# nipponjo/tts-arabic-pytorch

Measured on AMD Instinct MI355X. Metric: audio samples/sec (FastPitch+HiFi-GAN, synthetic 64-phoneme inputs), higher is better.
Workload: dtype f32

## Files before the change

### include/ttsamd.h

```cpp
#ifndef TTSAMD_H
#define TTSAMD_H

#include <stdint.h>

#ifdef __cplusplus
extern "C" {
#endif

#define TTSAMD_OK 0
#define TTSAMD_EINVAL (-1)
#define TTSAMD_EHIP (-2)
#define TTSAMD_ENOMEM (-3)

typedef struct ttsamd_tensor {
    const char* name;
    const float* data;
    int32_t ndim;
    int64_t shape[4];
} ttsamd_tensor;

typedef struct ttsamd_hifigan_cfg {
    int32_t num_mels;
    int32_t upsample_initial_channel;
    int32_t n_ups;
    int32_t upsample_rates[8];
    int32_t upsample_kernel_sizes[8];
    int32_t n_kernels;
    int32_t resblock_kernel_sizes[8];
    int32_t n_dilations;
    int32_t resblock_dilations[8][8];
} ttsamd_hifigan_cfg;

typedef struct ttsamd_fastpitch_cfg {
    int32_t n_mel_channels;
    int32_t n_symbols;
    int32_t padding_idx;
    int32_t d_model;
    int32_t in_fft_n_layers, in_fft_n_heads, in_fft_d_head, in_fft_kernel, in_fft_filter;
    int32_t out_fft_n_layers, out_fft_n_heads, out_fft_d_head, out_fft_kernel, out_fft_filter;
    int32_t dur_kernel, dur_filter, dur_n_layers;
    int32_t pitch_kernel, pitch_filter, pitch_n_layers, pitch_emb_kernel;
    int32_t energy_conditioning, energy_kernel, energy_filter, energy_n_layers, energy_emb_kernel;
    int32_t n_speakers;
    float speaker_emb_weight;
} ttsamd_fastpitch_cfg;

typedef struct ttsamd_tacotron2_cfg {
    int32_t n_symbol;
    int32_t num_speakers;
    int32_t speaker_embedding_dim;
    int32_t symbol_embedding_dim;
    int32_t encoder_embedding_dim;
    int32_t encoder_n_convolution;
    int32_t encoder_kernel_size;
    int32_t n_mels;
    int32_t prenet_dim;
    int32_t attention_rnn_dim;
    int32_t decoder_rnn_dim;
    int32_t attention_hidden_dim;
    int32_t attention_location_n_filter;
    int32_t attention_location_kernel_size;
    int32_t postnet_n_convolution;
    int32_t postnet_kernel_size;
    int32_t postnet_embedding_dim;
    float gate_threshold;
    int32_t decoder_early_stopping;
} ttsamd_tacotron2_cfg;

typedef struct ttsamd_tagger_cfg {
    int32_t n_vocab;
    int32_t emb_dim;
    int32_t n_lstm;
    int32_t lstm_hidden[4];
    int32_t hard_sigmoid;
    int32_t bn_after_lstm0;
    float bn_eps;
    int32_t n_dense;
    int32_t dense_dim[4];
} ttsamd_tagger_cfg;

const char* ttsamd_last_error(void);
#define TTSAMD_ABI_VERSION 7
int32_t ttsamd_version(void);
int32_t ttsamd_set_option(const char* name, const char* value);
int32_t ttsamd_get_option(const char* name, char* value, int32_t capacity);
const char* ttsamd_option_name(int32_t index);
int32_t ttsamd_options_check(void);
int32_t ttsamd_device_ok(void);


int32_t ttsamd_hifigan_create(const ttsamd_tensor* weights, int32_t n_weights,
                              const ttsamd_hifigan_cfg* cfg, void** handle);
int32_t ttsamd_hifigan_destroy(void* handle);
int64_t ttsamd_hifigan_workspace_bytes(void* handle, int32_t batch, int32_t t_max);
int32_t ttsamd_hifigan_forward(void* handle, const float* mel, const int64_t* lens,
                               int32_t batch, int32_t t_max, float* wave,
                               void* workspace, int64_t workspace_bytes, void* stream);


int32_t ttsamd_fastpitch_create(const ttsamd_tensor* weights, int32_t n_weights,
                                const ttsamd_fastpitch_cfg* cfg, void** handle);
int32_t ttsamd_fastpitch_destroy(void* handle);
int64_t ttsamd_fastpitch_encode_workspace_bytes(void* handle, int32_t batch, int32_t n_tokens);
int64_t ttsamd_fastpitch_decode_workspace_bytes(void* handle, int32_t batch, int32_t t_max);

int32_t ttsamd_fastpitch_encode(void* handle, const int64_t* ids, int32_t batch, int32_t n_tokens,
                                int32_t speaker, float pace, const float* dur_tgt,
                                const float* pitch_tgt, const float* energy_tgt,
                                float pitch_mul, float pitch_add, float max_duration,
                                float* enc_cond, float* dur_pred, float* pitch_pred,
                                float* energy_pred, int64_t* reps, int64_t* dec_lens,
                                void* workspace, int64_t workspace_bytes, void* stream);

int32_t ttsamd_length_regulate(const float* enc, const int64_t* reps, int32_t batch,
                               int32_t n_tokens, int32_t channels, int32_t t_max,
                               float* out, int32_t* idx, void* stream);

int32_t ttsamd_fastpitch_decode(void* handle, float* x, const int64_t* dec_lens, int32_t batch,
                                int32_t t_max, float* mel, void* workspace,
                                int64_t workspace_bytes, void* stream);

int32_t ttsamd_fastpitch_set_batch_mode(void* handle, int32_t mode);

int32_t ttsamd_denoiser_create(void** handle);
int32_t ttsamd_denoiser_destroy(void* handle);
int64_t ttsamd_denoiser_workspace_bytes(int32_t batch, int32_t n_max);
int32_t ttsamd_denoiser_bias_spec(void* handle, const float* audio, const int64_t* n_dev, int32_t n,
                                  float* bias_spec, void* workspace, int64_t workspace_bytes,
                                  void* stream);
int32_t ttsamd_denoise(void* handle, float* wave, int64_t wave_stride, const int64_t* nsamples,
                       int32_t batch, int32_t n_max, const float* bias_spec, float strength,
                       void* workspace, int64_t workspace_bytes, void* stream);

int32_t ttsamd_vocos_create(const ttsamd_tensor* weights, int32_t n_weights, int32_t input_channels,
                            int32_t dim, int32_t intermediate_dim, int32_t num_layers, void** handle);
int32_t ttsamd_vocos_destroy(void* handle);
int64_t ttsamd_vocos_workspace_bytes(void* handle, int32_t batch, int32_t t_max);
int32_t ttsamd_vocos_bias_vec(void* handle, float* bias_vec, void* workspace, int64_t workspace_bytes,
                              void* stream);
int32_t ttsamd_vocos_forward(void* handle, const float* mel, const int64_t* lens, int32_t batch,
                             int32_t t_max, float denoise, const float* bias_vec, float* wave,
                             void* workspace, int64_t workspace_bytes, void* stream);

int32_t ttsamd_tacotron2_create(const ttsamd_tensor* weights, int32_t n_weights,
                                const ttsamd_tacotron2_cfg* cfg, void** handle);
int32_t ttsamd_tacotron2_destroy(void* handle);
int64_t ttsamd_tacotron2_workspace_bytes(void* handle, int32_t batch, int32_t n_tokens, int32_t max_step);
int32_t ttsamd_tacotron2_infer(void* handle, const int64_t* tokens, const int64_t* lengths,
                               const int64_t* speaker_ids, int32_t batch, int32_t n_tokens, int32_t max_step,
                               int64_t dropout_seed, float* mel_post, int32_t* mel_lens, float* alignments,
                               float* mel_raw, int32_t* n_steps, void* workspace, int64_t workspace_bytes,
                               void* stream);

int32_t ttsamd_tagger_create(const ttsamd_tensor* weights, int32_t n_weights, const ttsamd_tagger_cfg* cfg,
                             void** handle);
int32_t ttsamd_tagger_destroy(void* handle);
int64_t ttsamd_tagger_workspace_bytes(void* handle, int32_t batch, int32_t n_chars);
int32_t ttsamd_tagger_forward(void* handle, const int64_t* ids, int32_t batch, int32_t n_chars, float* probs,
                              void* workspace, int64_t workspace_bytes, void* stream);


int64_t ttsamd_conv1d_packed_floats(int32_t cout, int32_t cin, int32_t k);
int32_t ttsamd_conv1d(const float* x, const float* w, const float* bias, const int64_t* lens,
                      int32_t batch, int32_t cin, int32_t cout, int32_t k, int32_t dilation,
                      int32_t lin, float in_slope, int32_t relu_out, float* y, float* packed,
                      void* stream);
int32_t ttsamd_conv1d_ex(const float* x, const float* w, const float* bias, const float* res, const int64_t* lens, int32_t batch,
                         int32_t cin, int32_t cout, int32_t k, int32_t dilation, int32_t lin, float in_slope,
                         int32_t relu_out, int32_t mode, float div, float* y, float* packed, void* stream);

int64_t ttsamd_resblock_pair_packed_floats(int32_t channels, int32_t k, int32_t variant);
int32_t ttsamd_resblock_pair(const float* x, float* y, const float* w1, const float* b1, const float* w2, const float* b2,
                             int32_t channels, int32_t k, int32_t dil, const int64_t* lens, int32_t len_mul, int32_t L,
                             int32_t batch, int32_t mode, float div, float slope, int32_t variant, float* packed, int64_t packed_floats,
                             void* stream);

int32_t ttsamd_bfo_pack(const float* x, int32_t batch, int32_t channels, int32_t len, float slope, void* out, void* stream);
int32_t ttsamd_bfo_unpack(const void* in, int32_t batch, int32_t channels, int32_t len, float slope, float* out, void* stream);
int64_t ttsamd_bfo_weight_elems(int32_t cout, int32_t cin, int32_t k, int32_t up);
int32_t ttsamd_bfo_pack_weight(const float* w, int32_t cout, int32_t cin, int32_t k, int32_t up, uint16_t* out);
int32_t ttsamd_bfo_conv1d(const void* x, const void* w_packed, const float* bias, const void* res, const void* sum_in,
                          const int64_t* lens, int32_t len_mul, int32_t batch, int32_t cin, int32_t cout, int32_t k,
                          int32_t dilation, int32_t up, int32_t len_in, int32_t mode, float div, float res_slope,
                          float out_slope, void* y, float* y_f32, const float* res_f32, void* stream);
int32_t ttsamd_bfo_resblock_pair(const void* x, const void* w1, const float* b1, const void* w2, const float* b2,
                                 const void* sum_in, const int64_t* lens, int32_t len_mul, int32_t batch, int32_t channels,
                                 int32_t k, int32_t dilation, int32_t len, int32_t mode, float div, float in_slope,
                                 float mid_slope, float out_slope, void* y, void* stream);
int32_t ttsamd_bfo_resblock_chain(const void* x, const void* const* w1, const float* const* b1, const void* const* w2,
                                  const float* const* b2, const int32_t* dilations, const void* sum_in, const int64_t* lens,
                                  int32_t len_mul, int32_t batch, int32_t channels, int32_t len, int32_t mode, float div,
                                  float in_slope, float mid_slope, float out_slope, void* y, void* stream, int32_t k);
int32_t ttsamd_bfo_conv_post(const void* x, const float* w, const float* bias, const int64_t* lens, int32_t len_mul,
                             int32_t batch, int32_t channels, int32_t len, float* wave, int64_t wave_stride, void* stream);

int32_t ttsamd_bfo3_pack(const float* x, int32_t batch, int32_t channels, int32_t len, float slope, void* out, void* stream);
int32_t ttsamd_bfo3_unpack(const void* in, int32_t batch, int32_t channels, int32_t len, float slope, float* out, void* stream);
int64_t ttsamd_bfo3_weight_elems(int32_t cout, int32_t cin, int32_t k, int32_t up);
int32_t ttsamd_bfo3_pack_weight(const float* w, int32_t cout, int32_t cin, int32_t k, int32_t up, uint16_t* out);
int32_t ttsamd_bfo3_conv1d(const void* x, const void* w_packed, const float* bias, const void* res, const void* sum_in,
                           const int64_t* lens, int32_t len_mul, int32_t batch, int32_t cin, int32_t cout, int32_t k,
                           int32_t dilation, int32_t up, int32_t len_in, int32_t mode, float div, float res_slope,
                           float out_slope, void* y, float* y_f32, const float* res_f32, void* stream);
int32_t ttsamd_bfo3_resblock_pair(const void* x, const void* w1, const float* b1, const void* w2, const float* b2,
                                  const void* sum_in, const int64_t* lens, int32_t len_mul, int32_t batch, int32_t channels,
                                  int32_t k, int32_t dilation, int32_t len, int32_t mode, float div, float in_slope,
                                  float mid_slope, float out_slope, void* y, void* stream);
int32_t ttsamd_bfo3_resblock_chain(const void* x, const void* const* w1, const float* const* b1, const void* const* w2,
                                   const float* const* b2, const int32_t* dilations, const void* sum_in, const int64_t* lens,
                                   int32_t len_mul, int32_t batch, int32_t channels, int32_t len, int32_t mode, float div,
                                   float in_slope, float mid_slope, float out_slope, void* y, void* stream);
int32_t ttsamd_bfo3_conv_post(const void* x, const float* w, const float* bias, const int64_t* lens, int32_t len_mul,
                              int32_t batch, int32_t channels, int32_t len, float* wave, int64_t wave_stride, void* stream);

int32_t ttsamd_set_precision(int32_t precision);
int32_t ttsamd_get_precision(void);

#define TTSAMD_DP_ID_BYTES 128
#define TTSAMD_DP_HIFIGAN 0
#define TTSAMD_DP_FASTPITCH 1
int32_t ttsamd_dp_unique_id(void* id128 );
int32_t ttsamd_dp_init(int32_t rank, int32_t world, const void* id128 , void** comm);
int32_t ttsamd_dp_destroy(void* comm);
int32_t ttsamd_dp_rank(void* comm);
int32_t ttsamd_dp_world(void* comm);
int32_t ttsamd_dp_broadcast(void* comm, void* buf, int64_t nbytes, int32_t root, void* stream);
int32_t ttsamd_dp_broadcast_weights(void* comm, int32_t kind, void* handle, int32_t root, void* stream);
int32_t ttsamd_dp_allgather(void* comm, const void* send, void* recv, int64_t nbytes_per_rank, void* stream);
int32_t ttsamd_dp_pack_audio(const float* wave, int64_t wave_stride, const int64_t* nsamples, int32_t batch,
                             int64_t n_max, float* packed, void* stream);
int32_t ttsamd_dp_gather_audio(void* comm, const float* packed, float* recv, const int64_t* counts,
                               const int64_t* offsets, int32_t root, void* stream);

int32_t ttsamd_profile_enable(int32_t on);
int32_t ttsamd_profile_read(double* out3);

#ifdef __cplusplus
}
#endif
#endif
```

### tts-arabic-pytorch_amd/csrc/api.hip

```cpp
#include <cerrno>
#include <cstdio>
#include <cstdlib>
#include <cstring>
#include <algorithm>
#include <atomic>
#include <mutex>
#include <string>
#include <vector>

#include "kernels.hpp"

namespace ttsamd {

static thread_local std::string g_err;

void set_error(const char* fmt, ...) {
    char buf[1024];
    va_list ap;
    va_start(ap, fmt);
    vsnprintf(buf, sizeof(buf), fmt, ap);
    va_end(ap);
    g_err = buf;
}

static int g_precision = 0;
int32_t default_precision() { return g_precision; }

struct Prof {
    std::mutex mu;
    bool on = false;
    std::vector<hipEvent_t> ev;
    size_t used = 0;
    size_t launches = 0;
    double flops_per_frame = 0.0;
} g_prof;

void prof_section_begin(hipStream_t s) {
    if (!g_prof.on) return;
    std::lock_guard<std::mutex> lk(g_prof.mu);
    if (g_prof.used + 2 > g_prof.ev.size()) {
        hipEvent_t a, b;
        if (hipEventCreate(&a) != hipSuccess || hipEventCreate(&b) != hipSuccess) return;
        g_prof.ev.push_back(a);
        g_prof.ev.push_back(b);
    }
    (void)hipEventRecord(g_prof.ev[g_prof.used], s);
}

void prof_section_end(hipStream_t s) {
    if (!g_prof.on) return;
    std::lock_guard<std::mutex> lk(g_prof.mu);
    if (g_prof.used + 2 > g_prof.ev.size()) return;
    (void)hipEventRecord(g_prof.ev[g_prof.used + 1], s);
    g_prof.used += 2;
}

void prof_add(double flops_per_frame) {
    if (!g_prof.on) return;
    std::lock_guard<std::mutex> lk(g_prof.mu);
    g_prof.launches += 1;
    g_prof.flops_per_frame += flops_per_frame;
}

void prof_begin(hipStream_t s, double flops_per_frame) {
    prof_section_begin(s);
    prof_add(flops_per_frame);
}

void prof_end(hipStream_t s) { prof_section_end(s); }

struct HifiGan;
struct FastPitch;
struct Denoiser;
struct Vocos;
int32_t vocos_create(const ttsamd_tensor*, int32_t, int32_t, int32_t, int32_t, int32_t, Vocos**);
void vocos_destroy(Vocos*);
int64_t vocos_workspace_bytes(const Vocos*, int32_t, int32_t);
int64_t vocos_bias_workspace_bytes(const Vocos*);
int32_t vocos_bias_vec(const Vocos*, float*, void*, int64_t, hipStream_t);
int32_t vocos_forward(const Vocos*, const float*, const int64_t*, int32_t, int32_t, float, const float*, float*, void*,
                      int64_t, hipStream_t);
struct Taco2;
int32_t tacotron2_create(const ttsamd_tensor*, int32_t, const ttsamd_tacotron2_cfg*, Taco2**);
void tacotron2_destroy(Taco2*);
int64_t tacotron2_workspace_bytes(const Taco2*, int32_t, int32_t, int32_t);
int32_t tacotron2_infer(const Taco2*, const int64_t*, const int64_t*, const int64_t*, int32_t, int32_t, int32_t, int64_t,
                        float*, int32_t*, float*, float*, int32_t*, void*, int64_t, hipStream_t);
struct Tagger;
int32_t tagger_create(const ttsamd_tensor*, int32_t, const ttsamd_tagger_cfg*, Tagger**);
void tagger_destroy(Tagger*);
int64_t tagger_workspace_bytes(const Tagger*, int32_t, int32_t);
int32_t tagger_forward(const Tagger*, const int64_t*, int32_t, int32_t, float*, void*, int64_t, hipStream_t);
int32_t denoiser_create(Denoiser**);
void denoiser_destroy(Denoiser*);
int64_t denoiser_workspace_bytes(int32_t, int32_t);
int32_t denoiser_bias_spec(const Denoiser*, const float*, const int64_t*, int32_t, float*, void*, int64_t, hipStream_t);
int32_t denoise(const Denoiser*, float*, int64_t, const int64_t*, int32_t, int32_t, const float*, float, void*, int64_t,
                hipStream_t);
int32_t hifigan_create(const ttsamd_tensor*, int32_t, const ttsamd_hifigan_cfg*, HifiGan**);
void hifigan_destroy(HifiGan*);
int64_t hifigan_workspace_bytes(const HifiGan*, int32_t, int32_t);
int32_t hifigan_forward(const HifiGan*, const float*, const int64_t*, int32_t, int32_t, float*, void*, int64_t,
                        hipStream_t);
int32_t fastpitch_create(const ttsamd_tensor*, int32_t, const ttsamd_fastpitch_cfg*, int32_t, FastPitch**);
void fastpitch_destroy(FastPitch*);
int64_t fastpitch_encode_workspace_bytes(const FastPitch*, int32_t, int32_t);
int64_t fastpitch_decode_workspace_bytes(const FastPitch*, int32_t, int32_t);
int32_t fastpitch_encode(const FastPitch*, const int64_t*, int32_t, int32_t, int32_t, float, const float*,
                         const float*, const float*, float, float, float, float*, float*, float*, float*, int64_t*,
                         int64_t*, void*, int64_t, hipStream_t);
void fastpitch_set_batch_mode(const FastPitch*, int);
int32_t fastpitch_decode(const FastPitch*, float*, const int64_t*, int32_t, int32_t, float*, void*, int64_t,
                         hipStream_t);

__global__ void pack_conv_weight_kernel(const float* __restrict__ w, int cout, int cin, int k, int cp,
                                        float* __restrict__ out) {
    const int64_t i = (int64_t)blockIdx.x * 256 + threadIdx.x;
    const int64_t n = (int64_t)cin * k * cp;
    if (i >= n) return;
    const int pq = (int)(i % 4);
    const int co = (int)((i / 4) % cp);
    const int kk = (int)((i / (4 * (int64_t)cp)) % 2);
    const int t = (int)((i / (8 * (int64_t)cp)) % k);
    const int o = (int)(i / (8 * (int64_t)cp * k));
    out[i] = co < cout ? w[((int64_t)co * cin + (8 * o + 2 * pq + kk)) * k + t] : 0.f;
}

__global__ void split_bf16_kernel(const float* __restrict__ packed, int64_t n, unsigned short* __restrict__ out) {
    const int64_t i = (int64_t)blockIdx.x * 256 + threadIdx.x;
    if (i >= n) return;
    const float f = packed[i];
    unsigned u = __float_as_uint(f);
    u += 0x7fffu + ((u >> 16) & 1u);
    const unsigned h = u >> 16;
    const float r = f - __uint_as_float(h << 16);
    unsigned v = __float_as_uint(r);
    v += 0x7fffu + ((v >> 16) & 1u);
    out[i] = (unsigned short)h;
    out[n + i] = (unsigned short)(v >> 16);
}

namespace {
struct OptDesc { const char* name; int kind; long long lo, hi; };
const OptDesc kOpts[OPT_COUNT] = {
#define TTS_OPT_DESC(name, kind, lo, hi) {"TTSAMD_" #name, kind, lo, hi},
    TTS_OPTIONS(TTS_OPT_DESC)
#undef TTS_OPT_DESC
};
std::atomic<const char*> g_opt[OPT_COUNT];
std::once_flag g_opt_once;
std::string g_opt_env_error;

bool opt_valid(const OptDesc& d, const char* v) {
    if (!v || !*v) return false;
    char* end = nullptr;
    errno = 0;
    const long long x = std::strtoll(v, &end, d.kind == 1 ? 16 : 10);
    return errno == 0 && end != v && *end == '\0' && x >= d.lo && x <= d.hi;
}
void opt_init() {
    std::call_once(g_opt_once, [] {
        for (int i = 0; i < OPT_COUNT; ++i) {
            const char* e = std::getenv(kOpts[i].name);
            if (!e || !*e) continue;
            if (!opt_valid(kOpts[i], e)) {
                if (g_opt_env_error.empty()) {
                    char buf[256];
                    std::snprintf(buf, sizeof buf, "%s='%s' in the environment is not a valid value (%s in [%llx, %llx])", kOpts[i].name, e,
                                  kOpts[i].kind == 1 ? "hex mask" : "integer", kOpts[i].lo, kOpts[i].hi);
                    g_opt_env_error = buf;
                }
                continue;
            }
            g_opt[i].store(strdup(e), std::memory_order_release);
        }
    });
}
int opt_find(const char* name) {
    if (!name) return -1;
    for (int i = 0; i < OPT_COUNT; ++i)
        if (std::strcmp(name, kOpts[i].name) == 0 || std::strcmp(name, kOpts[i].name + 7) == 0) return i;
    return -1;
}
}

int64_t opt_int(Opt o, int64_t unset) {
    opt_init();
    const char* v = g_opt[o].load(std::memory_order_acquire);
    return v ? (int64_t)std::strtoll(v, nullptr, kOpts[o].kind == 1 ? 16 : 10) : unset;
}

}

using namespace ttsamd;

extern "C" {

const char* ttsamd_last_error(void) { return g_err.c_str(); }
int32_t ttsamd_version(void) { return TTSAMD_ABI_VERSION; }

int32_t ttsamd_set_option(const char* name, const char* value) {
    opt_init();
    const int i = opt_find(name);
    TTS_REQUIRE(i >= 0, "set_option: unknown option '%s' (ttsamd_option_name lists them)", name ? name : "(null)");
    if (!value || !*value) {
        g_opt[i].store(nullptr, std::memory_order_release);
        return 0;
    }
    TTS_REQUIRE(opt_valid(kOpts[i], value), "set_option: %s='%s' is not a valid value (%s in [%llx, %llx])", kOpts[i].name, value,
                kOpts[i].kind == 1 ? "hex mask" : "integer", kOpts[i].lo, kOpts[i].hi);
    g_opt[i].store(strdup(value), std::memory_order_release);
    return 0;
}
int32_t ttsamd_get_option(const char* name, char* value, int32_t capacity) {
    opt_init();
    const int i = opt_find(name);
    TTS_REQUIRE(i >= 0 && value && capacity > 0, "get_option: unknown option '%s' or no buffer", name ? name : "(null)");
    const char* v = g_opt[i].load(std::memory_order_acquire);
    std::snprintf(value, (size_t)capacity, "%s", v ? v : "");
    return 0;
}
const char* ttsamd_option_name(int32_t index) { return (index >= 0 && index < OPT_COUNT) ? kOpts[index].name : nullptr; }
int32_t ttsamd_options_check(void) {
    opt_init();
    TTS_REQUIRE(g_opt_env_error.empty(), "%s", g_opt_env_error.c_str());
    return 0;
}

int32_t ttsamd_device_ok(void) {
    int n = 0;
    if (hipGetDeviceCount(&n) != hipSuccess || n <= 0) return 0;
    hipDeviceProp_t prop;
    if (hipGetDeviceProperties(&prop, 0) != hipSuccess) return 0;
    return std::string(prop.gcnArchName).rfind("gfx950", 0) == 0 ? 1 : 0;
}

int32_t ttsamd_hifigan_create(const ttsamd_tensor* weights, int32_t n, const ttsamd_hifigan_cfg* cfg, void** handle) {
    HifiGan* h = nullptr;
    const int32_t rc = hifigan_create(weights, n, cfg, &h);
    if (rc == 0) *handle = h;
    return rc;
}
int32_t ttsamd_hifigan_destroy(void* handle) {
    hifigan_destroy((HifiGan*)handle);
    return 0;
}
int64_t ttsamd_hifigan_workspace_bytes(void* handle, int32_t batch, int32_t t_max) {
    if (!handle || batch < 1 || t_max < 1) return 0;
    return hifigan_workspace_bytes((HifiGan*)handle, batch, t_max);
}
int32_t ttsamd_hifigan_forward(void* handle, const float* mel, const int64_t* lens, int32_t batch, int32_t t_max,
                               float* wave, void* workspace, int64_t workspace_bytes, void* stream) {
    return hifigan_forward((HifiGan*)handle, mel, lens, batch, t_max, wave, workspace, workspace_bytes,
                           (hipStream_t)stream);
}

int32_t ttsamd_fastpitch_create(const ttsamd_tensor* weights, int32_t n, const ttsamd_fastpitch_cfg* cfg,
                                void** handle) {
    FastPitch* h = nullptr;
    const int32_t rc = fastpitch_create(weights, n, cfg, 16384, &h);
    if (rc == 0) *handle = h;
    return rc;
}
int32_t ttsamd_fastpitch_destroy(void* handle) {
    fastpitch_destroy((FastPitch*)handle);
    return 0;
}
int64_t ttsamd_fastpitch_encode_workspace_bytes(void* handle, int32_t batch, int32_t n_tokens) {
    if (!handle || batch < 1 || n_tokens < 1) return 0;
    return fastpitch_encode_workspace_bytes((FastPitch*)handle, batch, n_tokens);
}
int64_t ttsamd_fastpitch_decode_workspace_bytes(void* handle, int32_t batch, int32_t t_max) {
    if (!handle || batch < 1 || t_max < 1) return 0;
    return fastpitch_decode_workspace_bytes((FastPitch*)handle, batch, t_max);
}
int32_t ttsamd_fastpitch_encode(void* handle, const int64_t* ids, int32_t batch, int32_t n_tokens, int32_t speaker,
                                float pace, const float* dur_tgt, const float* pitch_tgt, const float* energy_tgt,
                                float pitch_mul, float pitch_add, float max_duration, float* enc_cond,
                                float* dur_pred, float* pitch_pred, float* energy_pred, int64_t* reps,
                                int64_t* dec_lens, void* workspace, int64_t workspace_bytes, void* stream) {
    return fastpitch_encode((FastPitch*)handle, ids, batch, n_tokens, speaker, pace, dur_tgt, pitch_tgt, energy_tgt,
                            pitch_mul, pitch_add, max_duration, enc_cond, dur_pred, pitch_pred, energy_pred, reps,
                            dec_lens, workspace, workspace_bytes, (hipStream_t)stream);
}
int32_t ttsamd_length_regulate(const float* enc, const int64_t* reps, int32_t batch, int32_t n_tokens,
                               int32_t channels, int32_t t_max, float* out, int32_t* idx, void* stream) {
    TTS_REQUIRE(enc && reps && out && batch >= 1 && n_tokens >= 1 && channels >= 1 && t_max >= 0,
                "length_regulate: bad argument");
    return launch_regulate_gather(enc, reps, nullptr, 0, batch, n_tokens, channels, t_max, out, idx,
                                  (hipStream_t)stream);
}
int32_t ttsamd_fastpitch_set_batch_mode(void* handle, int32_t mode) {
    TTS_REQUIRE(handle != nullptr, "fastpitch_set_batch_mode: null handle");
    TTS_REQUIRE(mode == 0 || mode == 1, "fastpitch_set_batch_mode: mode %d (0 = padded-batch arithmetic, 1 = every utterance alone)", mode);
    fastpitch_set_batch_mode((const FastPitch*)handle, mode);
    return 0;
}
int32_t ttsamd_fastpitch_decode(void* handle, float* x, const int64_t* dec_lens, int32_t batch, int32_t t_max,
                                float* mel, void* workspace, int64_t workspace_bytes, void* stream) {
    return fastpitch_decode((FastPitch*)handle, x, dec_lens, batch, t_max, mel, workspace, workspace_bytes,
                            (hipStream_t)stream);
}

int32_t ttsamd_denoiser_create(void** handle) {
    Denoiser* h = nullptr;
    const int32_t rc = denoiser_create(&h);
    if (rc == 0) *handle = h;
    return rc;
}
int32_t ttsamd_denoiser_destroy(void* handle) {
    denoiser_destroy((Denoiser*)handle);
    return 0;
}
int64_t ttsamd_denoiser_workspace_bytes(int32_t batch, int32_t n_max) {
    if (batch < 1 || n_max < 1) return 0;
    return denoiser_workspace_bytes(batch, n_max);
}
int32_t ttsamd_denoiser_bias_spec(void* handle, const float* audio, const int64_t* n_dev, int32_t n,
                                  float* bias_spec, void* workspace, int64_t workspace_bytes, void* stream) {
    return denoiser_bias_spec((Denoiser*)handle, audio, n_dev, n, bias_spec, workspace, workspace_bytes,
                              (hipStream_t)stream);
}
int32_t ttsamd_denoise(void* handle, float* wave, int64_t wave_stride, const int64_t* nsamples, int32_t batch,
                       int32_t n_max, const float* bias_spec, float strength, void* workspace,
                       int64_t workspace_bytes, void* stream) {
    return denoise((Denoiser*)handle, wave, wave_stride, nsamples, batch, n_max, bias_spec, strength, workspace,
                   workspace_bytes, (hipStream_t)stream);
}

int32_t ttsamd_vocos_create(const ttsamd_tensor* weights, int32_t n, int32_t input_channels, int32_t dim,
                            int32_t intermediate_dim, int32_t num_layers, void** handle) {
    Vocos* h = nullptr;
    const int32_t rc = vocos_create(weights, n, input_channels, dim, intermediate_dim, num_layers, &h);
    if (rc == 0) *handle = h;
    return rc;
}
int32_t ttsamd_vocos_destroy(void* handle) {
    vocos_destroy((Vocos*)handle);
    return 0;
}
int64_t ttsamd_vocos_workspace_bytes(void* handle, int32_t batch, int32_t t_max) {
    if (!handle || batch < 1 || t_max < 1) return 0;
    const int64_t a = vocos_workspace_bytes((Vocos*)handle, batch, t_max), b = vocos_bias_workspace_bytes((Vocos*)handle);
    return a > b ? a : b;
}
int32_t ttsamd_vocos_bias_vec(void* handle, float* bias_vec, void* workspace, int64_t workspace_bytes, void* stream) {
    return vocos_bias_vec((Vocos*)handle, bias_vec, workspace, workspace_bytes, (hipStream_t)stream);
}
int32_t ttsamd_vocos_forward(void* handle, const float* mel, const int64_t* lens, int32_t batch, int32_t t_max,
                             float denoise, const float* bias_vec, float* wave, void* workspace,
                             int64_t workspace_bytes, void* stream) {
    return vocos_forward((Vocos*)handle, mel, lens, batch, t_max, denoise, bias_vec, wave, workspace, workspace_bytes,
                         (hipStream_t)stream);
}

int32_t ttsamd_tacotron2_create(const ttsamd_tensor* weights, int32_t n, const ttsamd_tacotron2_cfg* cfg, void** handle) {
    TTS_REQUIRE(handle, "tacotron2_create: null handle");
    Taco2* h = nullptr;
    const int32_t rc = tacotron2_create(weights, n, cfg, &h);
    if (rc == 0) *handle = h;
    return rc;
}
int32_t ttsamd_tacotron2_destroy(void* handle) {
    tacotron2_destroy((Taco2*)handle);
    return 0;
}
int64_t ttsamd_tacotron2_workspace_bytes(void* handle, int32_t batch, int32_t n_tokens, int32_t max_step) {
    if (!handle || batch < 1 || n_tokens < 1 || max_step < 1) return 0;
    return tacotron2_workspace_bytes((Taco2*)handle, batch, n_tokens, max_step);
}
int32_t ttsamd_tacotron2_infer(void* handle, const int64_t* tokens, const int64_t* lengths, const int64_t* speaker_ids,
                               int32_t batch, int32_t n_tokens, int32_t max_step, int64_t dropout_seed, float* mel_post,
                               int32_t* mel_lens, float* alignments, float* mel_raw, int32_t* n_steps, void* workspace,
                               int64_t workspace_bytes, void* stream) {
    return tacotron2_infer((Taco2*)handle, tokens, lengths, speaker_ids, batch, n_tokens, max_step, dropout_seed, mel_post,
                           mel_lens, alignments, mel_raw, n_steps, workspace, workspace_bytes, (hipStream_t)stream);
}

int32_t ttsamd_tagger_create(const ttsamd_tensor* weights, int32_t n, const ttsamd_tagger_cfg* cfg, void** handle) {
    TTS_REQUIRE(handle, "tagger_create: null handle");
    Tagger* h = nullptr;
    const int32_t rc = tagger_create(weights, n, cfg, &h);
    if (rc == 0) *handle = h;
    return rc;
}
int32_t ttsamd_tagger_destroy(void* handle) {
    tagger_destroy((Tagger*)handle);
    return 0;
}
int64_t ttsamd_tagger_workspace_bytes(void* handle, int32_t batch, int32_t n_chars) {
    if (!handle || batch < 1 || n_chars < 1) return 0;
    return tagger_workspace_bytes((Tagger*)handle, batch, n_chars);
}
int32_t ttsamd_tagger_forward(void* handle, const int64_t* ids, int32_t batch, int32_t n_chars, float* probs,
                              void* workspace, int64_t workspace_bytes, void* stream) {
    return tagger_forward((Tagger*)handle, ids, batch, n_chars, probs, workspace, workspace_bytes, (hipStream_t)stream);
}

int64_t ttsamd_conv1d_packed_floats(int32_t cout, int32_t cin, int32_t k) {
    return 2 * (int64_t)cin * k * cout_padded(cout) +
           ((k == 3 || k == 7 || k == 11) ? (int64_t)cin * (wino2_groups(k) + wino4_groups(k)) * cout_padded(cout) : 0);
}

__global__ void pack_wino4_weight_kernel(const float* __restrict__ w, int cout, int cin, int k, int cp, float* __restrict__ out) {
    const int ng = k == 3 ? 6 : (k == 7 ? 16 : 24), nsf = k == 3 ? 1 : (k == 7 ? 2 : 4);
    const int64_t i = (int64_t)blockIdx.x * 256 + threadIdx.x;
    const int64_t n = (int64_t)cin * ng * cp;
    if (i >= n) return;
    const int pq = (int)(i & 3);
    const int64_t r = i >> 2;
    const int co = (int)(r % cp);
    const int64_t r2 = r / cp;
    const int kk = (int)(r2 & 1);
    const int64_t r3 = r2 >> 1;
    const int t = (int)(r3 % ng), o = (int)(r3 / ng);
    float v = 0.f;
    if (co < cout) {
        const float* g = w + ((int64_t)co * cin + (8 * o + 2 * pq + kk)) * k;
        if (t < 6 * nsf) {
            const int s = t / 6, j = t % 6;
            const double g0 = g[3 * s], g1 = 3 * s + 1 < k ? g[3 * s + 1] : 0.0, g2 = 3 * s + 2 < k ? g[3 * s + 2] : 0.0;
            v = j == 0 ? (float)(g0 / 4) : (j == 1 ? (float)(-(g0 + g1 + g2) / 6) : (j == 2 ? (float)(-(g0 - g1 + g2) / 6) :
                (j == 3 ? (float)(g0 / 24 + g1 / 12 + g2 / 6) : (j == 4 ? (float)(g0 / 24 - g1 / 12 + g2 / 6) : (float)g2))));
        } else {
            v = g[6];
        }
    }
    out[i] = v;
}

__global__ void pack_wino2_weight_kernel(const float* __restrict__ w, int cout, int cin, int k, int cp, float* __restrict__ out) {
    const int ns = k / 3, ng = 4 * ns + 2 * (k - 3 * ns);
    const int64_t i = (int64_t)blockIdx.x * 256 + threadIdx.x;
    const int64_t n = (int64_t)cin * ng * cp;
    if (i >= n) return;
    const int pq = (int)(i & 3);
    const int64_t r = i >> 2;
    const int co = (int)(r % cp);
    const int64_t r2 = r / cp;
    const int kk = (int)(r2 & 1);
    const int64_t r3 = r2 >> 1;
    const int t = (int)(r3 % ng), o = (int)(r3 / ng);
    float v = 0.f;
    if (co < cout) {
        const float* g = w + ((int64_t)co * cin + (8 * o + 2 * pq + kk)) * k;
        if (t < 4 * ns) {
            const int s = t >> 2, j = t & 3;
            const double g0 = g[3 * s], g1 = g[3 * s + 1], g2 = g[3 * s + 2];
            v = j == 0 ? (float)g0 : (j == 1 ? (float)((g0 + g1 + g2) * 0.5) : (j == 2 ? (float)((g0 - g1 + g2) * 0.5) : (float)g2));
        } else {
            const int l = (t - 4 * ns) >> 1;
            v = ((t - 4 * ns) & 1) ? -g[3 * ns + l] : g[3 * ns + l];
        }
    }
    out[i] = v;
}

int32_t ttsamd_conv1d_ex(const float* x, const float* w, const float* bias, const float* res, const int64_t* lens, int32_t batch,
                         int32_t cin, int32_t cout, int32_t k, int32_t dilation, int32_t lin, float in_slope,
                         int32_t relu_out, int32_t mode, float div, float* y, float* packed, void* stream) {
    TTS_REQUIRE(x && w && y && packed, "conv1d: null argument");
    TTS_REQUIRE(mode >= 0 && mode <= 2 && (mode != 2 || div != 0.f), "conv1d: bad mode / div");
    TTS_REQUIRE(relu_out == 0 || mode == 0, "conv1d: relu_out with an accumulate mode (mode %d) is not defined", mode);
    hipStream_t s = (hipStream_t)stream;
    const int cp = cout_padded(cout);
    const int64_t n = (int64_t)cin * k * cp;
    hipLaunchKernelGGL(pack_conv_weight_kernel, dim3((unsigned)((n + 255) / 256)), dim3(256), 0, s, w, cout, cin, k,
                       cp, packed);
    TTS_CHECK_HIP(hipGetLastError());
    ConvParams p;
    std::memset(&p, 0, sizeof(p));
    p.x = x; p.x_bs = (int64_t)cin * lin; p.x_cs = lin;
    p.w = packed; p.bias = bias;
    p.precision = default_precision();
    if (p.precision != 0) {
        unsigned short* planes = reinterpret_cast<unsigned short*>(packed + n);
        hipLaunchKernelGGL(split_bf16_kernel, dim3((unsigned)((n + 255) / 256)), dim3(256), 0, s, packed, n, planes);
        TTS_CHECK_HIP(hipGetLastError());
        p.w_bf16 = planes;
    }
    if ((k == 3 || k == 7 || k == 11) && p.precision == 0 && cin % 8 == 0) {
        float* wino = packed + 2 * n;
        const int64_t nw = (int64_t)cin * wino2_groups(k) * cp;
        hipLaunchKernelGGL(pack_wino2_weight_kernel, dim3((unsigned)((nw + 255) / 256)), dim3(256), 0, s, w, cout, cin, k, cp, wino);
        TTS_CHECK_HIP(hipGetLastError());
        p.w_wino = wino;
        float* wino4 = wino + nw;
        const int64_t nw4 = (int64_t)cin * wino4_groups(k) * cp;
        hipLaunchKernelGGL(pack_wino4_weight_kernel, dim3((unsigned)((nw4 + 255) / 256)), dim3(256), 0, s, w, cout, cin, k, cp, wino4);
        TTS_CHECK_HIP(hipGetLastError());
        p.w_wino4 = wino4;
    }
    p.y = y; p.y_bs = (int64_t)cout * lin; p.y_cs = lin; p.y_ts = 1;
    p.lens_in = lens; p.lens_out = lens; p.len_in_mul = 1; p.len_out_mul = 1;
    p.Lin = lin; p.Nout = lin; p.Cin = cin; p.Cout = cout; p.CoutP = cp; p.K = k;
    p.dil = dilation; p.pad = (k * dilation - dilation) / 2;
    p.res = res; p.r_bs = (int64_t)cout * lin; p.r_cs = lin;
    p.n_phase = 1; p.in_slope = in_slope; p.relu_out = relu_out; p.mode = mode; p.div = div; p.batch = batch;
    prof_begin(s, 2.0 * cout * cin * k);
    const int32_t rc = launch_conv(p, s);
    prof_end(s);
    return rc;
}

int32_t ttsamd_conv1d(const float* x, const float* w, const float* bias, const int64_t* lens, int32_t batch,
                      int32_t cin, int32_t cout, int32_t k, int32_t dilation, int32_t lin, float in_slope,
                      int32_t relu_out, float* y, float* packed, void* stream) {
    return ttsamd_conv1d_ex(x, w, bias, nullptr, lens, batch, cin, cout, k, dilation, lin, in_slope, relu_out, 0, 1.f, y, packed, stream);
}

int64_t ttsamd_resblock_pair_packed_floats(int32_t channels, int32_t k, int32_t variant) {
    if (channels < 1 || k < 1) return 0;
    const int64_t n = 2 * (int64_t)channels * k * channels;
    const int nwino = (variant == 4 ? 1 : (variant == 5 ? 2 : 0));
    if (variant == 6) return n + ((k == 3 || k == 7 || k == 11) ? 2 * (int64_t)channels * wino4_groups(k) * channels : 0);
    return n + ((k == 3 || k == 7 || k == 11) ? nwino * (int64_t)channels * wino2_groups(k) * channels : 0);
}

int32_t ttsamd_resblock_pair(const float* x, float* y, const float* w1, const float* b1, const float* w2, const float* b2,
                             int32_t channels, int32_t k, int32_t dil, const int64_t* lens, int32_t len_mul, int32_t L,
                             int32_t batch, int32_t mode, float div, float slope, int32_t variant, float* packed, int64_t packed_floats,
                             void* stream) {
    TTS_REQUIRE(x && y && w1 && b1 && w2 && b2 && packed && channels % 32 == 0 && k >= 1 && batch >= 1 && L >= 1 && len_mul >= 1 &&
                mode >= 0 && mode <= 2, "resblock_pair: bad argument");
    TTS_REQUIRE(packed_floats >= ttsamd_resblock_pair_packed_floats(channels, k, variant),
                "resblock_pair: `packed` holds %lld floats, variant %d at C = %d, k = %d needs %lld (ttsamd_resblock_pair_packed_floats)",
                (long long)packed_floats, variant, channels, k, (long long)ttsamd_resblock_pair_packed_floats(channels, k, variant));
    hipStream_t s = (hipStream_t)stream;
    const int64_t n = (int64_t)channels * k * channels;
    for (int i = 0; i < 2; ++i) {
        hipLaunchKernelGGL(pack_conv_weight_kernel, dim3((unsigned)((n + 255) / 256)), dim3(256), 0, s, i == 0 ? w1 : w2, channels,
                           channels, k, channels, packed + i * n);
        TTS_CHECK_HIP(hipGetLastError());
    }
    const double fl = 2.0 * (2.0 * channels * channels * k);
    int32_t rc;
    prof_begin(s, fl);
    if (variant == 1) {
        rc = launch_fused_pair(channels, x, y, packed, b1, packed + n, b2, k, dil, lens, len_mul, L, batch, mode, div, slope, s);
    } else if (variant >= 2 && variant <= 5) {
        const float *w2w = nullptr, *w1w = nullptr;
        if (variant >= 4) {
            TTS_REQUIRE((k == 3 || k == 7 || k == 11) && (channels <= 64 || (variant == 5 && channels == 128)),
                        "resblock_pair: variants 4 / 5 are built for C = 32 / 64 (5: and 128), k = 3 / 7 / 11");
            const int64_t nw = (int64_t)channels * wino2_groups(k) * channels;
            for (int i = 0; i < (variant == 5 ? 2 : 1); ++i) {
                float* wino = packed + 2 * n + i * nw;
                hipLaunchKernelGGL(pack_wino2_weight_kernel, dim3((unsigned)((nw + 255) / 256)), dim3(256), 0, s, i == 0 ? w2 : w1, channels,
                                   channels, k, channels, wino);
                TTS_CHECK_HIP(hipGetLastError());
                (i == 0 ? w2w : w1w) = wino;
            }
        }
        rc = launch_fused_pair2(channels, x, y, packed, b1, packed + n, b2, k, dil, lens, len_mul, L, batch, mode, div, slope,
                                variant == 3 ? 1 : 2, s, w2w, w1w);
    } else if (variant == 6) {
        TTS_REQUIRE(channels == 32 && (k == 3 || k == 7 || k == 11), "resblock_pair: variant 6 is built for C = 32, k = 3 / 7 / 11");
        const int64_t nw4 = (int64_t)channels * wino4_groups(k) * channels;
        for (int i = 0; i < 2; ++i) {
            hipLaunchKernelGGL(pack_wino4_weight_kernel, dim3((unsigned)((nw4 + 255) / 256)), dim3(256), 0, s, i == 0 ? w1 : w2, channels,
                               channels, k, channels, packed + 2 * n + i * nw4);
            TTS_CHECK_HIP(hipGetLastError());
        }
        rc = launch_fused_pair4(channels, x, y, packed + 2 * n, b1, packed + 2 * n + nw4, b2, k, dil, lens, len_mul, L, batch, mode, div,
                                slope, s);
    } else if (variant == -1) {
        rc = 0;
    } else {
        set_error("resblock_pair: variant %d (1: first generation, 2 / 3: second generation with 256- / 128-column blocks, 4 / 5: 256 columns + Winograd phase B / both phases, 6: C = 32 with both phases on Winograd F(4,3))", variant);
        rc = TTSAMD_EINVAL;
    }
    prof_end(s);
    return rc;
}

int32_t ttsamd_set_precision(int32_t precision) {
    TTS_REQUIRE(precision >= 0 && precision <= 2, "set_precision: 0 = fp32 MFMA, 1 = bf16 MFMA, 2 = split-bf16 MFMA");
    g_precision = precision;
    return 0;
}
int32_t ttsamd_get_precision(void) { return g_precision; }

int32_t ttsamd_profile_enable(int32_t on) {
    std::lock_guard<std::mutex> lk(g_prof.mu);
    g_prof.on = on != 0;
    g_prof.used = 0;
    g_prof.launches = 0;
    g_prof.flops_per_frame = 0.0;
    return 0;
}

int32_t ttsamd_profile_read(double* out3) {
    TTS_REQUIRE(out3, "profile_read: null argument");
    std::lock_guard<std::mutex> lk(g_prof.mu);
    std::vector<std::pair<float, float>> iv;
    for (size_t i = 0; i + 1 < g_prof.used; i += 2) {
        TTS_CHECK_HIP(hipEventSynchronize(g_prof.ev[i + 1]));
        float t0 = 0.f, t1 = 0.f;
        if (i > 0) TTS_CHECK_HIP(hipEventElapsedTime(&t0, g_prof.ev[0], g_prof.ev[i]));
        TTS_CHECK_HIP(hipEventElapsedTime(&t1, g_prof.ev[0], g_prof.ev[i + 1]));
        iv.emplace_back(t0, std::max(t0, t1));
    }
    std::sort(iv.begin(), iv.end());
    double ms = 0.0;
    float lo = 0.f, hi = -1.f;
    for (const auto& v : iv) {
        if (hi < lo || v.first > hi) {
            if (hi >= lo) ms += hi - lo;
            lo = v.first;
            hi = v.second;
        } else {
            hi = std::max(hi, v.second);
        }
    }
    if (hi >= lo) ms += hi - lo;
    out3[0] = ms;
    out3[1] = (double)g_prof.launches;
    out3[2] = (double)(g_prof.used / 2);
    return 0;
}

}
```

### tts-arabic-pytorch_amd/csrc/common.hpp

```cpp
#pragma once
#include <hip/hip_runtime.h>
#include <stdint.h>
#include <atomic>
#include <cstdarg>
#include <cstdio>
#include <cstdlib>
#include <string>

#include "../../include/ttsamd.h"

namespace ttsamd {

void set_error(const char* fmt, ...);

#define TTS_CHECK_HIP(expr)                                                         \
    do {                                                                            \
        hipError_t e_ = (expr);                                                     \
        if (e_ != hipSuccess) {                                                     \
            ttsamd::set_error("%s failed: %s (%s:%d)", #expr, hipGetErrorString(e_), \
                              __FILE__, __LINE__);                                  \
            return TTSAMD_EHIP;                                                     \
        }                                                                           \
    } while (0)

#define TTS_REQUIRE(cond, ...)              \
    do {                                    \
        if (!(cond)) {                      \
            ttsamd::set_error(__VA_ARGS__); \
            return TTSAMD_EINVAL;           \
        }                                   \
    } while (0)

#define TTS_TRY(expr)               \
    do {                            \
        int32_t rc_ = (expr);       \
        if (rc_ != 0) return rc_;   \
    } while (0)

inline int64_t align_up(int64_t x, int64_t a) { return (x + a - 1) / a * a; }

inline hipError_t lds_opt_in(const void* fn, int bytes, std::atomic<uint64_t>& done) {
    int dev = 0;
    hipError_t e = hipGetDevice(&dev);
    if (e != hipSuccess) return e;
    if (dev >= 0 && dev < 64 && ((done.load(std::memory_order_acquire) >> dev) & 1)) return hipSuccess;
    e = hipFuncSetAttribute(fn, hipFuncAttributeMaxDynamicSharedMemorySize, bytes);
    if (e == hipSuccess && dev >= 0 && dev < 64) done.fetch_or(1ull << dev, std::memory_order_release);
    return e;
}

#define TTS_OPTIONS(X)                                                                                     \
    X(HIFIGAN_STREAMS, 0, 0, 1)    \
    X(WINO, 0, 0, 1)                                              \
    X(WINO2, 0, 0, 31)             \
    X(WINO4, 0, 0, 31)             \
    X(FUSED_PAIR, 0, 0, 1)                   \
    X(FUSED2, 0, 0, 1)                                           \
    X(FUSED2_MASK, 1, 0, 0x1ff)               \
    X(FUSED2_MASK_N1, 1, 0, 0x1ff)          \
    X(FUSED2_WB, 0, 0, 2)                     \
    X(PAIR4, 0, 0, 1)              \
    X(CONVT, 0, 0, 1)                              \
    X(BFO, 0, 0, 1)                \
    X(BFO_CHAIN, 0, 0, 1)                           \
    X(BFO_CHAIN7, 0, 0, 1)                                 \
    X(BFO_FF, 0, 0, 1)                              \
    X(BFO_SPLITK, 0, 0, 1)                                              \
    X(BFO_SMALL_TILES, 0, 0, 1)            \
    X(BF16_ATTN, 0, 0, 1)                                         \
    X(BF16_PACKED_T, 0, 0, 1)                   \
    X(ATT_RA, 0, 1, 4)                             \
    X(ATT_SPLIT, 0, 0, 1)                      \
    X(XCD_W, 0, 0, 1)                            \
    X(XCD_WMAX_KB, 0, 0, 1 << 20)     \
    X(DEEP_SPLITK, 0, 0, 1)        \
    X(TACO_PERSISTENT, 0, 0, 2)    \
    X(TACO_SEG, 0, 8, 1 << 20)
enum Opt : int {
#define TTS_OPT_ENUM(name, kind, lo, hi) OPT_##name,
    TTS_OPTIONS(TTS_OPT_ENUM)
#undef TTS_OPT_ENUM
    OPT_COUNT
};
int64_t opt_int(Opt o, int64_t unset);

struct Arena {
    char* base;
    int64_t size;
    int64_t off = 0;
    bool ok = true;
    Arena(void* p, int64_t n) : base((char*)p), size(n) {}
    template <typename T>
    T* take(int64_t count) {
        int64_t bytes = align_up(count * (int64_t)sizeof(T), 256);
        if (base != nullptr && off + bytes > size) ok = false;
        T* r = base ? (T*)(base + off) : nullptr;
        off += bytes;
        return r;
    }
};

struct ConvParams {
    const float* x;
    int64_t x_bs;
    int32_t x_cs;
    const float* w;
    const void* w_bf16;
    const float* w_wino;
    const float* w_wino4;
    int32_t precision;
    const float* bias;
    float* y;
    int64_t y_bs;
    int32_t y_cs, y_ts;
    const float* res;
    int64_t r_bs;
    int32_t r_cs;
    const int64_t* lens_in;
    const int64_t* lens_out;
    int32_t len_in_mul, len_out_mul;
    int32_t Lin, Nout;
    int32_t Cin, Cout, CoutP, K;
    int32_t dil, pad;
    int32_t n_phase;
    int32_t phase_p;
    float in_slope;
    const float* scale;
    int32_t relu_out;
    int32_t mode;
    float div;
    int32_t batch;
    float* splitk_ws;
    int64_t splitk_floats;
    int32_t ksplit;
    int32_t y_packed;
    float pack_slope;
    int32_t x_packed;
    int32_t xcd_w;
    int32_t tile_major;
    int32_t compact;
    unsigned long long* timing;
};
constexpr int64_t kSplitKFloats = 4 << 20;
constexpr int64_t kSplitKFloatsFp = 8 << 20;

void conv_log(const char* kind, int K, int cin, int cout, int nout, int batch, int has_res, int mode, int len_mul, int ragged,
              int n_phase);
bool compact_order(const void* lens, int batch);
int32_t launch_conv(const ConvParams& p, hipStream_t stream);
bool convt_supported(const ConvParams& p);
int32_t launch_convt(const ConvParams& p, hipStream_t stream);
bool fused_pair_supported(int32_t channels, int32_t k, int32_t dil, int32_t L, const float* x, const float* y);
int32_t launch_fused_pair(int32_t channels, const float* x, float* y, const float* w1, const float* b1, const float* w2,
                          const float* b2, int32_t k, int32_t dil, const int64_t* lens, int32_t len_mul, int32_t L, int32_t batch,
                          int32_t mode, float div, float slope, hipStream_t stream);
bool fused_pair2_supported(int32_t channels, int32_t k, int32_t dil, int32_t L, const float* x, const float* y, int32_t ntw);
int32_t launch_fused_pair2(int32_t channels, const float* x, float* y, const float* w1, const float* b1, const float* w2,
                           const float* b2, int32_t k, int32_t dil, const int64_t* lens, int32_t len_mul, int32_t L, int32_t batch,
                           int32_t mode, float div, float slope, int32_t ntw, hipStream_t stream, const float* w2_wino = nullptr,
                           const float* w1_wino = nullptr);
bool fused_pair4_supported(int32_t channels, int32_t k, int32_t dil, int32_t L, const float* x, const float* y);
int32_t launch_fused_pair4(int32_t channels, const float* x, float* y, const float* w1_wino4, const float* b1, const float* w2_wino4,
                           const float* b2, int32_t k, int32_t dil, const int64_t* lens, int32_t len_mul, int32_t L, int32_t batch,
                           int32_t mode, float div, float slope, hipStream_t stream);
int wino_route(const ConvParams& p);
int32_t launch_wino(const ConvParams& p, hipStream_t stream);
void pack_wino_weight(const float* w, int cout, int cin, float* out);
int wino2_groups(int k);
int wino2_block_outputs(int coutp, int dil);
int32_t launch_wino2(const ConvParams& p, hipStream_t stream);
void pack_wino2_weight(const float* w, int cout, int cin, int k, float* out);
int wino4_groups(int k);
int wino4_block_outputs(int dil);
int wino4_ksplit(const ConvParams& p);
int32_t launch_splitk_reduce(const ConvParams& q, hipStream_t stream);
int32_t launch_wino4(const ConvParams& p, hipStream_t stream);
void wino4_filter_groups(const float* g, int k, float* o);
void pack_wino4_weight(const float* w, int cout, int cin, int k, float* out);
void pack_conv_weight(const float* w, int cout, int cin, int k, float* out);
void pack_convt_weight(const float* w, int cin, int cout, int kt, int u, int p, float* out);
inline int cout_padded(int cout) { return (int)align_up(cout, 32); }
void split_packed_bf16(const float* packed, int64_t n, uint16_t* out);
int32_t default_precision();

#ifdef __HIPCC__
__device__ __forceinline__ bool live_tile(const int64_t* __restrict__ lens, const int mul, const int n_max, const int tile_w,
                                          const int batch, const unsigned lin, int& b, int& tile) {
    const int lane = threadIdx.x & 63;
    unsigned base = 0;
    for (int u0 = 0; u0 < batch; u0 += 64) {
        int n = 0;
        if (u0 + lane < batch) n = (max(min(n_max, (int)lens[u0 + lane] * mul), 0) + tile_w - 1) / tile_w;
        int incl = n;
#pragma unroll
        for (int d = 1; d < 64; d <<= 1) {
            const int t = __shfl_up(incl, d, 64);
            if (lane >= d) incl += t;
        }
        const unsigned total = (unsigned)__shfl(incl, 63, 64);
        if (lin < base + total) {
            const unsigned long long m = __ballot(base + (unsigned)incl > lin);
            const int l = __ffsll((long long)m) - 1;
            b = u0 + l;
            tile = (int)(lin - base) - (__shfl(incl, l, 64) - __shfl(n, l, 64));
            return true;
        }
        base += total;
    }
    return false;
}
#endif

}
```

### tts-arabic-pytorch_amd/csrc/hifigan.hip

```cpp
#include <cmath>
#include <cstring>
#include <cstdlib>
#include <map>
#include <mutex>
#include <string>
#include <vector>

#include "kernels.hpp"
#include "bfo3.hpp"

namespace ttsamd {

constexpr unsigned kFused2Mask = 0x00F;
constexpr int kPair4MinK = 7;
constexpr unsigned kFused2MaskN1 = 0x000;
constexpr int64_t kFused2SmallColumns = 2 * 256 * 252;

struct ConvW {
    int64_t w_off = 0, b_off = 0;
    int64_t w16_off = 0, w_n = 0;
    int64_t wo_off = -1;
    int64_t wo3_off = -1;
    int64_t ww4_off = -1;
    int64_t ww_off = -1;
    int cin = 0, cout = 0, k = 0;
};

struct HifiGan {
    ttsamd_hifigan_cfg cfg;
    float* dev = nullptr;
    uint16_t* dev16 = nullptr;
    int64_t dev_n = 0, dev16_n = 0;
    ConvW conv_pre, conv_post;
    std::vector<ConvW> ups;
    std::vector<ConvW> c1, c2;
    int hop = 1;
    int64_t max_cl = 0;
    bool bfo_ok = false;
    mutable std::mutex mu;
    mutable hipStream_t side[2] = {nullptr, nullptr};
    mutable hipEvent_t ev_fork = nullptr, ev_done[3] = {nullptr, nullptr, nullptr};
};

static bool use_branch_streams(const HifiGan* h, int32_t B, int32_t T) {
    if (h->cfg.n_kernels != 3) return false;
    const int64_t streams = opt_int(OPT_HIFIGAN_STREAMS, -1);
    if (streams >= 0) return streams == 1;
    if (default_precision() == 1 && h->bfo_ok) {
        if (opt_int(OPT_BFO, 1) != 0) return (int64_t)B * T >= 8192;
    }
    return true;
}

struct Fused2Switches {
    bool on = true, mask_forced = false;
    bool wino_b = true, wino_a = true;
    bool pair4 = true;
    unsigned mask = kFused2Mask, mask_n1 = kFused2MaskN1;
};
static Fused2Switches read_fused2_switches() {
    Fused2Switches sw;
    sw.on = opt_int(OPT_FUSED2, 1) != 0;
    const int64_t m = opt_int(OPT_FUSED2_MASK, -1);
    sw.mask_forced = m >= 0;
    if (sw.mask_forced) sw.mask = (unsigned)m;
    sw.mask_n1 = (unsigned)opt_int(OPT_FUSED2_MASK_N1, kFused2MaskN1);
    const int64_t wb = opt_int(OPT_FUSED2_WB, 2);
    sw.wino_b = wb != 0;
    sw.wino_a = wb == 2;
    sw.pair4 = opt_int(OPT_PAIR4, 1) != 0;
    return sw;
}

static int fused2_choice(const Fused2Switches& sw, int32_t channels, int32_t k, int32_t dil, int32_t L, const float* x, const float* y,
                         int64_t columns) {
    if (!sw.on) return 0;
    const int ci = channels == 32 ? 0 : (channels == 64 ? 1 : (channels == 128 ? 2 : -1));
    const int ki = k == 3 ? 0 : (k == 7 ? 1 : (k == 11 ? 2 : -1));
    if (ci < 0 || ki < 0) return 0;
    const unsigned bit = 1u << (3 * ci + ki);
    const bool small = columns < (int64_t)kFused2SmallColumns && !sw.mask_forced;
    if (small) return 0;
    if (!(sw.mask & bit)) return 0;
    int ntw = (sw.mask_n1 & bit) ? 1 : 2;
    if (!fused_pair2_supported(channels, k, dil, L, x, y, ntw)) {
        ntw = 3 - ntw;
        if (!fused_pair2_supported(channels, k, dil, L, x, y, ntw)) return 0;
    }
    return ntw;
}

using TensorMap = std::map<std::string, const ttsamd_tensor*>;

static int64_t numel(const ttsamd_tensor* t) {
    int64_t n = 1;
    for (int i = 0; i < t->ndim; ++i) n *= t->shape[i];
    return n;
}

static int32_t folded_weight(const TensorMap& tm, const std::string& base, int ndim_expected,
                             std::vector<float>& out, int64_t shape[3]) {
    const ttsamd_tensor *w = nullptr, *g = nullptr, *v = nullptr;
    auto it = tm.find(base + ".weight");
    if (it != tm.end()) w = it->second;
    if (!w) {
        auto ig = tm.find(base + ".parametrizations.weight.original0");
        auto iv = tm.find(base + ".parametrizations.weight.original1");
        if (ig == tm.end() || iv == tm.end()) {
            ig = tm.find(base + ".weight_g");
            iv = tm.find(base + ".weight_v");
        }
        TTS_REQUIRE(ig != tm.end() && iv != tm.end(), "hifigan: no weight for layer '%s'", base.c_str());
        g = ig->second;
        v = iv->second;
    }
    const ttsamd_tensor* src = w ? w : v;
    TTS_REQUIRE(src->ndim == ndim_expected, "hifigan: '%s' has ndim %d, expected %d", base.c_str(), src->ndim,
                ndim_expected);
    for (int i = 0; i < 3; ++i) shape[i] = src->shape[i];
    const int64_t n = numel(src);
    out.resize(n);
    if (w) {
        std::memcpy(out.data(), w->data, n * sizeof(float));
        return 0;
    }
    const int64_t d0 = v->shape[0], inner = n / d0;
    TTS_REQUIRE(numel(g) == d0, "hifigan: '%s' weight_g has %lld elements, expected %lld", base.c_str(),
                (long long)numel(g), (long long)d0);
    for (int64_t i = 0; i < d0; ++i) {
        double ss = 0.0;
        const float* vr = v->data + i * inner;
        for (int64_t j = 0; j < inner; ++j) ss += (double)vr[j] * vr[j];
        const float scale = g->data[i] / (float)std::sqrt(ss);
        for (int64_t j = 0; j < inner; ++j) out[i * inner + j] = vr[j] * scale;
    }
    return 0;
}

static int32_t get_bias(const TensorMap& tm, const std::string& base, int n, std::vector<float>& blob,
                        int64_t& off) {
    auto it = tm.find(base + ".bias");
    TTS_REQUIRE(it != tm.end() && numel(it->second) == n, "hifigan: missing/mis-sized '%s.bias'", base.c_str());
    off = (int64_t)blob.size();
    blob.insert(blob.end(), it->second->data, it->second->data + n);
    blob.resize(align_up((int64_t)blob.size(), 64));
    return 0;
}

static void add_bf16(std::vector<float>& blob, std::vector<uint16_t>& blob16, ConvW& cw, int64_t n) {
    cw.w_n = n;
    cw.w16_off = (int64_t)blob16.size();
    blob16.resize(blob16.size() + 2 * n);
    split_packed_bf16(blob.data() + cw.w_off, n, blob16.data() + cw.w16_off);
}

static int32_t add_conv(const TensorMap& tm, const std::string& base, int cin, int cout, int k,
                        std::vector<float>& blob, std::vector<uint16_t>& blob16, ConvW& cw) {
    std::vector<float> w;
    int64_t shp[3];
    TTS_TRY(folded_weight(tm, base, 3, w, shp));
    TTS_REQUIRE(shp[0] == cout && shp[1] == cin && shp[2] == k, "hifigan: '%s' has shape [%lld,%lld,%lld], expected [%d,%d,%d]",
                base.c_str(), (long long)shp[0], (long long)shp[1], (long long)shp[2], cout, cin, k);
    cw.cin = cin; cw.cout = cout; cw.k = k;
    cw.w_off = (int64_t)blob.size();
    blob.resize(blob.size() + (size_t)cin * k * cout_padded(cout));
    pack_conv_weight(w.data(), cout, cin, k, blob.data() + cw.w_off);
    add_bf16(blob, blob16, cw, (int64_t)cin * k * cout_padded(cout));
    if ((k == 3 || k == 7 || k == 11) && cin % 8 == 0 && cout % 32 == 0) {
        blob.resize(align_up((int64_t)blob.size(), 64));
        cw.ww_off = (int64_t)blob.size();
        blob.resize(blob.size() + (size_t)cin * wino2_groups(k) * cout_padded(cout));
        pack_wino2_weight(w.data(), cout, cin, k, blob.data() + cw.ww_off);
        if (cout >= 64 || (cout == 32 && cin == 32 && k >= kPair4MinK)) {
            blob.resize(align_up((int64_t)blob.size(), 64));
            cw.ww4_off = (int64_t)blob.size();
            blob.resize(blob.size() + (size_t)cin * wino4_groups(k) * cout_padded(cout));
            pack_wino4_weight(w.data(), cout, cin, k, blob.data() + cw.ww4_off);
        }
    }
    if (cin % 8 == 0 && cout % 32 == 0) {
        blob16.resize(align_up((int64_t)blob16.size(), 64));
        cw.wo_off = (int64_t)blob16.size();
        blob16.resize(blob16.size() + (size_t)bfo_packed_conv_elems(cout, cin, k));
        bfo_pack_conv_weight(w.data(), cout, cin, k, blob16.data() + cw.wo_off);
        blob16.resize(align_up((int64_t)blob16.size(), 64));
        cw.wo3_off = (int64_t)blob16.size();
        blob16.resize(blob16.size() + (size_t)bfo3_packed_conv_elems(cout, cin, k));
        bfo3_pack_conv_weight(w.data(), cout, cin, k, blob16.data() + cw.wo3_off);
    }
    blob.resize(align_up((int64_t)blob.size(), 64));
    return get_bias(tm, base, cout, blob, cw.b_off);
}

void hifigan_destroy(HifiGan* h);

__global__ void hifigan_touch_kernel() {}

int32_t hifigan_create(const ttsamd_tensor* weights, int32_t n, const ttsamd_hifigan_cfg* cfg, HifiGan** out) {
    TTS_REQUIRE(weights && cfg && out, "hifigan_create: null argument");
    TTS_REQUIRE(cfg->n_ups >= 1 && cfg->n_ups <= 8 && cfg->n_kernels >= 1 && cfg->n_kernels <= 8 &&
                cfg->n_dilations >= 1 && cfg->n_dilations <= 8, "hifigan_create: bad config counts");
    TensorMap tm;
    for (int i = 0; i < n; ++i) tm[weights[i].name] = &weights[i];
    auto* h = new HifiGan();
    h->cfg = *cfg;
    std::vector<float> blob;
    std::vector<uint16_t> blob16;
    const int c0 = cfg->upsample_initial_channel;
    int32_t rc = add_conv(tm, "conv_pre", cfg->num_mels, c0, 7, blob, blob16, h->conv_pre);
    int ch = c0, mul = 1;
    h->max_cl = c0;
    for (int i = 0; rc == 0 && i < cfg->n_ups; ++i) {
        const int u = cfg->upsample_rates[i], kt = cfg->upsample_kernel_sizes[i];
        const int cin = ch, cout = ch / 2;
        if (kt != 2 * u || (kt - u) % 2 != 0) {
            set_error("hifigan: upsample kernel %d / rate %d: only kernel = 2*rate is built", kt, u);
            rc = TTSAMD_EINVAL;
            break;
        }
        std::vector<float> w;
        int64_t shp[3];
        rc = folded_weight(tm, "ups." + std::to_string(i), 3, w, shp);
        if (rc) break;
        if (shp[0] != cin || shp[1] != cout || shp[2] != kt) {
            set_error("hifigan: ups.%d has shape [%lld,%lld,%lld], expected [%d,%d,%d]", i, (long long)shp[0],
                      (long long)shp[1], (long long)shp[2], cin, cout, kt);
            rc = TTSAMD_EINVAL;
            break;
        }
        ConvW cw;
        cw.cin = cin; cw.cout = cout; cw.k = kt;
        cw.w_off = (int64_t)blob.size();
        blob.resize(blob.size() + (size_t)u * cin * 2 * cout_padded(cout));
        pack_convt_weight(w.data(), cin, cout, kt, u, (kt - u) / 2, blob.data() + cw.w_off);
        add_bf16(blob, blob16, cw, (int64_t)u * cin * 2 * cout_padded(cout));
        if (cin % 16 == 0 && cout % 32 == 0 && (u == 8 || u == 2)) {
            blob16.resize(align_up((int64_t)blob16.size(), 64));
            cw.wo_off = (int64_t)blob16.size();
            blob16.resize(blob16.size() + (size_t)bfo_packed_convt_elems(cin, cout, u));
            bfo_pack_convt_weight(w.data(), cin, cout, u, blob16.data() + cw.wo_off);
            blob16.resize(align_up((int64_t)blob16.size(), 64));
            cw.wo3_off = (int64_t)blob16.size();
            blob16.resize(blob16.size() + (size_t)bfo3_packed_convt_elems(cin, cout, u));
            bfo3_pack_convt_weight(w.data(), cin, cout, u, blob16.data() + cw.wo3_off);
        }
        blob.resize(align_up((int64_t)blob.size(), 64));
        rc = get_bias(tm, "ups." + std::to_string(i), cout, blob, cw.b_off);
        if (rc) break;
        h->ups.push_back(cw);
        ch = cout;
        mul *= u;
        h->max_cl = std::max<int64_t>(h->max_cl, (int64_t)ch * mul);
        for (int j = 0; rc == 0 && j < cfg->n_kernels; ++j) {
            const int r = i * cfg->n_kernels + j, kk = cfg->resblock_kernel_sizes[j];
            for (int m = 0; rc == 0 && m < cfg->n_dilations; ++m) {
                ConvW a, b;
                rc = add_conv(tm, "resblocks." + std::to_string(r) + ".convs1." + std::to_string(m), ch, ch, kk, blob, blob16, a);
                if (rc) break;
                rc = add_conv(tm, "resblocks." + std::to_string(r) + ".convs2." + std::to_string(m), ch, ch, kk, blob, blob16, b);
                h->c1.push_back(a);
                h->c2.push_back(b);
            }
        }
    }
    h->hop = mul;
    if (rc == 0) {
        bool ok = h->conv_pre.wo_off >= 0 && ch == 32 && cfg->num_mels % 8 == 0;
        for (const ConvW& cw : h->ups) ok = ok && cw.wo_off >= 0;
        for (size_t i = 0; i < h->c1.size(); ++i) ok = ok && h->c1[i].wo_off >= 0 && h->c2[i].wo_off >= 0;
        for (int j = 0; j < cfg->n_kernels; ++j) {
            const int kk = cfg->resblock_kernel_sizes[j];
            ok = ok && (kk == 3 || kk == 7 || kk == 11);
            for (int m = 0; m < cfg->n_dilations; ++m) ok = ok && cfg->resblock_dilations[j][m] >= 1 && cfg->resblock_dilations[j][m] <= BFO_DMAX;
        }
        h->bfo_ok = ok;
    }
    if (rc == 0) {
        std::vector<float> w;
        int64_t shp[3];
        rc = folded_weight(tm, "conv_post", 3, w, shp);
        if (rc == 0 && (shp[0] != 1 || shp[1] != ch || shp[2] != 7)) {
            set_error("hifigan: conv_post has shape [%lld,%lld,%lld], expected [1,%d,7]", (long long)shp[0],
                      (long long)shp[1], (long long)shp[2], ch);
            rc = TTSAMD_EINVAL;
        }
        if (rc == 0) {
            h->conv_post.cin = ch; h->conv_post.cout = 1; h->conv_post.k = 7;
            h->conv_post.w_off = (int64_t)blob.size();
            blob.insert(blob.end(), w.begin(), w.end());
            blob.resize(align_up((int64_t)blob.size(), 64));
            rc = get_bias(tm, "conv_post", 1, blob, h->conv_post.b_off);
        }
    }
    if (rc == 0) {
        h->dev_n = (int64_t)blob.size();
        h->dev16_n = (int64_t)blob16.size();
        hipError_t e = hipMalloc((void**)&h->dev, blob.size() * sizeof(float));
        if (e == hipSuccess) e = hipMemcpy(h->dev, blob.data(), blob.size() * sizeof(float), hipMemcpyHostToDevice);
        if (e == hipSuccess) e = hipMalloc((void**)&h->dev16, blob16.size() * sizeof(uint16_t));
        if (e == hipSuccess) e = hipMemcpy(h->dev16, blob16.data(), blob16.size() * sizeof(uint16_t), hipMemcpyHostToDevice);
        if (e != hipSuccess) {
            set_error("hifigan_create: weight upload failed: %s", hipGetErrorString(e));
            rc = TTSAMD_EHIP;
        }
        if (e == hipSuccess && cfg->n_kernels == 3) {
            for (auto& st : h->side)
                if (e == hipSuccess) {
                    int lo = 0, hi = 0;
                    (void)hipDeviceGetStreamPriorityRange(&lo, &hi);
                    e = hipStreamCreateWithPriority(&st, hipStreamNonBlocking, hi);
                }
            if (e == hipSuccess) e = hipEventCreateWithFlags(&h->ev_fork, hipEventDisableTiming);
            for (auto& ev : h->ev_done)
                if (e == hipSuccess) e = hipEventCreateWithFlags(&ev, hipEventDisableTiming);
            for (auto& st : h->side)
                if (e == hipSuccess) {
                    hipLaunchKernelGGL(hifigan_touch_kernel, dim3(1), dim3(64), 0, st);
                    e = hipGetLastError();
                }
            for (auto& st : h->side)
                if (e == hipSuccess && st) e = hipStreamSynchronize(st);
            if (e != hipSuccess) {
                set_error("hifigan_create: branch streams: %s", hipGetErrorString(e));
                rc = TTSAMD_EHIP;
            }
        }
    }
    if (rc != 0) {
        hifigan_destroy(h);
        return rc;
    }
    *out = h;
    return 0;
}

void hifigan_destroy(HifiGan* h) {
    if (!h) return;
    if (h->dev) (void)hipFree(h->dev);
    if (h->dev16) (void)hipFree(h->dev16);
    for (hipStream_t st : h->side) if (st) (void)hipStreamDestroy(st);
    if (h->ev_fork) (void)hipEventDestroy(h->ev_fork);
    for (hipEvent_t e : h->ev_done) if (e) (void)hipEventDestroy(e);
    delete h;
}

int64_t hifigan_workspace_bytes(const HifiGan* h, int32_t B, int32_t T) {
    Arena a(nullptr, 0);
    const int nb = use_branch_streams(h, B, T) ? 3 : 1;
    for (int i = 0; i < 2 + 2 * nb; ++i) a.take<float>((int64_t)B * h->max_cl * T);
    for (int i = 0; i < nb; ++i) a.take<float>(kSplitKFloats);
    a.take<uint16_t>((int64_t)B * align_up(h->cfg.num_mels, 8) * T * 2);
    return a.off;
}

int32_t hifigan_forward(const HifiGan* h, const float* mel, const int64_t* lens, int32_t B, int32_t T, float* wave,
                        void* ws, int64_t ws_bytes, hipStream_t s) {
    TTS_REQUIRE(h && mel && wave && B >= 1 && T >= 1, "hifigan_forward: bad argument");
    Arena a(ws, ws_bytes);
    const bool multi = use_branch_streams(h, B, T);
    const int nb = multi ? 3 : 1;
    float* cur = a.take<float>((int64_t)B * h->max_cl * T);
    float* ups_out = a.take<float>((int64_t)B * h->max_cl * T);
    float *Tbs[3], *Rs[3], *splitks[3];
    for (int i = 0; i < nb; ++i) {
        Tbs[i] = a.take<float>((int64_t)B * h->max_cl * T);
        Rs[i] = a.take<float>((int64_t)B * h->max_cl * T);
    }
    for (int i = 0; i < nb; ++i) splitks[i] = a.take<float>(kSplitKFloats);
    for (int i = nb; i < 3; ++i) { Tbs[i] = Tbs[0]; Rs[i] = Rs[0]; splitks[i] = splitks[0]; }
    uint16_t* mel_o = a.take<uint16_t>((int64_t)B * align_up(h->cfg.num_mels, 8) * T * 2);
    if (!ws || !a.ok) {
        set_error("hifigan_forward: workspace of %lld bytes needed, %lld given", (long long)a.off, (long long)ws_bytes);
        return TTSAMD_ENOMEM;
    }
    const ttsamd_hifigan_cfg& cfg = h->cfg;
    std::unique_lock<std::mutex> lk(h->mu, std::defer_lock);
    hipStream_t bs[3] = {s, s, s};
    if (multi) {
        lk.lock();
        TTS_REQUIRE(h->ev_fork && h->side[0] && h->side[1], "hifigan_forward: the branch streams were not created (hifigan_create)");
        bs[1] = h->side[0];
        bs[2] = h->side[1];
    }

    struct Join {
        bool on; hipStream_t a, b;
        ~Join() { if (on) { (void)hipStreamSynchronize(a); (void)hipStreamSynchronize(b); } }
    } join{false, bs[1], bs[2]};
    const auto fail = [&](int32_t rc) { join.on = multi && rc != 0; return rc; };

    ConvParams p;
    std::memset(&p, 0, sizeof(p));
    p.batch = B;
    p.lens_in = lens; p.lens_out = lens;
    p.n_phase = 1; p.div = 1.f;
    p.splitk_ws = splitks[0]; p.splitk_floats = kSplitKFloats;
    const bool pack_t = default_precision() == 1 && opt_int(OPT_BF16_PACKED_T, 1) != 0;
    const Fused2Switches f2sw = read_fused2_switches();
    const bool fused_ok = default_precision() == 0 && opt_int(OPT_FUSED_PAIR, 1) != 0;
    const bool convt_ok = opt_int(OPT_CONVT, 1) != 0;
    bool in_section = false;
    int pack_io = 0;
    auto conv = [&](const ConvW& cw, const float* x, hipStream_t st, float* y, const float* res, int L, int mul,
                    int dil, float slope, int mode, float div) -> int32_t {
        p.x = x; p.x_bs = (int64_t)cw.cin * L; p.x_cs = L;
        p.w = h->dev + cw.w_off; p.bias = h->dev + cw.b_off;
        p.w_bf16 = h->dev16 + cw.w16_off; p.precision = default_precision();
        p.w_wino = cw.ww_off >= 0 ? h->dev + cw.ww_off : nullptr;
        p.w_wino4 = (cw.ww4_off >= 0 && cw.cout >= 64) ? h->dev + cw.ww4_off : nullptr;
        p.y = y; p.y_bs = (int64_t)cw.cout * L; p.y_cs = L; p.y_ts = 1;
        p.res = res; p.r_bs = (int64_t)cw.cout * L; p.r_cs = L;
        p.len_in_mul = mul; p.len_out_mul = mul; p.Lin = L; p.Nout = L;
        p.Cin = cw.cin; p.Cout = cw.cout; p.CoutP = cout_padded(cw.cout); p.K = cw.k;
        p.dil = dil; p.pad = (cw.k * dil - dil) / 2;
        p.n_phase = 1; p.phase_p = 0;
        p.in_slope = slope; p.relu_out = 0; p.mode = mode; p.div = div;
        p.x_packed = (pack_io & 1) ? 1 : 0; p.y_packed = (pack_io & 2) ? 1 : 0; p.pack_slope = 0.1f;
        if (in_section) prof_add(2.0 * cw.cout * cw.cin * cw.k * mul);
        else prof_begin(st, 2.0 * cw.cout * cw.cin * cw.k * mul);
        const int32_t rc = launch_conv(p, st);
        if (!in_section) prof_end(st);
        return rc;
    };

#define HG_TRY(expr) do { int32_t rc_ = (expr); if (rc_ != 0) return fail(rc_); } while (0)
#define HG_CHECK_HIP(expr) do { hipError_t e_ = (expr); if (e_ != hipSuccess) { set_error("%s failed: %s (%s:%d)", #expr, hipGetErrorString(e_), __FILE__, __LINE__); return fail(TTSAMD_EHIP); } } while (0)
    const int prec = default_precision();
    if ((prec == 1 || prec == 2) && h->bfo_ok && opt_int(OPT_BFO, 1) != 0) {
        const bool x3 = prec == 2;
        const uint16_t* W16 = h->dev16;
        const auto woff = [x3](const ConvW& cw) { return x3 ? cw.wo3_off : cw.wo_off; };
        const auto l_conv = x3 ? bfo3_launch_conv : bfo_launch_conv;
        const auto l_convt = x3 ? bfo3_launch_convt : bfo_launch_convt;
        const auto l_pair = x3 ? bfo3_launch_pair : bfo_launch_pair;
        const auto pair_ok = x3 ? bfo3_pair_supported : bfo_pair_supported;
        const bool chain3_on = opt_int(OPT_BFO_CHAIN, 1) != 0;
        void *curo = cur, *upso = ups_out;
        HG_TRY((x3 ? bfo3_launch_pack : bfo_launch_pack)(mel, B, cfg.num_mels, T, 1.f, mel_o, s));
        BfoConvParams cp;
        std::memset(&cp, 0, sizeof(cp));
        cp.batch = B; cp.lens = lens; cp.div = 1.f; cp.res_slope = 1.f;
        cp.x = mel_o; cp.y = curo; cp.w = W16 + woff(h->conv_pre); cp.bias = h->dev + h->conv_pre.b_off;
        cp.len_mul = 1; cp.Lin = T; cp.Cin = h->conv_pre.cin; cp.Cout = h->conv_pre.cout; cp.K = 7; cp.dil = 1; cp.up = 1;
        cp.mode = 0; cp.out_slope = 0.1f;
        prof_begin(s, 2.0 * cp.Cout * cp.Cin * 7);
        int32_t rc = l_conv(cp, s);
        prof_end(s);
        HG_TRY(rc);
        int L = T, mul = 1;
        for (int i = 0; i < cfg.n_ups; ++i) {
            const int u = cfg.upsample_rates[i];
            const ConvW& uw = h->ups[i];
            cp.x = curo; cp.y = upso; cp.w = W16 + woff(uw); cp.bias = h->dev + uw.b_off; cp.res = nullptr; cp.sum_in = nullptr;
            cp.len_mul = mul; cp.Lin = L; cp.Cin = uw.cin; cp.Cout = uw.cout; cp.K = 2; cp.dil = 1; cp.up = u;
            cp.mode = 0; cp.out_slope = 0.1f;
            prof_begin(s, 2.0 * uw.cout * uw.cin * 2 * u * mul);
            rc = l_convt(cp, s);
            prof_end(s);
            HG_TRY(rc);
            L *= u; mul *= u;
            const float next_slope = i + 1 < cfg.n_ups ? 0.1f : 0.01f;
            if (multi) {
                prof_section_begin(s);
                in_section = true;
                HG_CHECK_HIP(hipEventRecord(h->ev_fork, s));
            }
            for (int j = 0; j < cfg.n_kernels; ++j) {
                hipStream_t st = bs[j % 3];
                void *Tb = Tbs[j % 3], *R = Rs[j % 3];
                if (multi && j > 0) HG_CHECK_HIP(hipStreamWaitEvent(st, h->ev_fork, 0));
                const void* src = upso;
                {
                    const int li0 = (i * cfg.n_kernels + j) * cfg.n_dilations;
                    int32_t dl[3] = {0, 0, 0};
                    for (int m = 0; m < cfg.n_dilations && m < 3; ++m) dl[m] = cfg.resblock_dilations[j][m];
                    const bool chain3 = x3 && chain3_on && bfo3_chain_supported(h->c1[li0].cin, h->c1[li0].k, dl, cfg.n_dilations, L);
                    if (chain3 || (!x3 && bfo_chain_wanted(h->c1[li0].cin, h->c1[li0].k, dl, cfg.n_dilations, L, B))) {
                        BfoChainParams cc;
                        std::memset(&cc, 0, sizeof(cc));
                        cc.x = src; cc.y = curo; cc.sum_in = curo;
                        for (int m = 0; m < 3; ++m) {
                            const ConvW &w1 = h->c1[li0 + m], &w2 = h->c2[li0 + m];
                            cc.w1[m] = W16 + woff(w1); cc.w2[m] = W16 + woff(w2); cc.b1[m] = h->dev + w1.b_off; cc.b2[m] = h->dev + w2.b_off;
                            cc.dil[m] = dl[m];
                        }
                        cc.lens = lens; cc.len_mul = mul; cc.L = L; cc.batch = B; cc.k = h->c1[li0].k;
                        cc.mode = cfg.n_kernels == 1 ? 0 : (j == 0 ? 0 : (j + 1 < cfg.n_kernels ? 1 : 2));
                        cc.div = (float)cfg.n_kernels; cc.in_slope = 0.1f; cc.mid_slope = 0.1f;
                        cc.out_slope = j + 1 == cfg.n_kernels ? next_slope : 1.f;
                        if (multi && j > 0) HG_CHECK_HIP(hipStreamWaitEvent(st, h->ev_done[j - 1], 0));
                        const double fl = 3 * 2.0 * (2.0 * h->c1[li0].cin * h->c1[li0].cin * h->c1[li0].k) * mul;
                        if (in_section) prof_add(fl); else prof_begin(st, fl);
                        rc = x3 ? bfo3_launch_chain(h->c1[li0].cin, cc, st) : bfo_launch_chain(h->c1[li0].cin, cc, st);
                        if (!in_section) prof_end(st);
                        HG_TRY(rc);
                        if (multi) HG_CHECK_HIP(hipEventRecord(h->ev_done[j], st));
                        continue;
                    }
                }
                for (int m = 0; m < cfg.n_dilations; ++m) {
                    const int li = (i * cfg.n_kernels + j) * cfg.n_dilations + m;
                    const int d = cfg.resblock_dilations[j][m];
                    const bool last = m + 1 == cfg.n_dilations;
                    const ConvW &w1 = h->c1[li], &w2 = h->c2[li];
                    void* dst = last ? curo : (src == R ? Tb : R);
                    const int mode = !last || cfg.n_kernels == 1 ? 0 : (j == 0 ? 0 : (j + 1 < cfg.n_kernels ? 1 : 2));
                    const float out_slope = !last ? 0.1f : (j + 1 == cfg.n_kernels ? next_slope : 1.f);
                    if (multi && last && j > 0) HG_CHECK_HIP(hipStreamWaitEvent(st, h->ev_done[j - 1], 0));
                    const double fl = 2.0 * (2.0 * w1.cin * w1.cin * w1.k) * mul;
                    if (pair_ok(w1.cin, w1.k, d, L)) {
                        BfoPairParams pp;
                        std::memset(&pp, 0, sizeof(pp));
                        pp.x = src; pp.y = dst; pp.sum_in = curo;
                        pp.w1 = W16 + woff(w1); pp.w2 = W16 + woff(w2); pp.b1 = h->dev + w1.b_off; pp.b2 = h->dev + w2.b_off;
                        pp.lens = lens; pp.len_mul = mul; pp.L = L; pp.dil = d; pp.batch = B;
                        pp.mode = mode; pp.div = (float)cfg.n_kernels; pp.in_slope = 0.1f; pp.mid_slope = 0.1f; pp.out_slope = out_slope;
                        if (in_section) prof_add(fl); else prof_begin(st, fl);
                        rc = l_pair(w1.cin, w1.k, pp, st);
                        if (!in_section) prof_end(st);
                        HG_TRY(rc);
                    } else {
                        void* t1 = Tb;
                        if (!last) dst = R;
                        cp.x = src; cp.y = t1; cp.w = W16 + woff(w1); cp.bias = h->dev + w1.b_off; cp.res = nullptr; cp.sum_in = nullptr;
                        cp.len_mul = mul; cp.Lin = L; cp.Cin = w1.cin; cp.Cout = w1.cout; cp.K = w1.k; cp.dil = d; cp.up = 1;
                        cp.mode = 0; cp.out_slope = 0.1f; cp.res_slope = 1.f;
                        cp.splitk_ws = splitks[j % 3]; cp.splitk_floats = kSplitKFloats;
                        if (in_section) prof_add(fl); else prof_begin(st, fl);
                        rc = l_conv(cp, st);
                        if (rc == 0) {
                            cp.x = t1; cp.y = dst; cp.w = W16 + woff(w2); cp.bias = h->dev + w2.b_off; cp.res = src; cp.sum_in = curo;
                            cp.dil = 1; cp.mode = mode; cp.div = (float)cfg.n_kernels; cp.out_slope = out_slope; cp.res_slope = 0.1f;
                            rc = l_conv(cp, st);
                        }
                        if (!in_section) prof_end(st);
                        HG_TRY(rc);
                    }
                    if (multi && last) HG_CHECK_HIP(hipEventRecord(h->ev_done[j], st));
                    src = dst;
                }
            }
            if (multi) {
                HG_CHECK_HIP(hipStreamWaitEvent(s, h->ev_done[cfg.n_kernels - 1], 0));
                in_section = false;
                prof_section_end(s);
            }
        }
        HG_TRY((x3 ? bfo3_launch_conv_post : bfo_launch_conv_post)(curo, h->dev + h->conv_post.w_off, h->dev + h->conv_post.b_off, lens, mul, B, h->conv_post.cin,
                                    L, wave, (int64_t)L, s));
        return 0;
    }

    HG_TRY(conv(h->conv_pre, mel, s, cur, nullptr, T, 1, 1, 1.0f, 0, 1.f));
    int L = T, mul = 1;
    for (int i = 0; i < cfg.n_ups; ++i) {
        const int u = cfg.upsample_rates[i], kt = cfg.upsample_kernel_sizes[i];
        const ConvW& uw = h->ups[i];
        p.x = cur; p.x_bs = (int64_t)uw.cin * L; p.x_cs = L;
        p.w = h->dev + uw.w_off; p.bias = h->dev + uw.b_off;
        p.w_bf16 = h->dev16 + uw.w16_off; p.precision = default_precision(); p.w_wino = nullptr; p.w_wino4 = nullptr;
        p.y = ups_out; p.y_bs = (int64_t)uw.cout * L * u; p.y_cs = L * u; p.y_ts = u;
        p.res = nullptr;
        p.len_in_mul = mul; p.len_out_mul = mul; p.Lin = L; p.Nout = L;
        p.Cin = uw.cin; p.Cout = uw.cout; p.CoutP = cout_padded(uw.cout); p.K = 2;
        p.dil = -1; p.pad = 0; p.n_phase = u; p.phase_p = (kt - u) / 2;
        p.in_slope = 0.1f; p.relu_out = 0; p.mode = 0; p.div = 1.f;
        p.x_packed = 0; p.y_packed = 0;
        prof_begin(s, 2.0 * uw.cout * uw.cin * 2 * u * mul);
        int32_t rc = (convt_ok && convt_supported(p)) ? launch_convt(p, s) : launch_conv(p, s);
        prof_end(s);
        HG_TRY(rc);
        L *= u; mul *= u;
        if (multi) {
            prof_section_begin(s);
            in_section = true;
            HG_CHECK_HIP(hipEventRecord(h->ev_fork, s));
        }
        for (int j = 0; j < cfg.n_kernels; ++j) {
            hipStream_t st = bs[j % 3];
            float *Tb = Tbs[j % 3], *R = Rs[j % 3];
            p.splitk_ws = splitks[j % 3];
            if (multi && j > 0) HG_CHECK_HIP(hipStreamWaitEvent(st, h->ev_fork, 0));
            const float* src = ups_out;
            for (int m = 0; m < cfg.n_dilations; ++m) {
                const int li = (i * cfg.n_kernels + j) * cfg.n_dilations + m;
                const int d = cfg.resblock_dilations[j][m];
                {
                    const bool last = m + 1 == cfg.n_dilations;
                    float* dst = last ? cur : (src == R ? Tb : R);
                    const ConvW &w1 = h->c1[li], &w2 = h->c2[li];
                    const bool square = w1.cin == w1.cout && w2.cin == w1.cin && w2.cout == w1.cin && w1.k == w2.k;
                    const int ntw2 = (fused_ok && square) ? fused2_choice(f2sw, w1.cin, w1.k, d, L, src, dst, (int64_t)B * L) : 0;
                    const bool f43 = ntw2 == 2 && f2sw.pair4 && f2sw.wino_a && w1.k >= kPair4MinK && w1.ww4_off >= 0 && w2.ww4_off >= 0 &&
                                     fused_pair4_supported(w1.cin, w1.k, d, L, src, dst);
                    if (ntw2 != 0 || (fused_ok && square && fused_pair_supported(w1.cin, w1.k, d, L, src, dst))) {
                        const int mode = !last ? 0 : (cfg.n_kernels == 1 ? 0 : (j == 0 ? 0 : (j + 1 < cfg.n_kernels ? 1 : 2)));
                        if (multi && last && j > 0) HG_CHECK_HIP(hipStreamWaitEvent(st, h->ev_done[j - 1], 0));
                        const double fl = 2.0 * (2.0 * w1.cin * w1.cin * w1.k) * mul;
                        if (in_section) prof_add(fl); else prof_begin(st, fl);
                        const int32_t frc = f43
                            ? launch_fused_pair4(w1.cin, src, dst, h->dev + w1.ww4_off, h->dev + w1.b_off, h->dev + w2.ww4_off,
                                                 h->dev + w2.b_off, w1.k, d, lens, mul, L, B, mode, (float)cfg.n_kernels, 0.1f, st)
                            : ntw2 != 0
                            ? launch_fused_pair2(w1.cin, src, dst, h->dev + w1.w_off, h->dev + w1.b_off, h->dev + w2.w_off,
                                                 h->dev + w2.b_off, w1.k, d, lens, mul, L, B, mode, (float)cfg.n_kernels, 0.1f, ntw2, st,
                                                 (f2sw.wino_b && w2.ww_off >= 0) ? h->dev + w2.ww_off : nullptr,
                                                 (f2sw.wino_a && w1.ww_off >= 0) ? h->dev + w1.ww_off : nullptr)
                            : launch_fused_pair(w1.cin, src, dst, h->dev + w1.w_off, h->dev + w1.b_off, h->dev + w2.w_off,
                                                h->dev + w2.b_off, w1.k, d, lens, mul, L, B, mode, (float)cfg.n_kernels, 0.1f, st);
                        if (!in_section) prof_end(st);
                        HG_TRY(frc);
                        if (multi && last) HG_CHECK_HIP(hipEventRecord(h->ev_done[j], st));
                        src = dst;
                        continue;
                    }
                }
                pack_io = pack_t ? 2 : 0;
                HG_TRY(conv(h->c1[li], src, st, Tb, nullptr, L, mul, d, 0.1f, 0, 1.f));
                pack_io = pack_t ? 1 : 0;
                if (m + 1 < cfg.n_dilations) {
                    HG_TRY(conv(h->c2[li], Tb, st, R, src, L, mul, 1, 0.1f, 0, 1.f));
                    pack_io = 0;
                    src = R;
                } else {
                    const int mode = (j == 0) ? 0 : (j + 1 < cfg.n_kernels ? 1 : 2);
                    const int md = cfg.n_kernels == 1 ? 0 : mode;
                    if (multi && j > 0) HG_CHECK_HIP(hipStreamWaitEvent(st, h->ev_done[j - 1], 0));
                    HG_TRY(conv(h->c2[li], Tb, st, cur, src, L, mul, 1, 0.1f, md, (float)cfg.n_kernels));
                    pack_io = 0;
                    if (multi) HG_CHECK_HIP(hipEventRecord(h->ev_done[j], st));
                }
            }
        }
        p.splitk_ws = splitks[0];
        if (multi) {
            HG_CHECK_HIP(hipStreamWaitEvent(s, h->ev_done[cfg.n_kernels - 1], 0));
            in_section = false;
            prof_section_end(s);
        }
    }
    HG_TRY(launch_conv_post(cur, (int64_t)h->conv_post.cin * L, L, h->dev + h->conv_post.w_off,
                             h->dev + h->conv_post.b_off, lens, mul, B, h->conv_post.cin, L, 0.01f, wave,
                             (int64_t)L, s));
#undef HG_TRY
#undef HG_CHECK_HIP
    return 0;
}

void hifigan_blobs(const void* hv, void** f32, int64_t* n_f32, void** b16, int64_t* n_b16) {
    const HifiGan* h = (const HifiGan*)hv;
    *f32 = h->dev; *n_f32 = h->dev_n; *b16 = h->dev16; *n_b16 = h->dev16_n;
}

}
```

### tts-arabic-pytorch_amd/csrc/resblock_fused2.hip

```cpp
#include <algorithm>
#include <cstdlib>
#include <cstring>

#include "conv_mfma_common.hpp"

namespace ttsamd {

struct FusedPair2Params {
    const float* x;
    float* y;
    const float4* w1;
    const float4* w2;
    const float4* w1w;
    const float4* w2w;
    const float* b1;
    const float* b2;
    const int64_t* lens;
    int32_t len_mul, L, dil, batch;
    int32_t mode;
    float div, slope;
    int32_t compact;
};

template <int K, int C, int NTW>
struct Fused2Geo {
    static constexpr int NOCT = C / 8, MT = C / 32;
    static constexpr int H = (K - 1) / 2;
    static constexpr int NB = 128 * NTW;
    static constexpr int TS = (NB - 2 * H) & ~3;
    static constexpr int TSTR = NB + K - 1;
    static constexpr int NG = NOCT * K;
    static constexpr int NS = K / 3, NL = K - 3 * NS, NGW = 4 * NS + 2 * NL;
    static constexpr int TSH = TSTR / 2;
    static constexpr int PF = 2;
    static constexpr int MPO = 4 * MT * NTW * K;
    static constexpr int UO = NOCT * MPO <= 640 ? NOCT : (4 * MPO <= 640 ? 4 : 2);
    static_assert(NOCT % UO == 0 && (UO * K) % PF == 0, "unrolled body of the group loop");
    static constexpr int WAVES = (C == 128 && NTW == 2) ? 1 : (C == 32 ? 4 : 2);
    __host__ __device__ static constexpr int npa(int d) { return d * (128 / d); }
    __host__ __device__ static constexpr int ts_wa(int d) { return (2 * npa(d) - 2 * H) & ~3; }
    static size_t lds_bytes(int dil) { return (size_t)2 * NOCT * (NB + (K - 1) * dil) * sizeof(float4); }
};

__device__ __forceinline__ float lrelu_max(const float v, const float slope) {
    return __builtin_amdgcn_fmed3f(v, v * slope, __builtin_inff());
}

template <int K, int C, int NTW, bool ACT>
__device__ __forceinline__ void conv_phase2(f32x16 (&acc)[C / 32][NTW], float4 (&aq)[2][C / 32], const float4* sb, const int bstr,
                                            const int bdil, const float4* __restrict__ wl, const float4* __restrict__ wnext,
                                            const float slope) {
    using G = Fused2Geo<K, C, NTW>;
    constexpr int NOCT = G::NOCT, MT = G::MT, NG = G::NG, PF = G::PF, UO = G::UO, GB = UO * K;
    float4 bq[NTW];
#pragma unroll
    for (int j = 0; j < NTW; ++j) bq[j] = sb[32 * j];
#pragma unroll 1
    for (int ob = 0; ob < NOCT; ob += UO) {
        const float4* sbo = sb + ob * 2 * bstr;
        const int g0 = ob * K;
#pragma unroll
        for (int gl = 0; gl < GB; ++gl) {
            float4 a4[MT], b4[NTW];
#pragma unroll
            for (int mt = 0; mt < MT; ++mt) a4[mt] = aq[gl % PF][mt];
#pragma unroll
            for (int j = 0; j < NTW; ++j) b4[j] = bq[j];
            {
                const int gn = g0 + gl + PF;
                const float4* __restrict__ src = gn < NG ? wl + (int64_t)gn * 2 * C : wnext + (int64_t)(gn - NG) * 2 * C;
#pragma unroll
                for (int mt = 0; mt < MT; ++mt) aq[gl % PF][mt] = src[32 * mt];
            }
            {
                const int o1 = (gl + 1) / K, t1 = (gl + 1) % K;
                const float4* nb = (gl + 1 < GB) ? sbo + o1 * 2 * bstr + t1 * bdil
                                                 : sb + min(ob + UO, NOCT - 1) * 2 * bstr;
#pragma unroll
                for (int j = 0; j < NTW; ++j) bq[j] = nb[32 * j];
            }
            __builtin_amdgcn_sched_barrier(0);
            float bv[NTW][4];
#pragma unroll
            for (int j = 0; j < NTW; ++j) {
                bv[j][0] = b4[j].x; bv[j][1] = b4[j].y; bv[j][2] = b4[j].z; bv[j][3] = b4[j].w;
                if (ACT) {
#pragma unroll
                    for (int pq = 0; pq < 4; ++pq) bv[j][pq] = lrelu_max(bv[j][pq], slope);
                }
            }
#pragma unroll
            for (int pq = 0; pq < 4; ++pq)
#pragma unroll
                for (int mt = 0; mt < MT; ++mt) {
                    const float av = pq == 0 ? a4[mt].x : (pq == 1 ? a4[mt].y : (pq == 2 ? a4[mt].z : a4[mt].w));
#pragma unroll
                    for (int j = 0; j < NTW; ++j)
                        acc[mt][j] = __builtin_amdgcn_mfma_f32_32x32x2f32(av, bv[j][pq], acc[mt][j], 0, 0, 0);
                }
        }
    }
}

template <int K, int C, bool EO, int MTW>
__device__ __forceinline__ void conv_phase2_wino(f32x16 (&acc)[4][MTW], float4 (&aq)[2][MTW], const float4* sb,
                                                 const float4* __restrict__ wl, const int rstride, const int cstep,
                                                 const float4* __restrict__ wnext) {
    using G = Fused2Geo<K, C, 2>;
    constexpr int NOCT = G::NOCT, MT = MTW, PF = G::PF, NS = G::NS, NL = G::NL, NGW = G::NGW, TSH = G::TSH;
    constexpr int NBU = NS + NL;
    constexpr int NGT = NOCT * NGW;
    typedef float f32x4v __attribute__((ext_vector_type(4)));
#define TTS_ENT(SBO, CC) (SBO)[EO ? ((CC) & 1) * TSH + ((CC) >> 1) : (CC) * cstep]
    float4 bq[2][4];
#pragma unroll
    for (int m = 0; m < 4; ++m) bq[0][m] = TTS_ENT(sb, m);
#pragma unroll 1
    for (int o = 0; o < NOCT; ++o) {
        const float4* sbo = sb + o * 2 * rstride;
        const float4* sbn = sb + min(o + 1, NOCT - 1) * 2 * rstride;
#pragma unroll
        for (int u = 0; u < NBU; ++u) {
            const int cur = u & 1, nxt = cur ^ 1;
            {
                const int un = u + 1;
                if (un < NS) {
#pragma unroll
                    for (int m = 0; m < 4; ++m) bq[nxt][m] = TTS_ENT(sbo, 3 * un + m);
                } else if (un < NBU) {
                    bq[nxt][0] = TTS_ENT(sbo, 3 * NS + (un - NS));
                    bq[nxt][1] = TTS_ENT(sbo, 3 * NS + (un - NS) + 1);
                } else {
#pragma unroll
                    for (int m = 0; m < 4; ++m) bq[nxt][m] = TTS_ENT(sbn, m);
                }
            }
            f32x4v x[4], v[4];
#pragma unroll
            for (int m = 0; m < 4; ++m) x[m] = f32x4v{bq[cur][m].x, bq[cur][m].y, bq[cur][m].z, bq[cur][m].w};
            const bool sub = u < NS;
            if (sub) { v[0] = x[0] - x[2]; v[1] = x[1] + x[2]; v[2] = x[2] - x[1]; v[3] = x[1] - x[3]; }
            else { v[0] = x[0]; v[1] = x[1]; }
            const int ng = sub ? 4 : 2;
            const int g0 = sub ? 4 * u : 4 * NS + 2 * (u - NS);
#pragma unroll
            for (int i = 0; i < ng; ++i) {
                const int g = g0 + i;
                const int plane = sub ? i : (i ? 3 : 0);
                const int slot = g % PF;
                float4 a4[MT];
#pragma unroll
                for (int mt = 0; mt < MT; ++mt) a4[mt] = aq[slot][mt];
                {
                    const int gn = o * NGW + g + PF;
                    const float4* __restrict__ src = gn < NGT ? wl + (int64_t)gn * 2 * C
                                                              : (wnext ? wnext + (int64_t)(gn - NGT) * 2 * C : wl + (int64_t)(NGT - 1) * 2 * C);
#pragma unroll
                    for (int mt = 0; mt < MT; ++mt) aq[slot][mt] = src[32 * mt];
                }
                __builtin_amdgcn_sched_barrier(0);
#pragma unroll
                for (int pq = 0; pq < 4; ++pq)
#pragma unroll
                    for (int mt = 0; mt < MT; ++mt) {
                        const float av = pq == 0 ? a4[mt].x : (pq == 1 ? a4[mt].y : (pq == 2 ? a4[mt].z : a4[mt].w));
                        acc[plane][mt] = __builtin_amdgcn_mfma_f32_32x32x2f32(av, v[i][pq], acc[plane][mt], 0, 0, 0);
                    }
            }
        }
        if (NBU & 1) {
#pragma unroll
            for (int m = 0; m < 4; ++m) bq[0][m] = bq[1][m];
        }
    }
#undef TTS_ENT
}

constexpr int kF2Wa32Waves = 3;
template <int C, int WM>
constexpr int f2_row_halves() { return (WM == 2 && C == 128) ? 2 : 1; }

template <int K, int C, int NTW, int WM>
__global__ __launch_bounds__((256 * f2_row_halves<C, WM>()), ((WM == 2 && C == 32) ? kF2Wa32Waves : Fused2Geo<K, C, NTW>::WAVES))
void resblock_pair2(const FusedPair2Params p) {
    using G = Fused2Geo<K, C, NTW>;
    constexpr int NOCT = G::NOCT, MT = G::MT, H = G::H, NB = G::NB, TSTR = G::TSTR, PF = G::PF, TSH = G::TSH;
    constexpr bool WB = WM >= 1, WA = WM == 2;
    constexpr int RH = f2_row_halves<C, WM>(), MTW = MT / RH, NTH = 256 * RH;
    static_assert(!WB || NTW == 2, "Winograd phase B: a wave's 64 columns are its 32 output pairs");
    const int TS = WA ? G::ts_wa(p.dil) : G::TS;
    extern __shared__ __attribute__((aligned(16))) float4 smem4[];
    const int tid = threadIdx.x, lane = tid & 63, wid = tid >> 6;
    const int kk = lane >> 5, l31 = lane & 31;
    const int cg = wid & 3, mt0 = RH == 2 ? MTW * (wid >> 2) : 0;
    int b = blockIdx.z;
    int q0 = blockIdx.x * TS;
    if (p.compact) {
        int tile = 0;
        if (!live_tile(p.lens, p.len_mul, p.L, TS, p.batch, blockIdx.z * gridDim.x + blockIdx.x, b, tile)) return;
        b = __builtin_amdgcn_readfirstlane(b);
        q0 = __builtin_amdgcn_readfirstlane(tile) * TS;
    }
    int len = p.L;
    if (p.lens) len = min(len, (int)p.lens[b] * p.len_mul);
    if (q0 >= len) return;
    const int dil = p.dil, L = p.L;
    const int pad1 = H * dil;
    const int W1 = NB + (K - 1) * dil;
    const int x0 = q0 - H - pad1;
    const float slope = p.slope;
    const float* __restrict__ xb = p.x + (int64_t)b * C * L;
    float4* Xs = smem4;

    const float4* __restrict__ wl1 = (WA ? p.w1w : p.w1) + kk * C + l31 + 32 * mt0;
    const float4* __restrict__ wl2 = (WB ? p.w2w : p.w2) + kk * C + l31 + 32 * mt0;
    float4 aq[PF][MTW];
#pragma unroll
    for (int g = 0; g < PF; ++g)
#pragma unroll
        for (int mt = 0; mt < MTW; ++mt) aq[g][mt] = wl1[g * 2 * C + 32 * mt];

    {
        constexpr int NE = (2 * NOCT * (NB + (K - 1) * DMAX) + NTH - 1) / NTH;
        const int n_ent = 2 * NOCT * W1;
        float v[NE][4];
        int eo[NE];
        bool ok[NE];
        int okk = 0, col = tid;
        while (col >= W1) { col -= W1; ++okk; }
#pragma unroll
        for (int u = 0; u < NE; ++u) {
            const int pos = x0 + col;
            const int okc = min(okk, 2 * NOCT - 1);
            ok[u] = pos >= 0 && pos < len;
            eo[u] = tid + NTH * u < n_ent ? okc * W1 + col : -1;
            const float* src = xb + (int64_t)((okc >> 1) * 8 + (okc & 1)) * L + min(max(pos, 0), max(len - 1, 0));
#pragma unroll
            for (int pc = 0; pc < 4; ++pc) v[u][pc] = src[(int64_t)2 * pc * L];
            col += NTH;
            while (col >= W1) { col -= W1; ++okk; }
        }
#pragma unroll
        for (int u = 0; u < NE; ++u)
            if (eo[u] >= 0) {
                if (WA) {
#pragma unroll
                    for (int pc = 0; pc < 4; ++pc) v[u][pc] = lrelu_max(v[u][pc], slope);
                }
                Xs[eo[u]] = ok[u] ? make_float4(v[u][0], v[u][1], v[u][2], v[u][3]) : make_float4(0.f, 0.f, 0.f, 0.f);
            }
    }
    __syncthreads();

    float* ep = reinterpret_cast<float*>(smem4);
    if constexpr (WA) {
        const int jw = cg * 32 + l31;
        const int npa = G::npa(dil);
        const int pa = min(jw, npa - 1);
        const int na = dil == 1 ? 2 * pa : (pa / dil) * 2 * dil + pa % dil;
        {
            f32x16 accA[4][MTW];
#pragma unroll
            for (int mt = 0; mt < MTW; ++mt)
#pragma unroll
                for (int r = 0; r < 16; ++r) {
                    const float bv = p.b1[32 * (mt0 + mt) + (r & 3) + 8 * (r >> 2) + 4 * kk];
                    accA[0][mt][r] = bv; accA[1][mt][r] = 0.f; accA[2][mt][r] = 0.f; accA[3][mt][r] = -bv;
                }
            conv_phase2_wino<K, C, false, MTW>(accA, aq, Xs + kk * W1 + na, wl1, W1, dil, wl2);
            __syncthreads();
            if (jw < npa) {
#pragma unroll
                for (int hh = 0; hh < 2; ++hh) {
                    const int col = na + hh * dil;
                    const int pos = q0 - H + col;
                    const bool live = pos >= 0 && pos < len;
                    const int ent = (col & 1) * TSH + (col >> 1);
#pragma unroll
                    for (int mt = 0; mt < MTW; ++mt)
#pragma unroll
                        for (int oc = 0; oc < 4; ++oc)
#pragma unroll
                            for (int k2 = 0; k2 < 2; ++k2) {
                                const int r = 4 * oc + k2;
                                float v0 = hh ? accA[1][mt][r] - accA[2][mt][r] - accA[3][mt][r] : accA[0][mt][r] + accA[1][mt][r] + accA[2][mt][r];
                                float v1 = hh ? accA[1][mt][r + 2] - accA[2][mt][r + 2] - accA[3][mt][r + 2]
                                              : accA[0][mt][r + 2] + accA[1][mt][r + 2] + accA[2][mt][r + 2];
                                v0 = lrelu_max(v0, slope);
                                v1 = lrelu_max(v1, slope);
                                const float2 w2v = live ? make_float2(v0, v1) : make_float2(0.f, 0.f);
                                *reinterpret_cast<float2*>(reinterpret_cast<float*>(Xs + ((4 * (mt0 + mt) + oc) * 2 + k2) * 2 * TSH + ent) + 2 * kk) = w2v;
                            }
                }
            }
            __syncthreads();
        }
        f32x16 accw[4][MTW];
#pragma unroll
        for (int g = 0; g < 4; ++g)
#pragma unroll
            for (int mt = 0; mt < MTW; ++mt)
#pragma unroll
                for (int r = 0; r < 16; ++r) accw[g][mt][r] = 0.f;
        if (p.mode != 0) {
            const int n = 2 * jw, q = q0 + n;
            const int voff = ((n < TS && q < len) ? q : 0) * 4 + 4 * kk * L * 4;
            const auto ys = __builtin_amdgcn_make_buffer_rsrc(p.y + (int64_t)b * C * L, 0, C * L * 4, 0x00020000);
#pragma unroll
            for (int mt = 0; mt < MTW; ++mt)
#pragma unroll
                for (int r = 0; r < 16; ++r) {
                    const int so = (32 * (mt0 + mt) + (r & 3) + 8 * (r >> 2)) * L * 4;
                    accw[0][mt][r] = __builtin_bit_cast(float, __builtin_amdgcn_raw_buffer_load_b32(ys, voff, so, 0));
                    accw[3][mt][r] = -__builtin_bit_cast(float, __builtin_amdgcn_raw_buffer_load_b32(ys, voff + 4, so, 0));
                }
        }
        conv_phase2_wino<K, C, true, MTW>(accw, aq, Xs + kk * 2 * TSH + jw, wl2, 2 * TSH, 0, nullptr);
        __syncthreads();
#pragma unroll
        for (int mt = 0; mt < MTW; ++mt)
#pragma unroll
            for (int r = 0; r < 16; ++r) {
                float2 y2;
                y2.x = accw[0][mt][r] + accw[1][mt][r] + accw[2][mt][r];
                y2.y = accw[1][mt][r] - accw[2][mt][r] - accw[3][mt][r];
                *reinterpret_cast<float2*>(ep + (32 * (mt0 + mt) + (r & 3) + 8 * (r >> 2) + 4 * kk) * NB + 2 * jw) = y2;
            }
    } else {
    const int colw = wid * 32 * NTW + l31;
    f32x16 acc[MT][NTW];
#pragma unroll
    for (int mt = 0; mt < MT; ++mt)
#pragma unroll
        for (int r = 0; r < 16; ++r) {
            const float bv = p.b1[32 * mt + (r & 3) + 8 * (r >> 2) + 4 * kk];
#pragma unroll
            for (int j = 0; j < NTW; ++j) acc[mt][j][r] = bv;
        }

    conv_phase2<K, C, NTW, true>(acc, aq, Xs + kk * W1 + colw, W1, dil, wl1, wl2, slope);

    if constexpr (WB) {
        const int jw = wid * 32 + l31;
        f32x16 accw[4][MT];
#pragma unroll
        for (int mt = 0; mt < MT; ++mt) {
            const int colx = 2 * jw + H + pad1;
#pragma unroll
            for (int r = 0; r < 16; ++r) { accw[1][mt][r] = 0.f; accw[2][mt][r] = 0.f; }
#pragma unroll
            for (int oc = 0; oc < 4; ++oc)
#pragma unroll
                for (int k2 = 0; k2 < 2; ++k2) {
                    const float* src = reinterpret_cast<const float*>(Xs + ((4 * mt + oc) * 2 + k2) * W1 + colx) + 2 * kk;
                    const float2 r0 = *reinterpret_cast<const float2*>(src);
                    const float2 r1 = *reinterpret_cast<const float2*>(src + 4);
                    accw[0][mt][4 * oc + k2] = r0.x;
                    accw[0][mt][4 * oc + k2 + 2] = r0.y;
                    accw[3][mt][4 * oc + k2] = -r1.x;
                    accw[3][mt][4 * oc + k2 + 2] = -r1.y;
                }
        }
        if (p.mode != 0) {
            const int n = 2 * jw, q = q0 + n;
            const int voff = ((n < TS && q < len) ? q : 0) * 4 + 4 * kk * L * 4;
            const auto ys = __builtin_amdgcn_make_buffer_rsrc(p.y + (int64_t)b * C * L, 0, C * L * 4, 0x00020000);
#pragma unroll
            for (int mt = 0; mt < MT; ++mt) {
                f32x16 t0, t1;
#pragma unroll
                for (int r = 0; r < 16; ++r) {
                    const int so = (32 * mt + (r & 3) + 8 * (r >> 2)) * L * 4;
                    t0[r] = __builtin_bit_cast(float, __builtin_amdgcn_raw_buffer_load_b32(ys, voff, so, 0));
                    t1[r] = __builtin_bit_cast(float, __builtin_amdgcn_raw_buffer_load_b32(ys, voff + 4, so, 0));
                }
#pragma unroll
                for (int r = 0; r < 16; ++r) {
                    accw[0][mt][r] = t0[r] + accw[0][mt][r];
                    accw[3][mt][r] = accw[3][mt][r] - t1[r];
                }
            }
        }
        __syncthreads();

#pragma unroll
        for (int j = 0; j < NTW; ++j) {
            const int col = wid * 32 * NTW + l31 + 32 * j;
            const int pos = q0 - H + col;
            const bool live = pos >= 0 && pos < len;
            const int ent = (col & 1) * TSH + (col >> 1);
#pragma unroll
            for (int mt = 0; mt < MT; ++mt)
#pragma unroll
                for (int oc = 0; oc < 4; ++oc)
#pragma unroll
                    for (int k2 = 0; k2 < 2; ++k2) {
                        const int r = 4 * oc + k2;
                        float v0 = acc[mt][j][r], v1 = acc[mt][j][r + 2];
                        v0 = lrelu_max(v0, slope);
                        v1 = lrelu_max(v1, slope);
                        const float2 w2v = live ? make_float2(v0, v1) : make_float2(0.f, 0.f);
                        *reinterpret_cast<float2*>(reinterpret_cast<float*>(Xs + ((4 * mt + oc) * 2 + k2) * 2 * TSH + ent) + 2 * kk) = w2v;
                    }
        }
        __syncthreads();

        conv_phase2_wino<K, C, true, MT>(accw, aq, Xs + kk * 2 * TSH + jw, wl2, 2 * TSH, 0, nullptr);

        __syncthreads();
#pragma unroll
        for (int mt = 0; mt < MT; ++mt)
#pragma unroll
            for (int r = 0; r < 16; ++r) {
                float2 y2;
                y2.x = accw[0][mt][r] + accw[1][mt][r] + accw[2][mt][r];
                y2.y = accw[1][mt][r] - accw[2][mt][r] - accw[3][mt][r];
                *reinterpret_cast<float2*>(ep + (32 * mt + (r & 3) + 8 * (r >> 2) + 4 * kk) * NB + 2 * jw) = y2;
            }
    } else {
    f32x16 acc2[MT][NTW];
#pragma unroll
    for (int mt = 0; mt < MT; ++mt)
#pragma unroll
        for (int j = 0; j < NTW; ++j) {
            const int colx = colw + 32 * j + H + pad1;
#pragma unroll
            for (int oc = 0; oc < 4; ++oc)
#pragma unroll
                for (int k2 = 0; k2 < 2; ++k2) {
                    const float2 rv = *reinterpret_cast<const float2*>(
                        reinterpret_cast<const float*>(Xs + ((4 * mt + oc) * 2 + k2) * W1 + colx) + 2 * kk);
                    acc2[mt][j][4 * oc + k2] = rv.x;
                    acc2[mt][j][4 * oc + k2 + 2] = rv.y;
                }
        }
    if (p.mode != 0) {
        int voff[NTW];
#pragma unroll
        for (int j = 0; j < NTW; ++j) {
            const int n = colw + 32 * j;
            const int q = q0 + n;
            voff[j] = ((n < TS && q < len) ? q : 0) * 4 + 4 * kk * L * 4;
        }
        const auto ys = __builtin_amdgcn_make_buffer_rsrc(p.y + (int64_t)b * C * L, 0, C * L * 4, 0x00020000);
#pragma unroll
        for (int mt = 0; mt < MT; ++mt)
#pragma unroll
            for (int j = 0; j < NTW; ++j) {
                f32x16 t;
#pragma unroll
                for (int r = 0; r < 16; ++r)
                    t[r] = __builtin_bit_cast(float, __builtin_amdgcn_raw_buffer_load_b32(
                        ys, voff[j], (32 * mt + (r & 3) + 8 * (r >> 2)) * L * 4, 0));
#pragma unroll
                for (int r = 0; r < 16; ++r) acc2[mt][j][r] = t[r] + acc2[mt][j][r];
            }
    }
    __syncthreads();

#pragma unroll
    for (int j = 0; j < NTW; ++j) {
        const int col = colw + 32 * j;
        const int pos = q0 - H + col;
        const bool live = pos >= 0 && pos < len;
#pragma unroll
        for (int mt = 0; mt < MT; ++mt)
#pragma unroll
            for (int oc = 0; oc < 4; ++oc)
#pragma unroll
                for (int k2 = 0; k2 < 2; ++k2) {
                    const int r = 4 * oc + k2;
                    float v0 = acc[mt][j][r], v1 = acc[mt][j][r + 2];
                    v0 = lrelu_max(v0, slope);
                    v1 = lrelu_max(v1, slope);
                    const float2 w2v = live ? make_float2(v0, v1) : make_float2(0.f, 0.f);
                    *reinterpret_cast<float2*>(reinterpret_cast<float*>(Xs + ((4 * mt + oc) * 2 + k2) * TSTR + col) + 2 * kk) = w2v;
                }
    }
    __syncthreads();

    conv_phase2<K, C, NTW, false>(acc2, aq, Xs + kk * TSTR + colw, TSTR, 1, wl2, wl2, slope);

    __syncthreads();
#pragma unroll
    for (int mt = 0; mt < MT; ++mt)
#pragma unroll
        for (int j = 0; j < NTW; ++j)
#pragma unroll
            for (int r = 0; r < 16; ++r) ep[(32 * mt + (r & 3) + 8 * (r >> 2) + 4 * kk) * NB + colw + 32 * j] = acc2[mt][j][r];
    }
    }
    __syncthreads();
    const bool do_div = p.mode == 2;
    const float div = p.div;
    float* __restrict__ yb = p.y + (int64_t)b * C * L;
    constexpr int LPR = NB / 4;
    constexpr int RPW = 64 / LPR;
    const int n = (lane % LPR) * 4;
    const int rsub = lane / LPR;
    const int wid_u = __builtin_amdgcn_readfirstlane(wid);
#pragma unroll 4
    for (int it = 0; it < C / (4 * RH * RPW); ++it) {
        const int ch = (wid_u + 4 * RH * it) * RPW + rsub;
        const float bs = p.b2[ch];
        const int q = q0 + n;
        if (n >= TS || q >= len) continue;
        const float4 v4 = *reinterpret_cast<const float4*>(ep + ch * NB + n);
        float vv[4] = {v4.x + bs, v4.y + bs, v4.z + bs, v4.w + bs};
        if (WA) {
            const float* xp = xb + (int64_t)ch * L + q;
            if (q + 3 < len) {
                const float4 x4 = *reinterpret_cast<const float4*>(xp);
                vv[0] += x4.x; vv[1] += x4.y; vv[2] += x4.z; vv[3] += x4.w;
            } else {
#pragma unroll
                for (int e = 0; e < 4; ++e)
                    if (q + e < len) vv[e] += xp[e];
            }
        }
        if (do_div) {
#pragma unroll
            for (int e = 0; e < 4; ++e) vv[e] = vv[e] / div;
        }
        float* yp = yb + (int64_t)ch * L + q;
        if (q + 3 < len) {
            *reinterpret_cast<float4*>(yp) = make_float4(vv[0], vv[1], vv[2], vv[3]);
        } else {
#pragma unroll
            for (int e = 0; e < 4; ++e)
                if (q + e < len) yp[e] = vv[e];
        }
    }
}


template <int K, int C, int NTW, int WM>
static int32_t launch_fused2_k(const FusedPair2Params& p, hipStream_t stream) {
    using G = Fused2Geo<K, C, NTW>;
    static std::atomic<uint64_t> lds_done{0};
    TTS_CHECK_HIP(lds_opt_in((const void*)resblock_pair2<K, C, NTW, WM>, (int)G::lds_bytes(DMAX), lds_done));
    const int ts = WM == 2 ? G::ts_wa(p.dil) : G::TS;
    dim3 grid((p.L + ts - 1) / ts, 1, p.batch);
    hipLaunchKernelGGL((resblock_pair2<K, C, NTW, WM>), grid, dim3(256 * f2_row_halves<C, WM>()), G::lds_bytes(p.dil), stream, p);
    TTS_CHECK_HIP(hipGetLastError());
    return 0;
}

bool fused_pair2_supported(int32_t channels, int32_t k, int32_t dil, int32_t L, const float* x, const float* y, int32_t ntw) {
    if (!(channels == 32 || channels == 64 || channels == 128) || !(k == 3 || k == 7 || k == 11) || !(ntw == 1 || ntw == 2)) return false;
    if (dil < 1 || dil > DMAX || (L & 3) != 0 || ((((uintptr_t)x) | ((uintptr_t)y)) & 15) != 0 || x == y) return false;
    if ((int64_t)channels * L * 4 >= ((int64_t)1 << 31)) return false;
    const size_t lds = (size_t)2 * (channels / 8) * (128 * ntw + (k - 1) * dil) * 16;
    return lds <= 160 * 1024;
}

int32_t launch_fused_pair2(int32_t channels, const float* x, float* y, const float* w1, const float* b1, const float* w2,
                           const float* b2, int32_t k, int32_t dil, const int64_t* lens, int32_t len_mul, int32_t L, int32_t batch,
                           int32_t mode, float div, float slope, int32_t ntw, hipStream_t stream, const float* w2_wino,
                           const float* w1_wino) {
    TTS_REQUIRE(fused_pair2_supported(channels, k, dil, L, x, y, ntw),
                "fused ResBlock pair (direct weights): unsupported geometry (C=%d, k=%d, dil=%d, L=%d, ntw=%d)", channels, k, dil, L, ntw);
    TTS_REQUIRE(slope > 0.f && slope <= 1.f, "fused ResBlock pair: leaky-relu slope %g outside (0, 1]", (double)slope);
    const bool wa = w2_wino != nullptr && w1_wino != nullptr && ntw == 2 && (dil == 1 || dil == 3 || dil == 5);
    const bool wb = w2_wino != nullptr && ntw == 2 && (channels <= 64 || wa);
    conv_log(wa ? "fused_pair2ww" : wb ? "fused_pair2w" : (ntw == 2 ? "fused_pair2" : "fused_pair2n"), k, channels, channels, L, batch, 1, mode, len_mul, lens != nullptr, 1);
    FusedPair2Params p;
    std::memset(&p, 0, sizeof(p));
    p.x = x; p.y = y;
    p.w1 = reinterpret_cast<const float4*>(w1); p.w2 = reinterpret_cast<const float4*>(w2);
    p.w2w = reinterpret_cast<const float4*>(w2_wino);
    p.w1w = reinterpret_cast<const float4*>(w1_wino);
    p.b1 = b1; p.b2 = b2; p.lens = lens; p.len_mul = len_mul; p.L = L; p.dil = dil; p.batch = batch;
    p.mode = mode; p.div = div; p.slope = slope;
    p.compact = compact_order(lens, batch) ? 1 : 0;
#define TTS_F2W(KK, CC) if (wa && k == KK && channels == CC) return launch_fused2_k<KK, CC, 2, 2>(p, stream); \
                        if (wb && k == KK && channels == CC) return launch_fused2_k<KK, CC, 2, 1>(p, stream);
    TTS_F2W(3, 32) TTS_F2W(7, 32) TTS_F2W(11, 32) TTS_F2W(3, 64) TTS_F2W(7, 64) TTS_F2W(11, 64)
#undef TTS_F2W
    if (wa && channels == 128) {
        if (k == 3) return launch_fused2_k<3, 128, 2, 2>(p, stream);
        if (k == 7) return launch_fused2_k<7, 128, 2, 2>(p, stream);
        if (k == 11) return launch_fused2_k<11, 128, 2, 2>(p, stream);
    }
#define TTS_F2(KK, CC, NN) if (k == KK && channels == CC && ntw == NN) return launch_fused2_k<KK, CC, NN, 0>(p, stream);
    TTS_F2(3, 32, 2) TTS_F2(7, 32, 2) TTS_F2(11, 32, 2)
    TTS_F2(3, 64, 2) TTS_F2(7, 64, 2) TTS_F2(11, 64, 2)
    TTS_F2(3, 128, 2) TTS_F2(7, 128, 2) TTS_F2(11, 128, 2)
    TTS_F2(3, 32, 1) TTS_F2(7, 32, 1) TTS_F2(11, 32, 1)
    TTS_F2(3, 64, 1) TTS_F2(7, 64, 1) TTS_F2(11, 64, 1)
    TTS_F2(3, 128, 1) TTS_F2(7, 128, 1) TTS_F2(11, 128, 1)
#undef TTS_F2
    set_error("fused ResBlock pair (direct weights): no instantiation for C=%d, k=%d, ntw=%d", channels, k, ntw);
    return TTSAMD_EINVAL;
}

}
```

### tts-arabic-pytorch_amd/ttsamd/engine.py

```python
import ctypes as C

import numpy as np
import torch

from . import lib as L
from .config import NET_CONFIG, HIFIGAN_CONFIG, VOCOS_22K_CONFIG, TACOTRON2_CONFIG


def _require_gpu():
    if not torch.cuda.is_available():
        raise L.TtsAmdError('no ROCm device visible: the ttsamd engines run only on an MI355X (gfx950); '
                            'there is no CPU fallback')
    lib = L.load()
    if not lib.ttsamd_device_ok():
        raise L.TtsAmdError('device 0 is not gfx950')
    return lib


PRECISIONS = {'f32': 0, 'bf16': 1, 'bf16x3': 2}


def set_precision(name):
    lib = L.load()
    L.check(lib.ttsamd_set_precision(PRECISIONS[name]), 'set_precision')


def get_precision():
    code = L.load().ttsamd_get_precision()
    return {v: k for k, v in PRECISIONS.items()}[code]


def _ptr(t):
    return C.c_void_p(t.data_ptr()) if t is not None else C.c_void_p(0)


def _stream():
    return C.c_void_p(torch.cuda.current_stream().cuda_stream)


def _f32(t, device):
    if t is None:
        return None
    if not isinstance(t, torch.Tensor):
        t = torch.as_tensor(np.asarray(t))
    return t.to(device=device, dtype=torch.float32).contiguous()


def _check_ids(t, n, what):
    if isinstance(t, torch.Tensor) and t.device.type == 'cpu' and t.numel():
        lo, hi = int(t.min()), int(t.max())
        if lo < 0 or hi >= n:
            raise IndexError(f'{what}: index out of range [0, {n}) (got min {lo}, max {hi})')


class _Workspace:
    def __init__(self):
        self.buf = None

    def get(self, nbytes, device):
        if self.buf is None or self.buf.numel() < nbytes or self.buf.device != device:
            self.buf = torch.empty(int(nbytes), dtype=torch.uint8, device=device)
        return self.buf


class HifiGanEngine:

    def __init__(self, state_dict, config=None, device='cuda'):
        self.lib = _require_gpu()
        self.device = torch.device(device if device != 'cuda' else 'cuda:0')
        h = dict(HIFIGAN_CONFIG if config is None else config)
        if str(h.get('resblock', '1')) != '1':
            raise L.TtsAmdError('only ResBlock1 generators are built (config.json:2)')
        cfg = L.HifiGanCfg()
        cfg.num_mels = h.get('num_mels', 80)
        cfg.upsample_initial_channel = h['upsample_initial_channel']
        cfg.n_ups = len(h['upsample_rates'])
        for i, (u, k) in enumerate(zip(h['upsample_rates'], h['upsample_kernel_sizes'])):
            cfg.upsample_rates[i], cfg.upsample_kernel_sizes[i] = u, k
        cfg.n_kernels = len(h['resblock_kernel_sizes'])
        cfg.n_dilations = len(h['resblock_dilation_sizes'][0])
        for j, (k, ds) in enumerate(zip(h['resblock_kernel_sizes'], h['resblock_dilation_sizes'])):
            cfg.resblock_kernel_sizes[j] = k
            for m, d in enumerate(ds):
                cfg.resblock_dilations[j][m] = d
        self.hop = int(np.prod(h['upsample_rates']))
        self.num_mels = cfg.num_mels
        arr, keep = L.make_tensors(state_dict)
        handle = C.c_void_p()
        with torch.cuda.device(self.device):
            L.check(self.lib.ttsamd_hifigan_create(arr, len(arr), C.byref(cfg), C.byref(handle)), 'hifigan_create')
        self.handle = handle
        self.ws = _Workspace()

    def __del__(self):
        if getattr(self, 'handle', None):
            self.lib.ttsamd_hifigan_destroy(self.handle)
            self.handle = None

    def forward(self, mel, lens=None):
        mel = _f32(mel, self.device)
        B, M, T = mel.shape
        assert M == self.num_mels
        if lens is not None:
            lens = lens.to(device=self.device, dtype=torch.int64).contiguous()
        wave = torch.zeros(B, self.hop * T, dtype=torch.float32, device=self.device)
        if T == 0:
            return wave
        with torch.cuda.device(self.device):
            nbytes = self.lib.ttsamd_hifigan_workspace_bytes(self.handle, B, T)
            ws = self.ws.get(nbytes, self.device)
            L.check(self.lib.ttsamd_hifigan_forward(self.handle, _ptr(mel), _ptr(lens), B, T, _ptr(wave), _ptr(ws),
                                                    nbytes, _stream()), 'hifigan_forward')
        return wave


class FastPitchEngine:

    def __init__(self, state_dict, config=None, device='cuda'):
        self.lib = _require_gpu()
        self.device = torch.device(device if device != 'cuda' else 'cuda:0')
        c = dict(NET_CONFIG if config is None else config)
        self.config = c
        cfg = L.FastPitchCfg()
        cfg.n_mel_channels, cfg.n_symbols, cfg.padding_idx = c['n_mel_channels'], c['n_symbols'], c['padding_idx']
        cfg.d_model = c['symbols_embedding_dim']
        cfg.in_fft_n_layers, cfg.in_fft_n_heads, cfg.in_fft_d_head = c['in_fft_n_layers'], c['in_fft_n_heads'], c['in_fft_d_head']
        cfg.in_fft_kernel, cfg.in_fft_filter = c['in_fft_conv1d_kernel_size'], c['in_fft_conv1d_filter_size']
        cfg.out_fft_n_layers, cfg.out_fft_n_heads, cfg.out_fft_d_head = c['out_fft_n_layers'], c['out_fft_n_heads'], c['out_fft_d_head']
        cfg.out_fft_kernel, cfg.out_fft_filter = c['out_fft_conv1d_kernel_size'], c['out_fft_conv1d_filter_size']
        cfg.dur_kernel, cfg.dur_filter, cfg.dur_n_layers = c['dur_predictor_kernel_size'], c['dur_predictor_filter_size'], c['dur_predictor_n_layers']
        cfg.pitch_kernel, cfg.pitch_filter, cfg.pitch_n_layers = c['pitch_predictor_kernel_size'], c['pitch_predictor_filter_size'], c['pitch_predictor_n_layers']
        cfg.pitch_emb_kernel = c['pitch_embedding_kernel_size']
        cfg.energy_conditioning = int(bool(c['energy_conditioning']))
        cfg.energy_kernel, cfg.energy_filter, cfg.energy_n_layers = c['energy_predictor_kernel_size'], c['energy_predictor_filter_size'], c['energy_predictor_n_layers']
        cfg.energy_emb_kernel = c['energy_embedding_kernel_size']
        cfg.n_speakers, cfg.speaker_emb_weight = c['n_speakers'], float(c['speaker_emb_weight'])
        assert c.get('pitch_conditioning_formants', 1) == 1
        self.d_model, self.n_mel = cfg.d_model, cfg.n_mel_channels
        arr, keep = L.make_tensors(state_dict)
        handle = C.c_void_p()
        with torch.cuda.device(self.device):
            L.check(self.lib.ttsamd_fastpitch_create(arr, len(arr), C.byref(cfg), C.byref(handle)), 'fastpitch_create')
        self.handle = handle
        self.ws = _Workspace()
        self._alone = False
        self._pad_ok = all(int(c[k]) == 3 for k in ('in_fft_conv1d_kernel_size', 'out_fft_conv1d_kernel_size', 'dur_predictor_kernel_size',
                                                    'pitch_predictor_kernel_size')) and \
            (not c['energy_conditioning'] or int(c['energy_predictor_kernel_size']) == 3)

    def __del__(self):
        if getattr(self, 'handle', None):
            self.lib.ttsamd_fastpitch_destroy(self.handle)
            self.handle = None

    def infer(self, ids, pace=1.0, dur_tgt=None, pitch_tgt=None, energy_tgt=None, pitch_mul=1.0, pitch_add=0.0,
              max_duration=75, speaker=0, return_idx=False, lens_hook=None, alone=False):
        if bool(alone) != self._alone:
            L.check(self.lib.ttsamd_fastpitch_set_batch_mode(self.handle, int(bool(alone))), 'fastpitch_set_batch_mode')
            self._alone = bool(alone)
        dev = self.device
        ids = torch.as_tensor(ids).to(device=dev, dtype=torch.int64).contiguous()
        B, Lt0 = ids.shape
        d = self.d_model
        dur_tgt, pitch_tgt, energy_tgt = _f32(dur_tgt, dev), _f32(pitch_tgt, dev), _f32(energy_tgt, dev)
        pad = B >= 2 and self._pad_ok and get_precision() != 'bf16'
        Lt = Lt0
        enc = torch.empty(B, d, Lt, dtype=torch.float32, device=dev)
        dur_pred = torch.empty(B, Lt, dtype=torch.float32, device=dev)
        pitch_pred = torch.empty(B, 1, Lt, dtype=torch.float32, device=dev)
        energy_pred = torch.empty(B, Lt, dtype=torch.float32, device=dev) if self.config['energy_conditioning'] else None
        reps = torch.empty(B, Lt, dtype=torch.int64, device=dev)
        dec_lens = torch.empty(B, dtype=torch.int64, device=dev)
        lib = self.lib
        with torch.cuda.device(dev):
            nb = lib.ttsamd_fastpitch_encode_workspace_bytes(self.handle, B, Lt)
            ws = self.ws.get(nb, dev)
            L.check(lib.ttsamd_fastpitch_encode(self.handle, _ptr(ids), B, Lt, int(speaker), float(pace), _ptr(dur_tgt),
                                                _ptr(pitch_tgt), _ptr(energy_tgt), float(pitch_mul), float(pitch_add),
                                                float(max_duration), _ptr(enc), _ptr(dur_pred), _ptr(pitch_pred),
                                                _ptr(energy_pred), _ptr(reps), _ptr(dec_lens), _ptr(ws), nb, _stream()),
                    'fastpitch_encode')
            if lens_hook is None:
                t_max0 = int(dec_lens.max().item())
            else:
                t_max0 = int(max(lens_hook(dec_lens), default=0))
            t_max = (t_max0 + 3) & ~3 if pad else t_max0
            x = torch.empty(B, d, t_max, dtype=torch.float32, device=dev)
            idx = torch.empty(B, t_max, dtype=torch.int32, device=dev) if return_idx else None
            mel = torch.empty(B, self.n_mel, t_max, dtype=torch.float32, device=dev)
            if t_max > 0:
                L.check(lib.ttsamd_length_regulate(_ptr(enc), _ptr(reps), B, Lt, d, t_max, _ptr(x), _ptr(idx), _stream()),
                        'length_regulate')
                nb = lib.ttsamd_fastpitch_decode_workspace_bytes(self.handle, B, t_max)
                ws = self.ws.get(nb, dev)
                L.check(lib.ttsamd_fastpitch_decode(self.handle, _ptr(x), _ptr(dec_lens), B, t_max, _ptr(mel), _ptr(ws), nb,
                                                    _stream()), 'fastpitch_decode')
        if t_max != t_max0:
            mel = mel[:, :, :t_max0]
            idx = None if idx is None else idx[:, :t_max0]
        out = (mel, dec_lens, dur_pred, pitch_pred, energy_pred)
        return out + (idx,) if return_idx else out


class DenoiserEngine:

    def __init__(self, device='cuda'):
        self.lib = _require_gpu()
        self.device = torch.device(device if device != 'cuda' else 'cuda:0')
        handle = C.c_void_p()
        with torch.cuda.device(self.device):
            L.check(self.lib.ttsamd_denoiser_create(C.byref(handle)), 'denoiser_create')
        self.handle = handle
        self.ws = _Workspace()

    def __del__(self):
        if getattr(self, 'handle', None):
            self.lib.ttsamd_denoiser_destroy(self.handle)
            self.handle = None

    def bias_spec(self, audio):
        audio = _f32(audio, self.device).reshape(-1)
        n = audio.numel()
        out = torch.empty(513, dtype=torch.float32, device=self.device)
        n_dev = torch.tensor([n], dtype=torch.int64, device=self.device)
        with torch.cuda.device(self.device):
            nb = self.lib.ttsamd_denoiser_workspace_bytes(1, n)
            ws = self.ws.get(nb, self.device)
            L.check(self.lib.ttsamd_denoiser_bias_spec(self.handle, _ptr(audio), _ptr(n_dev), n, _ptr(out), _ptr(ws), nb,
                                                       _stream()), 'denoiser_bias_spec')
        return out.reshape(1, 513, 1)

    def denoise(self, wave, nsamples, bias_spec, strength):
        assert wave.is_contiguous() and wave.dtype == torch.float32
        B, n_max = wave.shape
        nsamples = nsamples.to(device=self.device, dtype=torch.int64).contiguous()
        bias = _f32(bias_spec, self.device).reshape(-1)
        with torch.cuda.device(self.device):
            nb = self.lib.ttsamd_denoiser_workspace_bytes(B, n_max)
            ws = self.ws.get(nb, self.device)
            L.check(self.lib.ttsamd_denoise(self.handle, _ptr(wave), n_max, _ptr(nsamples), B, n_max, _ptr(bias),
                                            float(strength), _ptr(ws), nb, _stream()), 'denoise')
        return wave


class VocosEngine:

    def __init__(self, state_dict, config=None, device='cuda'):
        self.lib = _require_gpu()
        self.device = torch.device(device if device != 'cuda' else 'cuda:0')
        c = dict(VOCOS_22K_CONFIG if config is None else config)
        assert c['n_fft'] == 1024 and c['hop_length'] == 256 and c['padding'] == 'same'
        self.hop, self.n_mels = c['hop_length'], c['input_channels']
        arr, keep = L.make_tensors(state_dict)
        handle = C.c_void_p()
        with torch.cuda.device(self.device):
            L.check(self.lib.ttsamd_vocos_create(arr, len(arr), c['input_channels'], c['dim'], c['intermediate_dim'],
                                                 c['num_layers'], C.byref(handle)), 'vocos_create')
        self.handle = handle
        self.ws = _Workspace()
        self._bias = None

    def __del__(self):
        if getattr(self, 'handle', None):
            self.lib.ttsamd_vocos_destroy(self.handle)
            self.handle = None

    def bias_vec(self):
        if self._bias is None:
            out = torch.empty(513, dtype=torch.float32, device=self.device)
            with torch.cuda.device(self.device):
                nb = self.lib.ttsamd_vocos_workspace_bytes(self.handle, 1, 88)
                ws = self.ws.get(nb, self.device)
                L.check(self.lib.ttsamd_vocos_bias_vec(self.handle, _ptr(out), _ptr(ws), nb, _stream()), 'vocos_bias_vec')
            self._bias = out.reshape(1, 513, 1)
        return self._bias

    def forward(self, mel, lens=None, denoise=0.0):
        mel = _f32(mel, self.device)
        B, M, T0 = mel.shape
        assert M == self.n_mels
        if lens is None:
            lens = torch.full((B,), T0, dtype=torch.int64, device=self.device)
        lens = lens.to(device=self.device, dtype=torch.int64).contiguous()
        if T0 == 0:
            return torch.zeros(B, 0, dtype=torch.float32, device=self.device)
        T = (T0 + 3) & ~3
        if T != T0:
            mel = torch.nn.functional.pad(mel, (0, T - T0))
        wave = torch.zeros(B, self.hop * T, dtype=torch.float32, device=self.device)
        bias = self.bias_vec().reshape(-1) if denoise != 0 else None
        with torch.cuda.device(self.device):
            nb = self.lib.ttsamd_vocos_workspace_bytes(self.handle, B, T)
            ws = self.ws.get(nb, self.device)
            L.check(self.lib.ttsamd_vocos_forward(self.handle, _ptr(mel), _ptr(lens), B, T, float(denoise), _ptr(bias),
                                                  _ptr(wave), _ptr(ws), nb, _stream()), 'vocos_forward')
        return wave if T == T0 else wave[:, :self.hop * T0]


class Tacotron2Engine:

    def __init__(self, state_dict, config=None, device='cuda'):
        self.lib = _require_gpu()
        self.device = torch.device(device if device != 'cuda' else 'cuda:0')
        c = dict(TACOTRON2_CONFIG if config is None else config)
        self.config = c
        cfg = L.Tacotron2Cfg()
        for name, _ in L.Tacotron2Cfg._fields_:
            setattr(cfg, name, int(bool(c.get(name, True))) if name == 'decoder_early_stopping' else c[name])
        arr, keep = L.make_tensors(state_dict)
        handle = C.c_void_p()
        with torch.cuda.device(self.device):
            L.check(self.lib.ttsamd_tacotron2_create(arr, len(arr), C.byref(cfg), C.byref(handle)), 'tacotron2_create')
        self.handle = handle
        self.ws = _Workspace()
        self.n_mels = c['n_mels']
        self.max_decoder_steps = c.get('decoder_max_step', 2000)

    def __del__(self):
        if getattr(self, 'handle', None):
            self.lib.ttsamd_tacotron2_destroy(self.handle)
            self.handle = None

    def infer(self, tokens, speaker_ids=None, lengths=None, max_step=None, dropout_seed=-1):
        _check_ids(tokens, self.config['n_symbol'], 'Tacotron2 tokens')
        if speaker_ids is not None and self.config['num_speakers'] > 1:
            _check_ids(speaker_ids, self.config['num_speakers'], 'Tacotron2 speaker_ids')
        tokens = tokens.to(device=self.device, dtype=torch.int64).contiguous()
        B, Ltok = tokens.shape
        if lengths is None:
            lengths = torch.full((B,), Ltok, dtype=torch.int64)
        lengths = lengths.to(device=self.device, dtype=torch.int64).contiguous()
        if self.config['num_speakers'] > 1:
            if speaker_ids is None:
                speaker_ids = torch.zeros(B, dtype=torch.int64)
            speaker_ids = speaker_ids.to(device=self.device, dtype=torch.int64).contiguous()
        else:
            speaker_ids = None
        max_step = int(self.max_decoder_steps if max_step is None else max_step)
        if dropout_seed is None:
            dropout_seed = int(torch.randint(0, 2 ** 31 - 1, (1,)).item())
        mel_post = torch.zeros(B, self.n_mels, max_step, dtype=torch.float32, device=self.device)
        mel_raw = torch.zeros(B, self.n_mels, max_step, dtype=torch.float32, device=self.device)
        mel_lens = torch.zeros(B, dtype=torch.int32, device=self.device)
        align = torch.zeros(B, max_step, Ltok, dtype=torch.float32, device=self.device)
        n_steps = C.c_int32(0)
        with torch.cuda.device(self.device):
            nb = self.lib.ttsamd_tacotron2_workspace_bytes(self.handle, B, Ltok, max_step)
            ws = self.ws.get(nb, self.device)
            L.check(self.lib.ttsamd_tacotron2_infer(self.handle, _ptr(tokens), _ptr(lengths), _ptr(speaker_ids), B, Ltok,
                                                    max_step, int(dropout_seed), _ptr(mel_post), _ptr(mel_lens),
                                                    _ptr(align), _ptr(mel_raw), C.byref(n_steps), _ptr(ws), nb,
                                                    _stream()), 'tacotron2_infer')
        T = n_steps.value
        return mel_post[:, :, :T], mel_lens, align[:, :T]


class TaggerEngine:

    RENAME = {'emb0.weight': 'emb.weight', 'emb_input.weight': 'emb.weight'}

    def __init__(self, state_dict, config, device='cuda'):
        self.lib = _require_gpu()
        self.device = torch.device(device if device != 'cuda' else 'cuda:0')
        c = dict(config)
        cfg = L.TaggerCfg()
        cfg.n_vocab, cfg.emb_dim = c['n_vocab'], c['emb_dim']
        cfg.n_lstm, cfg.n_dense = len(c['lstm_hidden']), len(c['dense_dim'])
        for i, v in enumerate(c['lstm_hidden']):
            cfg.lstm_hidden[i] = v
        for i, v in enumerate(c['dense_dim']):
            cfg.dense_dim[i] = v
        cfg.hard_sigmoid, cfg.bn_after_lstm0, cfg.bn_eps = c['hard_sigmoid'], c['bn_after_lstm0'], c['bn_eps']
        self.n_classes = c['dense_dim'][-1]
        self.n_vocab = c['n_vocab']
        arr, keep = L.make_tensors({self.RENAME.get(k, k): v for k, v in state_dict.items()})
        handle = C.c_void_p()
        with torch.cuda.device(self.device):
            L.check(self.lib.ttsamd_tagger_create(arr, len(arr), C.byref(cfg), C.byref(handle)), 'tagger_create')
        self.handle = handle
        self.ws = _Workspace()

    def __del__(self):
        if getattr(self, 'handle', None):
            self.lib.ttsamd_tagger_destroy(self.handle)
            self.handle = None

    def forward(self, ids):
        ids = torch.as_tensor(ids)
        _check_ids(ids, self.n_vocab, 'tagger ids')
        ids = ids.to(device=self.device, dtype=torch.int64).contiguous()
        B, T = ids.shape
        probs = torch.empty(B, T, self.n_classes, dtype=torch.float32, device=self.device)
        if T == 0:
            return probs
        with torch.cuda.device(self.device):
            nb = self.lib.ttsamd_tagger_workspace_bytes(self.handle, B, T)
            ws = self.ws.get(nb, self.device)
            L.check(self.lib.ttsamd_tagger_forward(self.handle, _ptr(ids), B, T, _ptr(probs), _ptr(ws), nb, _stream()),
                    'tagger_forward')
        return probs


def conv1d(x, w, bias=None, lens=None, dilation=1, in_slope=1.0, relu_out=False, res=None, mode=0, div=1.0, y=None):
    lib = _require_gpu()
    x = x.contiguous().float()
    w = w.contiguous().float()
    B, cin, lin = x.shape
    cout, cin2, k = w.shape
    assert cin == cin2
    if y is None:
        y = torch.zeros(B, cout, lin, dtype=torch.float32, device=x.device)
    packed = torch.empty(lib.ttsamd_conv1d_packed_floats(cout, cin, k), dtype=torch.float32, device=x.device)
    with torch.cuda.device(x.device):
        L.check(lib.ttsamd_conv1d_ex(_ptr(x), _ptr(w), _ptr(bias), _ptr(res), _ptr(lens), B, cin, cout, k, dilation, lin,
                                     float(in_slope), int(relu_out), int(mode), float(div), _ptr(y), _ptr(packed), _stream()), 'conv1d')
    return y


def resblock_pair(x, w1, b1, w2, b2, dil, lens=None, len_mul=1, y=None, mode=0, div=1.0, slope=0.1, variant=2):
    lib = _require_gpu()
    x = x.contiguous().float()
    w1, w2, b1, b2 = (t.contiguous().float() for t in (w1, w2, b1, b2))
    B, Cc, Lx = x.shape
    k = w1.shape[2]
    assert tuple(w1.shape) == tuple(w2.shape) == (Cc, Cc, k)
    if y is None:
        assert mode == 0
        y = torch.zeros_like(x)
    if lens is not None:
        lens = lens.to(device=x.device, dtype=torch.int64).contiguous()
    n_packed = int(lib.ttsamd_resblock_pair_packed_floats(Cc, k, int(variant)))
    packed = torch.empty(max(n_packed, 1), dtype=torch.float32, device=x.device)
    with torch.cuda.device(x.device):
        L.check(lib.ttsamd_resblock_pair(_ptr(x), _ptr(y), _ptr(w1), _ptr(b1), _ptr(w2), _ptr(b2), Cc, k, int(dil), _ptr(lens),
                                         int(len_mul), Lx, B, int(mode), float(div), float(slope), int(variant), _ptr(packed),
                                         n_packed, _stream()), 'resblock_pair')
    return y


def length_regulate(enc, reps, t_max):
    lib = _require_gpu()
    enc = enc.contiguous().float()
    reps = reps.contiguous().to(torch.int64)
    B, Cc, Lt = enc.shape
    out = torch.empty(B, Cc, t_max, dtype=torch.float32, device=enc.device)
    idx = torch.empty(B, t_max, dtype=torch.int32, device=enc.device)
    with torch.cuda.device(enc.device):
        L.check(lib.ttsamd_length_regulate(_ptr(enc), _ptr(reps), B, Lt, Cc, t_max, _ptr(out), _ptr(idx), _stream()),
                'length_regulate')
    return out, idx
```

### tts-arabic-pytorch_amd/ttsamd/lib.py

```python
import ctypes as C
import os

_HERE = os.path.dirname(os.path.abspath(__file__))
LIB_PATH = os.environ.get('TTSAMD_LIB') or os.path.join(_HERE, 'lib', 'libttsamd.so')


class TtsAmdError(RuntimeError):
    pass


class Tensor(C.Structure):
    _fields_ = [('name', C.c_char_p), ('data', C.POINTER(C.c_float)), ('ndim', C.c_int32),
                ('shape', C.c_int64 * 4)]


class HifiGanCfg(C.Structure):
    _fields_ = [('num_mels', C.c_int32), ('upsample_initial_channel', C.c_int32), ('n_ups', C.c_int32),
                ('upsample_rates', C.c_int32 * 8), ('upsample_kernel_sizes', C.c_int32 * 8),
                ('n_kernels', C.c_int32), ('resblock_kernel_sizes', C.c_int32 * 8),
                ('n_dilations', C.c_int32), ('resblock_dilations', (C.c_int32 * 8) * 8)]


class FastPitchCfg(C.Structure):
    _fields_ = [(n, C.c_int32) for n in (
        'n_mel_channels', 'n_symbols', 'padding_idx', 'd_model',
        'in_fft_n_layers', 'in_fft_n_heads', 'in_fft_d_head', 'in_fft_kernel', 'in_fft_filter',
        'out_fft_n_layers', 'out_fft_n_heads', 'out_fft_d_head', 'out_fft_kernel', 'out_fft_filter',
        'dur_kernel', 'dur_filter', 'dur_n_layers',
        'pitch_kernel', 'pitch_filter', 'pitch_n_layers', 'pitch_emb_kernel',
        'energy_conditioning', 'energy_kernel', 'energy_filter', 'energy_n_layers', 'energy_emb_kernel',
        'n_speakers')] + [('speaker_emb_weight', C.c_float)]


class Tacotron2Cfg(C.Structure):
    _fields_ = [(n, C.c_int32) for n in (
        'n_symbol', 'num_speakers', 'speaker_embedding_dim', 'symbol_embedding_dim', 'encoder_embedding_dim',
        'encoder_n_convolution', 'encoder_kernel_size', 'n_mels', 'prenet_dim', 'attention_rnn_dim',
        'decoder_rnn_dim', 'attention_hidden_dim', 'attention_location_n_filter',
        'attention_location_kernel_size', 'postnet_n_convolution', 'postnet_kernel_size',
        'postnet_embedding_dim')] + [('gate_threshold', C.c_float), ('decoder_early_stopping', C.c_int32)]


class TaggerCfg(C.Structure):
    _fields_ = [('n_vocab', C.c_int32), ('emb_dim', C.c_int32), ('n_lstm', C.c_int32), ('lstm_hidden', C.c_int32 * 4),
                ('hard_sigmoid', C.c_int32), ('bn_after_lstm0', C.c_int32), ('bn_eps', C.c_float),
                ('n_dense', C.c_int32), ('dense_dim', C.c_int32 * 4)]


_P, _I32, _I64, _F = C.c_void_p, C.c_int32, C.c_int64, C.c_float
SYMBOLS = {
    'ttsamd_last_error': (C.c_char_p, []),
    'ttsamd_version': (_I32, []),
    'ttsamd_set_option': (_I32, [C.c_char_p, C.c_char_p]),
    'ttsamd_get_option': (_I32, [C.c_char_p, C.c_char_p, _I32]),
    'ttsamd_option_name': (C.c_char_p, [_I32]),
    'ttsamd_options_check': (_I32, []),
    'ttsamd_device_ok': (_I32, []),
    'ttsamd_hifigan_create': (_I32, [C.POINTER(Tensor), _I32, C.POINTER(HifiGanCfg), C.POINTER(_P)]),
    'ttsamd_hifigan_destroy': (_I32, [_P]),
    'ttsamd_hifigan_workspace_bytes': (_I64, [_P, _I32, _I32]),
    'ttsamd_hifigan_forward': (_I32, [_P, _P, _P, _I32, _I32, _P, _P, _I64, _P]),
    'ttsamd_fastpitch_create': (_I32, [C.POINTER(Tensor), _I32, C.POINTER(FastPitchCfg), C.POINTER(_P)]),
    'ttsamd_fastpitch_destroy': (_I32, [_P]),
    'ttsamd_fastpitch_encode_workspace_bytes': (_I64, [_P, _I32, _I32]),
    'ttsamd_fastpitch_decode_workspace_bytes': (_I64, [_P, _I32, _I32]),
    'ttsamd_fastpitch_encode': (_I32, [_P, _P, _I32, _I32, _I32, _F, _P, _P, _P, _F, _F, _F,
                                       _P, _P, _P, _P, _P, _P, _P, _I64, _P]),
    'ttsamd_length_regulate': (_I32, [_P, _P, _I32, _I32, _I32, _I32, _P, _P, _P]),
    'ttsamd_fastpitch_decode': (_I32, [_P, _P, _P, _I32, _I32, _P, _P, _I64, _P]),
    'ttsamd_fastpitch_set_batch_mode': (_I32, [_P, _I32]),
    'ttsamd_denoiser_create': (_I32, [C.POINTER(_P)]),
    'ttsamd_denoiser_destroy': (_I32, [_P]),
    'ttsamd_denoiser_workspace_bytes': (_I64, [_I32, _I32]),
    'ttsamd_denoiser_bias_spec': (_I32, [_P, _P, _P, _I32, _P, _P, _I64, _P]),
    'ttsamd_denoise': (_I32, [_P, _P, _I64, _P, _I32, _I32, _P, _F, _P, _I64, _P]),
    'ttsamd_vocos_create': (_I32, [C.POINTER(Tensor), _I32, _I32, _I32, _I32, _I32, C.POINTER(_P)]),
    'ttsamd_vocos_destroy': (_I32, [_P]),
    'ttsamd_vocos_workspace_bytes': (_I64, [_P, _I32, _I32]),
    'ttsamd_vocos_bias_vec': (_I32, [_P, _P, _P, _I64, _P]),
    'ttsamd_vocos_forward': (_I32, [_P, _P, _P, _I32, _I32, _F, _P, _P, _P, _I64, _P]),
    'ttsamd_tacotron2_create': (_I32, [C.POINTER(Tensor), _I32, C.POINTER(Tacotron2Cfg), C.POINTER(_P)]),
    'ttsamd_tacotron2_destroy': (_I32, [_P]),
    'ttsamd_tacotron2_workspace_bytes': (_I64, [_P, _I32, _I32, _I32]),
    'ttsamd_tacotron2_infer': (_I32, [_P, _P, _P, _P, _I32, _I32, _I32, _I64, _P, _P, _P, _P,
                                      C.POINTER(_I32), _P, _I64, _P]),
    'ttsamd_tagger_create': (_I32, [C.POINTER(Tensor), _I32, C.POINTER(TaggerCfg), C.POINTER(_P)]),
    'ttsamd_tagger_destroy': (_I32, [_P]),
    'ttsamd_tagger_workspace_bytes': (_I64, [_P, _I32, _I32]),
    'ttsamd_tagger_forward': (_I32, [_P, _P, _I32, _I32, _P, _P, _I64, _P]),
    'ttsamd_conv1d_packed_floats': (_I64, [_I32, _I32, _I32]),
    'ttsamd_conv1d': (_I32, [_P, _P, _P, _P, _I32, _I32, _I32, _I32, _I32, _I32, _F, _I32, _P, _P, _P]),
    'ttsamd_conv1d_ex': (_I32, [_P, _P, _P, _P, _P, _I32, _I32, _I32, _I32, _I32, _I32, _F, _I32, _I32, _F, _P, _P, _P]),
    'ttsamd_resblock_pair_packed_floats': (_I64, [_I32, _I32, _I32]),
    'ttsamd_resblock_pair': (_I32, [_P, _P, _P, _P, _P, _P, _I32, _I32, _I32, _P, _I32, _I32, _I32, _I32, _F, _F, _I32, _P, _I64, _P]),
    'ttsamd_bfo_pack': (_I32, [_P, _I32, _I32, _I32, _F, _P, _P]),
    'ttsamd_bfo_unpack': (_I32, [_P, _I32, _I32, _I32, _F, _P, _P]),
    'ttsamd_bfo_weight_elems': (_I64, [_I32, _I32, _I32, _I32]),
    'ttsamd_bfo_pack_weight': (_I32, [_P, _I32, _I32, _I32, _I32, _P]),
    'ttsamd_bfo_conv1d': (_I32, [_P, _P, _P, _P, _P, _P, _I32, _I32, _I32, _I32, _I32, _I32, _I32, _I32, _I32, _F, _F, _F, _P, _P, _P, _P]),
    'ttsamd_bfo_resblock_pair': (_I32, [_P, _P, _P, _P, _P, _P, _P, _I32, _I32, _I32, _I32, _I32, _I32, _I32, _F, _F, _F, _F, _P, _P]),
    'ttsamd_bfo_resblock_chain': (_I32, [_P, _P, _P, _P, _P, _P, _P, _P, _I32, _I32, _I32, _I32, _I32, _F, _F, _F, _F, _P, _P, _I32]),
    'ttsamd_bfo_conv_post': (_I32, [_P, _P, _P, _P, _I32, _I32, _I32, _I32, _P, _I64, _P]),
    'ttsamd_bfo3_pack': (_I32, [_P, _I32, _I32, _I32, _F, _P, _P]),
    'ttsamd_bfo3_unpack': (_I32, [_P, _I32, _I32, _I32, _F, _P, _P]),
    'ttsamd_bfo3_weight_elems': (_I64, [_I32, _I32, _I32, _I32]),
    'ttsamd_bfo3_pack_weight': (_I32, [_P, _I32, _I32, _I32, _I32, _P]),
    'ttsamd_bfo3_conv1d': (_I32, [_P, _P, _P, _P, _P, _P, _I32, _I32, _I32, _I32, _I32, _I32, _I32, _I32, _I32, _F, _F, _F, _P, _P, _P, _P]),
    'ttsamd_bfo3_resblock_pair': (_I32, [_P, _P, _P, _P, _P, _P, _P, _I32, _I32, _I32, _I32, _I32, _I32, _I32, _F, _F, _F, _F, _P, _P]),
    'ttsamd_bfo3_resblock_chain': (_I32, [_P, _P, _P, _P, _P, _P, _P, _P, _I32, _I32, _I32, _I32, _I32, _F, _F, _F, _F, _P, _P]),
    'ttsamd_bfo3_conv_post': (_I32, [_P, _P, _P, _P, _I32, _I32, _I32, _I32, _P, _I64, _P]),
    'ttsamd_set_precision': (_I32, [_I32]),
    'ttsamd_get_precision': (_I32, []),
    'ttsamd_dp_unique_id': (_I32, [_P]),
    'ttsamd_dp_init': (_I32, [_I32, _I32, _P, C.POINTER(_P)]),
    'ttsamd_dp_destroy': (_I32, [_P]),
    'ttsamd_dp_rank': (_I32, [_P]),
    'ttsamd_dp_world': (_I32, [_P]),
    'ttsamd_dp_broadcast': (_I32, [_P, _P, _I64, _I32, _P]),
    'ttsamd_dp_broadcast_weights': (_I32, [_P, _I32, _P, _I32, _P]),
    'ttsamd_dp_allgather': (_I32, [_P, _P, _P, _I64, _P]),
    'ttsamd_dp_pack_audio': (_I32, [_P, _I64, _P, _I32, _I64, _P, _P]),
    'ttsamd_dp_gather_audio': (_I32, [_P, _P, _P, C.POINTER(_I64), C.POINTER(_I64), _I32, _P]),
    'ttsamd_profile_enable': (_I32, [_I32]),
    'ttsamd_profile_read': (_I32, [C.POINTER(C.c_double)]),
}

_lib = None
ABI_VERSION = 7


def load():
    global _lib
    if _lib is not None:
        return _lib
    if not os.path.exists(LIB_PATH):
        raise TtsAmdError(f'{LIB_PATH} is missing: build it with `make -C tts-arabic-pytorch_amd/csrc` '
                          '(hipcc --offload-arch=gfx950); there is no CPU/PyTorch fallback')
    import torch
    lib = C.CDLL(LIB_PATH)
    for name, (res, args) in SYMBOLS.items():
        fn = getattr(lib, name)
        fn.restype, fn.argtypes = res, args
    got = lib.ttsamd_version()
    if got != ABI_VERSION:
        raise TtsAmdError(f'{LIB_PATH} was built from another revision of include/ttsamd.h (library ABI {got}, this binding '
                          f'{ABI_VERSION}): rebuild it with `make -C tts-arabic-pytorch_amd/csrc`')
    if lib.ttsamd_options_check() != 0:
        msg = lib.ttsamd_last_error()
        raise TtsAmdError(f'bad routing option in the environment: {msg.decode() if msg else "?"}')
    _lib = lib
    return lib


def set_option(name, value):
    v = None if value is None else str(value).encode()
    check(load().ttsamd_set_option(name.encode(), v), f'set_option({name}={value})')


def get_option(name):
    buf = C.create_string_buffer(64)
    check(load().ttsamd_get_option(name.encode(), buf, 64), f'get_option({name})')
    return buf.value.decode() or None


def option_names():
    lib, out, i = load(), [], 0
    while True:
        n = lib.ttsamd_option_name(i)
        if not n:
            return out
        out.append(n.decode())
        i += 1


class options:

    def __init__(self, **kv):
        self.kv = kv

    def __enter__(self):
        self.old = {k: get_option(k) for k in self.kv}
        for k, v in self.kv.items():
            set_option(k, v)
        return self

    def __exit__(self, *a):
        for k, v in self.old.items():
            set_option(k, v)


def check(rc, what):
    if rc != 0:
        msg = load().ttsamd_last_error()
        raise TtsAmdError(f'{what} failed ({rc}): {msg.decode() if msg else "?"}')


def make_tensors(state_dict):
    import numpy as np
    keep, items = [], []
    for name, v in state_dict.items():
        if hasattr(v, 'detach'):
            if not v.is_floating_point():
                continue
            v = v.detach().cpu().float().numpy()
        a = np.ascontiguousarray(v, dtype=np.float32)
        if a.ndim > 4:
            continue
        t = Tensor()
        nb = name.encode()
        t.name = nb
        t.data = a.ctypes.data_as(C.POINTER(C.c_float))
        t.ndim = a.ndim
        for i, s in enumerate(a.shape):
            t.shape[i] = s
        keep += [a, nb]
        items.append(t)
    arr = (Tensor * len(items))(*items)
    return arr, keep
```

Before: 69.30 million.

## Fuse three-dilation HiFi-GAN resblock into one f32 Winograd chain kernel

Adds a kernel that runs all three dilated conv pairs of a C=32/64 resblock in a single launch. The input tile with its halo stays in LDS across the stages, so the intermediate activations are never written to or read back from global memory. The HiFi-GAN forward uses it by default when the geometry and switches allow. The cost is a wider halo that the tile has to recompute, plus extra LDS and register pressure that may reduce occupancy.

New measurement: 69.65 million (median of 6 runs). No clear change (+0.5%).

```diff
diff --git a/include/ttsamd.h b/include/ttsamd.h
--- a/include/ttsamd.h
+++ b/include/ttsamd.h
@@ -80,7 +80,7 @@
 } ttsamd_tagger_cfg;
 
 const char* ttsamd_last_error(void);
-#define TTSAMD_ABI_VERSION 7
+#define TTSAMD_ABI_VERSION 8
 int32_t ttsamd_version(void);
 int32_t ttsamd_set_option(const char* name, const char* value);
 int32_t ttsamd_get_option(const char* name, char* value, int32_t capacity);
@@ -174,6 +174,13 @@
                              int32_t channels, int32_t k, int32_t dil, const int64_t* lens, int32_t len_mul, int32_t L,
                              int32_t batch, int32_t mode, float div, float slope, int32_t variant, float* packed, int64_t packed_floats,
                              void* stream);
+
+int64_t ttsamd_resblock_chain_packed_floats(int32_t channels);
+int32_t ttsamd_resblock_chain_geometry(int32_t channels, const int32_t* dilations, int32_t L, int32_t batch, int64_t* out);
+int32_t ttsamd_resblock_chain(const float* x, float* y, const float* const* w1, const float* const* b1, const float* const* w2,
+                              const float* const* b2, const int32_t* dilations, int32_t channels, const int64_t* lens, int32_t len_mul,
+                              int32_t L, int32_t batch, int32_t mode, float div, float slope, float* packed, int64_t packed_floats,
+                              void* stream);
 
 int32_t ttsamd_bfo_pack(const float* x, int32_t batch, int32_t channels, int32_t len, float slope, void* out, void* stream);
 int32_t ttsamd_bfo_unpack(const void* in, int32_t batch, int32_t channels, int32_t len, float slope, float* out, void* stream);
diff --git a/tts-arabic-pytorch_amd/csrc/api.hip b/tts-arabic-pytorch_amd/csrc/api.hip
--- a/tts-arabic-pytorch_amd/csrc/api.hip
+++ b/tts-arabic-pytorch_amd/csrc/api.hip
@@ -574,6 +574,52 @@
     return rc;
 }
 
+int64_t ttsamd_resblock_chain_packed_floats(int32_t channels) {
+    return channels < 1 ? 0 : 6 * (int64_t)channels * wino2_groups(3) * channels;
+}
+
+int32_t ttsamd_resblock_chain_geometry(int32_t channels, const int32_t* dilations, int32_t L, int32_t batch, int64_t* out) {
+    TTS_REQUIRE(dilations && out && (channels == 32 || channels == 64) && L >= 1 && batch >= 1, "resblock_chain_geometry: bad argument");
+    int32_t ht = 0, ts = 0;
+    int64_t lds = 0, blocks = 0;
+    const int32_t rc = resblock_chain_f32_geometry(channels, dilations, L, batch, &ht, &ts, &lds, &blocks);
+    out[0] = ht; out[1] = ts; out[2] = lds; out[3] = blocks;
+    if (rc != 0) set_error("resblock_chain_geometry: dilations %d / %d / %d do not chain", dilations[0], dilations[1], dilations[2]);
+    return rc;
+}
+
+int32_t ttsamd_resblock_chain(const float* x, float* y, const float* const* w1, const float* const* b1, const float* const* w2,
+                              const float* const* b2, const int32_t* dilations, int32_t channels, const int64_t* lens, int32_t len_mul,
+                              int32_t L, int32_t batch, int32_t mode, float div, float slope, float* packed, int64_t packed_floats,
+                              void* stream) {
+    TTS_REQUIRE(x && y && w1 && b1 && w2 && b2 && dilations && packed && batch >= 1 && L >= 1 && len_mul >= 1 && mode >= 0 && mode <= 2,
+                "resblock_chain: bad argument");
+    TTS_REQUIRE(channels == 32 || channels == 64, "resblock_chain: built for C = 32 / 64, not %d", channels);
+    TTS_REQUIRE(packed_floats >= ttsamd_resblock_chain_packed_floats(channels),
+                "resblock_chain: `packed` holds %lld floats, C = %d needs %lld (ttsamd_resblock_chain_packed_floats)",
+                (long long)packed_floats, channels, (long long)ttsamd_resblock_chain_packed_floats(channels));
+    TTS_REQUIRE(resblock_chain_f32_supported(channels, 3, dilations, 3, L, x, y),
+                "resblock_chain: unsupported geometry (C = %d, dilations %d / %d / %d, L = %d; L a multiple of 4, y != x, 16-byte aligned)",
+                channels, dilations[0], dilations[1], dilations[2], L);
+    hipStream_t s = (hipStream_t)stream;
+    const int64_t nw = (int64_t)channels * wino2_groups(3) * channels;
+    const float *w1w[3], *w2w[3];
+    for (int m = 0; m < 3; ++m) {
+        TTS_REQUIRE(w1[m] && b1[m] && w2[m] && b2[m], "resblock_chain: null weight of pair %d", m);
+        for (int i = 0; i < 2; ++i) {
+            float* wino = packed + (2 * m + i) * nw;
+            hipLaunchKernelGGL(pack_wino2_weight_kernel, dim3((unsigned)((nw + 255) / 256)), dim3(256), 0, s, i == 0 ? w1[m] : w2[m],
+                               channels, channels, 3, channels, wino);
+            TTS_CHECK_HIP(hipGetLastError());
+            (i == 0 ? w1w : w2w)[m] = wino;
+        }
+    }
+    prof_begin(s, 3 * 2.0 * (2.0 * channels * channels * 3));
+    const int32_t rc = launch_resblock_chain_f32(channels, x, y, w1w, b1, w2w, b2, dilations, lens, len_mul, L, batch, mode, div, slope, s);
+    prof_end(s);
+    return rc;
+}
+
 int32_t ttsamd_set_precision(int32_t precision) {
     TTS_REQUIRE(precision >= 0 && precision <= 2, "set_precision: 0 = fp32 MFMA, 1 = bf16 MFMA, 2 = split-bf16 MFMA");
     g_precision = precision;
diff --git a/tts-arabic-pytorch_amd/csrc/common.hpp b/tts-arabic-pytorch_amd/csrc/common.hpp
--- a/tts-arabic-pytorch_amd/csrc/common.hpp
+++ b/tts-arabic-pytorch_amd/csrc/common.hpp
@@ -60,6 +60,7 @@
     X(FUSED2_MASK_N1, 1, 0, 0x1ff)          \
     X(FUSED2_WB, 0, 0, 2)                     \
     X(PAIR4, 0, 0, 1)              \
+    X(RESBLOCK_CHAIN, 0, 0, 1)     \
     X(CONVT, 0, 0, 1)                              \
     X(BFO, 0, 0, 1)                \
     X(BFO_CHAIN, 0, 0, 1)                           \
@@ -163,6 +164,14 @@
 int32_t launch_fused_pair4(int32_t channels, const float* x, float* y, const float* w1_wino4, const float* b1, const float* w2_wino4,
                            const float* b2, int32_t k, int32_t dil, const int64_t* lens, int32_t len_mul, int32_t L, int32_t batch,
                            int32_t mode, float div, float slope, hipStream_t stream);
+bool resblock_chain_f32_supported(int32_t channels, int32_t k, const int32_t* dil, int32_t n_dil, int32_t L, const float* x,
+                                  const float* y);
+int32_t launch_resblock_chain_f32(int32_t channels, const float* x, float* y, const float* const* w1_wino, const float* const* b1,
+                                  const float* const* w2_wino, const float* const* b2, const int32_t* dil, const int64_t* lens,
+                                  int32_t len_mul, int32_t L, int32_t batch, int32_t mode, float div, float slope, hipStream_t stream);
+size_t resblock_chain_f32_lds_bytes(int32_t channels);
+int32_t resblock_chain_f32_geometry(int32_t channels, const int32_t* dil, int32_t L, int32_t batch, int32_t* ht, int32_t* ts,
+                                    int64_t* lds_bytes, int64_t* blocks);
 int wino_route(const ConvParams& p);
 int32_t launch_wino(const ConvParams& p, hipStream_t stream);
 void pack_wino_weight(const float* w, int cout, int cin, float* out);
diff --git a/tts-arabic-pytorch_amd/csrc/hifigan.hip b/tts-arabic-pytorch_amd/csrc/hifigan.hip
--- a/tts-arabic-pytorch_amd/csrc/hifigan.hip
+++ b/tts-arabic-pytorch_amd/csrc/hifigan.hip
@@ -56,6 +56,7 @@
     bool on = true, mask_forced = false;
     bool wino_b = true, wino_a = true;
     bool pair4 = true;
+    bool chain = true;
     unsigned mask = kFused2Mask, mask_n1 = kFused2MaskN1;
 };
 static Fused2Switches read_fused2_switches() {
@@ -69,6 +70,7 @@
     sw.wino_b = wb != 0;
     sw.wino_a = wb == 2;
     sw.pair4 = opt_int(OPT_PAIR4, 1) != 0;
+    sw.chain = opt_int(OPT_RESBLOCK_CHAIN, 1) != 0;
     return sw;
 }
 
@@ -88,6 +90,18 @@
         if (!fused_pair2_supported(channels, k, dil, L, x, y, ntw)) return 0;
     }
     return ntw;
+}
+
+static bool chain_f32_wanted(const Fused2Switches& sw, const HifiGan* h, int li0, const int32_t* dl, int n_dil, int32_t L,
+                             const float* x, const float* y, int64_t columns) {
+    if (!sw.chain || !sw.wino_b || !sw.wino_a || n_dil != 3) return false;
+    const int c = h->c1[li0].cin;
+    for (int m = 0; m < 3; ++m) {
+        const ConvW &w1 = h->c1[li0 + m], &w2 = h->c2[li0 + m];
+        if (w1.cin != c || w1.cout != c || w2.cin != c || w2.cout != c || w1.k != 3 || w2.k != 3 || w1.ww_off < 0 || w2.ww_off < 0) return false;
+    }
+    if (!resblock_chain_f32_supported(c, 3, dl, 3, L, x, y)) return false;
+    return fused2_choice(sw, c, 3, dl[0], L, x, y, columns) == 2;
 }
 
 using TensorMap = std::map<std::string, const ttsamd_tensor*>;
@@ -582,6 +596,28 @@
             p.splitk_ws = splitks[j % 3];
             if (multi && j > 0) HG_CHECK_HIP(hipStreamWaitEvent(st, h->ev_fork, 0));
             const float* src = ups_out;
+            if (fused_ok) {
+                const int li0 = (i * cfg.n_kernels + j) * cfg.n_dilations;
+                int32_t dl[3] = {0, 0, 0};
+                for (int m = 0; m < cfg.n_dilations && m < 3; ++m) dl[m] = cfg.resblock_dilations[j][m];
+                if (chain_f32_wanted(f2sw, h, li0, dl, cfg.n_dilations, L, src, cur, (int64_t)B * L)) {
+                    const float *w1w[3], *b1[3], *w2w[3], *b2[3];
+                    for (int m = 0; m < 3; ++m) {
+                        const ConvW &w1 = h->c1[li0 + m], &w2 = h->c2[li0 + m];
+                        w1w[m] = h->dev + w1.ww_off; b1[m] = h->dev + w1.b_off; w2w[m] = h->dev + w2.ww_off; b2[m] = h->dev + w2.b_off;
+                    }
+                    const int mode = cfg.n_kernels == 1 ? 0 : (j == 0 ? 0 : (j + 1 < cfg.n_kernels ? 1 : 2));
+                    if (multi && j > 0) HG_CHECK_HIP(hipStreamWaitEvent(st, h->ev_done[j - 1], 0));
+                    const double fl = 3 * 2.0 * (2.0 * h->c1[li0].cin * h->c1[li0].cin * 3) * mul;
+                    if (in_section) prof_add(fl); else prof_begin(st, fl);
+                    const int32_t crc = launch_resblock_chain_f32(h->c1[li0].cin, src, cur, w1w, b1, w2w, b2, dl, lens, mul, L, B, mode,
+                                                                  (float)cfg.n_kernels, 0.1f, st);
+                    if (!in_section) prof_end(st);
+                    HG_TRY(crc);
+                    if (multi) HG_CHECK_HIP(hipEventRecord(h->ev_done[j], st));
+                    continue;
+                }
+            }
             for (int m = 0; m < cfg.n_dilations; ++m) {
                 const int li = (i * cfg.n_kernels + j) * cfg.n_dilations + m;
                 const int d = cfg.resblock_dilations[j][m];
diff --git a/tts-arabic-pytorch_amd/csrc/resblock_chain_f32.hip b/tts-arabic-pytorch_amd/csrc/resblock_chain_f32.hip
--- /dev/null
+++ b/tts-arabic-pytorch_amd/csrc/resblock_chain_f32.hip
@@ -0,0 +1,333 @@
+#include <algorithm>
+#include <cstdlib>
+#include <cstring>
+
+#include "resblock_fused2.hpp"
+
+namespace ttsamd {
+
+namespace {
+
+constexpr int kChainNB = 256;
+constexpr int kChainPadL = 8;
+constexpr int kChainW = kChainNB + 2 * kChainPadL;
+
+struct ChainF32Params {
+    const float* x;
+    float* y;
+    const float4* w1w[3];
+    const float4* w2w[3];
+    const float* b1[3];
+    const float* b2[3];
+    const int64_t* lens;
+    int32_t len_mul, L, batch;
+    int32_t dil[3];
+    int32_t ht, ts;
+    int32_t mode;
+    float div, slope;
+    int32_t compact;
+};
+
+constexpr int chain_npa(int d) { return d * (128 / d); }
+
+void chain_geometry(const int32_t* d, int32_t& ht, int32_t& ts) {
+    ht = 0; ts = 0;
+    int lo = -kChainPadL, hi = kChainNB + kChainPadL, h = 0;
+    for (int m = 0; m < 3; ++m) {
+        if (d[m] < 1 || d[m] > DMAX) return;
+        const int ilo = std::max(lo + d[m], 0), ihi = std::min(hi - d[m], 2 * chain_npa(d[m]));
+        lo = ilo + 1;
+        hi = std::min(ihi - 1, kChainNB);
+        h += d[m] + 1;
+    }
+    if (lo > h || (h & 3) != 0) return;
+    ht = h;
+    ts = std::max(hi - h, 0) & ~3;
+}
+
+template <typename T>
+__device__ __forceinline__ T pick3(const T (&a)[3], const int m) { return m == 0 ? a[0] : (m == 1 ? a[1] : a[2]); }
+
+template <int C>
+__global__ __launch_bounds__(256, (C == 32 ? kF2Wa32Waves : 2))
+void resblock_chain_f32(const ChainF32Params p) {
+    using G = Fused2Geo<3, C, 2>;
+    constexpr int NOCT = G::NOCT, MT = G::MT, PF = G::PF, TSH = G::TSH, NB = kChainNB, PADL = kChainPadL, W = kChainW;
+    static_assert(G::NB == NB, "one column frame for both phases");
+    extern __shared__ __attribute__((aligned(16))) float4 smem4[];
+    const int tid = threadIdx.x, lane = tid & 63, wid = tid >> 6;
+    const int kk = lane >> 5, l31 = lane & 31;
+    const int jw = wid * 32 + l31;
+    const int HT = p.ht, TS = p.ts;
+    int b = blockIdx.z;
+    int q0 = blockIdx.x * TS;
+    if (p.compact) {
+        int tile = 0;
+        if (!live_tile(p.lens, p.len_mul, p.L, TS, p.batch, blockIdx.z * gridDim.x + blockIdx.x, b, tile)) return;
+        b = __builtin_amdgcn_readfirstlane(b);
+        q0 = __builtin_amdgcn_readfirstlane(tile) * TS;
+    }
+    const int L = p.L;
+    int len = L;
+    if (p.lens) len = min(len, (int)p.lens[b] * p.len_mul);
+    if (q0 >= len) return;
+    const int xf = q0 - HT;
+    const float slope = p.slope;
+    const float* __restrict__ xb = p.x + (int64_t)b * C * L;
+    float4* Xs = smem4;
+
+    float4 aq[PF][MT];
+    {
+        const float4* __restrict__ w0 = p.w1w[0] + kk * C + l31;
+#pragma unroll
+        for (int g = 0; g < PF; ++g)
+#pragma unroll
+            for (int mt = 0; mt < MT; ++mt) aq[g][mt] = w0[g * 2 * C + 32 * mt];
+    }
+
+    {
+        constexpr int NE = (2 * NOCT * W + 255) / 256;
+        float v[NE][4];
+        int eo[NE];
+        bool ok[NE];
+        int okk = 0, col = tid;
+        while (col >= W) { col -= W; ++okk; }
+#pragma unroll
+        for (int u = 0; u < NE; ++u) {
+            const int pos = xf - PADL + col;
+            const int okc = min(okk, 2 * NOCT - 1);
+            ok[u] = pos >= 0 && pos < len;
+            eo[u] = tid + 256 * u < 2 * NOCT * W ? okc * W + col : -1;
+            const float* src = xb + (int64_t)((okc >> 1) * 8 + (okc & 1)) * L + min(max(pos, 0), max(len - 1, 0));
+#pragma unroll
+            for (int pc = 0; pc < 4; ++pc) v[u][pc] = src[(int64_t)2 * pc * L];
+            col += 256;
+            while (col >= W) { col -= W; ++okk; }
+        }
+#pragma unroll
+        for (int u = 0; u < NE; ++u)
+            if (eo[u] >= 0) Xs[eo[u]] = ok[u] ? make_float4(v[u][0], v[u][1], v[u][2], v[u][3]) : make_float4(0.f, 0.f, 0.f, 0.f);
+    }
+    __syncthreads();
+
+    f32x16 accw[4][MT];
+#pragma unroll 1
+    for (int m = 0; m < 3; ++m) {
+        const int dil = pick3(p.dil, m);
+        const bool last = m == 2;
+        const float4* __restrict__ wl1 = pick3(p.w1w, m) + kk * C + l31;
+        const float4* __restrict__ wl2 = pick3(p.w2w, m) + kk * C + l31;
+        const float4* __restrict__ wn1 = last ? nullptr : pick3(p.w1w, m + 1) + kk * C + l31;
+        const float* __restrict__ b1 = pick3(p.b1, m);
+        const float* __restrict__ b2 = pick3(p.b2, m);
+
+        const int npa = dil * (128 / dil);
+        const int pa = min(jw, npa - 1);
+        const int na = dil == 1 ? 2 * pa : (pa / dil) * 2 * dil + pa % dil;
+        f32x16 accA[4][MT];
+#pragma unroll
+        for (int mt = 0; mt < MT; ++mt)
+#pragma unroll
+            for (int r = 0; r < 16; ++r) {
+                const float bv = b1[32 * mt + (r & 3) + 8 * (r >> 2) + 4 * kk];
+                accA[0][mt][r] = bv; accA[1][mt][r] = 0.f; accA[2][mt][r] = 0.f; accA[3][mt][r] = -bv;
+            }
+        conv_phase2_wino<3, C, false, MT, true>(accA, aq, Xs + kk * W + PADL + na - dil, wl1, W, dil, wl2, slope);
+
+        float res0[MT][16], res1[MT][16];
+#pragma unroll
+        for (int mt = 0; mt < MT; ++mt)
+#pragma unroll
+            for (int oc = 0; oc < 4; ++oc)
+#pragma unroll
+                for (int k2 = 0; k2 < 2; ++k2) {
+                    const float* src = reinterpret_cast<const float*>(Xs + ((4 * mt + oc) * 2 + k2) * W + PADL + 2 * jw) + 2 * kk;
+                    const float2 r0 = *reinterpret_cast<const float2*>(src);
+                    const float2 r1 = *reinterpret_cast<const float2*>(src + 4);
+                    res0[mt][4 * oc + k2] = r0.x; res0[mt][4 * oc + k2 + 2] = r0.y;
+                    res1[mt][4 * oc + k2] = r1.x; res1[mt][4 * oc + k2 + 2] = r1.y;
+                }
+        __syncthreads();
+
+        if (jw < npa) {
+#pragma unroll
+            for (int hh = 0; hh < 2; ++hh) {
+                const int t = na + hh * dil;
+                const int pos = xf + t;
+                const bool live = pos >= 0 && pos < len;
+                const int ent = ((t + 1) & 1) * TSH + ((t + 1) >> 1);
+#pragma unroll
+                for (int mt = 0; mt < MT; ++mt)
+#pragma unroll
+                    for (int oc = 0; oc < 4; ++oc)
+#pragma unroll
+                        for (int k2 = 0; k2 < 2; ++k2) {
+                            const int r = 4 * oc + k2;
+                            float v0 = hh ? accA[1][mt][r] - accA[2][mt][r] - accA[3][mt][r] : accA[0][mt][r] + accA[1][mt][r] + accA[2][mt][r];
+                            float v1 = hh ? accA[1][mt][r + 2] - accA[2][mt][r + 2] - accA[3][mt][r + 2]
+                                          : accA[0][mt][r + 2] + accA[1][mt][r + 2] + accA[2][mt][r + 2];
+                            v0 = lrelu_max(v0, slope);
+                            v1 = lrelu_max(v1, slope);
+                            const float2 w2v = live ? make_float2(v0, v1) : make_float2(0.f, 0.f);
+                            *reinterpret_cast<float2*>(reinterpret_cast<float*>(Xs + ((4 * mt + oc) * 2 + k2) * 2 * TSH + ent) + 2 * kk) = w2v;
+                        }
+            }
+        }
+        __syncthreads();
+
+#pragma unroll
+        for (int mt = 0; mt < MT; ++mt)
+#pragma unroll
+            for (int r = 0; r < 16; ++r) {
+                accw[0][mt][r] = res0[mt][r]; accw[1][mt][r] = 0.f; accw[2][mt][r] = 0.f; accw[3][mt][r] = -res1[mt][r];
+            }
+        if (last && p.mode != 0) {
+            const int n = 2 * jw, q = xf + n;
+            const int voff = ((n >= HT && n - HT < TS && q < len) ? q : 0) * 4 + 4 * kk * L * 4;
+            const auto ys = __builtin_amdgcn_make_buffer_rsrc(p.y + (int64_t)b * C * L, 0, C * L * 4, 0x00020000);
+#pragma unroll
+            for (int mt = 0; mt < MT; ++mt) {
+                f32x16 t0, t1;
+#pragma unroll
+                for (int r = 0; r < 16; ++r) {
+                    const int so = (32 * mt + (r & 3) + 8 * (r >> 2)) * L * 4;
+                    t0[r] = __builtin_bit_cast(float, __builtin_amdgcn_raw_buffer_load_b32(ys, voff, so, 0));
+                    t1[r] = __builtin_bit_cast(float, __builtin_amdgcn_raw_buffer_load_b32(ys, voff + 4, so, 0));
+                }
+#pragma unroll
+                for (int r = 0; r < 16; ++r) {
+                    accw[0][mt][r] = t0[r] + accw[0][mt][r];
+                    accw[3][mt][r] = accw[3][mt][r] - t1[r];
+                }
+            }
+        }
+        conv_phase2_wino<3, C, true, MT>(accw, aq, Xs + kk * 2 * TSH + jw, wl2, 2 * TSH, 0, wn1);
+        __syncthreads();
+        if (last) break;
+
+#pragma unroll
+        for (int hh = 0; hh < 2; ++hh) {
+            const int pos = xf + 2 * jw + hh;
+            const bool live = pos >= 0 && pos < len;
+#pragma unroll
+            for (int mt = 0; mt < MT; ++mt)
+#pragma unroll
+                for (int oc = 0; oc < 4; ++oc)
+#pragma unroll
+                    for (int k2 = 0; k2 < 2; ++k2) {
+                        const int r = 4 * oc + k2;
+                        const int ch = 32 * mt + 8 * oc + k2 + 4 * kk;
+                        float v0 = hh ? accw[1][mt][r] - accw[2][mt][r] - accw[3][mt][r] : accw[0][mt][r] + accw[1][mt][r] + accw[2][mt][r];
+                        float v1 = hh ? accw[1][mt][r + 2] - accw[2][mt][r + 2] - accw[3][mt][r + 2]
+                                      : accw[0][mt][r + 2] + accw[1][mt][r + 2] + accw[2][mt][r + 2];
+                        v0 = v0 + b2[ch];
+                        v1 = v1 + b2[ch + 2];
+                        const float2 w2v = live ? make_float2(v0, v1) : make_float2(0.f, 0.f);
+                        *reinterpret_cast<float2*>(reinterpret_cast<float*>(Xs + ((4 * mt + oc) * 2 + k2) * W + PADL + 2 * jw + hh) + 2 * kk) = w2v;
+                    }
+        }
+        __syncthreads();
+    }
+
+    float* ep = reinterpret_cast<float*>(smem4);
+#pragma unroll
+    for (int mt = 0; mt < MT; ++mt)
+#pragma unroll
+        for (int r = 0; r < 16; ++r) {
+            float2 y2;
+            y2.x = accw[0][mt][r] + accw[1][mt][r] + accw[2][mt][r];
+            y2.y = accw[1][mt][r] - accw[2][mt][r] - accw[3][mt][r];
+            *reinterpret_cast<float2*>(ep + (32 * mt + (r & 3) + 8 * (r >> 2) + 4 * kk) * NB + 2 * jw) = y2;
+        }
+    __syncthreads();
+    const bool do_div = p.mode == 2;
+    const float div = p.div;
+    const float* __restrict__ b2 = p.b2[2];
+    float* __restrict__ yb = p.y + (int64_t)b * C * L;
+    const int n = lane * 4;
+    const int wid_u = __builtin_amdgcn_readfirstlane(wid);
+#pragma unroll 4
+    for (int it = 0; it < C / 4; ++it) {
+        const int ch = wid_u + 4 * it;
+        const float bs = b2[ch];
+        const int q = xf + n;
+        if (n < HT || n - HT >= TS || q >= len) continue;
+        const float4 v4 = *reinterpret_cast<const float4*>(ep + ch * NB + n);
+        float vv[4] = {v4.x + bs, v4.y + bs, v4.z + bs, v4.w + bs};
+        if (do_div) {
+#pragma unroll
+            for (int e = 0; e < 4; ++e) vv[e] = vv[e] / div;
+        }
+        float* yp = yb + (int64_t)ch * L + q;
+        if (q + 3 < len) {
+            *reinterpret_cast<float4*>(yp) = make_float4(vv[0], vv[1], vv[2], vv[3]);
+        } else {
+#pragma unroll
+            for (int e = 0; e < 4; ++e)
+                if (q + e < len) yp[e] = vv[e];
+        }
+    }
+}
+
+template <int C>
+int32_t launch_chain_c(const ChainF32Params& p, hipStream_t stream) {
+    static std::atomic<uint64_t> lds_done{0};
+    const size_t lds = resblock_chain_f32_lds_bytes(C);
+    TTS_CHECK_HIP(lds_opt_in((const void*)resblock_chain_f32<C>, (int)lds, lds_done));
+    dim3 grid((p.L + p.ts - 1) / p.ts, 1, p.batch);
+    hipLaunchKernelGGL(resblock_chain_f32<C>, grid, dim3(256), lds, stream, p);
+    TTS_CHECK_HIP(hipGetLastError());
+    return 0;
+}
+
+}
+
+size_t resblock_chain_f32_lds_bytes(int32_t channels) { return (size_t)2 * (channels / 8) * kChainW * sizeof(float4); }
+
+int32_t resblock_chain_f32_geometry(int32_t channels, const int32_t* dil, int32_t L, int32_t batch, int32_t* ht, int32_t* ts,
+                                    int64_t* lds_bytes, int64_t* blocks) {
+    int32_t h = 0, t = 0;
+    chain_geometry(dil, h, t);
+    *ht = h; *ts = t;
+    *lds_bytes = (int64_t)resblock_chain_f32_lds_bytes(channels);
+    *blocks = t > 0 ? (int64_t)((L + t - 1) / t) * batch : 0;
+    return t > 0 ? 0 : TTSAMD_EINVAL;
+}
+
+bool resblock_chain_f32_supported(int32_t channels, int32_t k, const int32_t* dil, int32_t n_dil, int32_t L, const float* x,
+                                  const float* y) {
+    if (!(channels == 32 || channels == 64) || k != 3 || n_dil != 3 || L < 4 || (L & 3) != 0) return false;
+    if (((((uintptr_t)x) | ((uintptr_t)y)) & 15) != 0 || x == y) return false;
+    if ((int64_t)channels * L * 4 >= ((int64_t)1 << 31)) return false;
+    int32_t ht = 0, ts = 0;
+    chain_geometry(dil, ht, ts);
+    return ts >= 4;
+}
+
+int32_t launch_resblock_chain_f32(int32_t channels, const float* x, float* y, const float* const* w1_wino, const float* const* b1,
+                                  const float* const* w2_wino, const float* const* b2, const int32_t* dil, const int64_t* lens,
+                                  int32_t len_mul, int32_t L, int32_t batch, int32_t mode, float div, float slope, hipStream_t stream) {
+    TTS_REQUIRE(resblock_chain_f32_supported(channels, 3, dil, 3, L, x, y),
+                "fp32 ResBlock chain: unsupported geometry (C=%d, dilations %d/%d/%d, L=%d; C = 32 / 64, L a multiple of 4, y != x)",
+                channels, dil[0], dil[1], dil[2], L);
+    TTS_REQUIRE(slope > 0.f && slope <= 1.f, "fp32 ResBlock chain: leaky-relu slope %g outside (0, 1]", (double)slope);
+    TTS_REQUIRE(mode >= 0 && mode <= 2 && batch >= 1 && len_mul >= 1, "fp32 ResBlock chain: bad mode / batch / len_mul");
+    conv_log("resblock_chain_f32", 3, channels, channels, L, batch, 1, mode, len_mul, lens != nullptr, 1);
+    ChainF32Params p;
+    std::memset(&p, 0, sizeof(p));
+    p.x = x; p.y = y;
+    for (int m = 0; m < 3; ++m) {
+        TTS_REQUIRE(w1_wino[m] && b1[m] && w2_wino[m] && b2[m], "fp32 ResBlock chain: null weight of pair %d", m);
+        p.w1w[m] = reinterpret_cast<const float4*>(w1_wino[m]);
+        p.w2w[m] = reinterpret_cast<const float4*>(w2_wino[m]);
+        p.b1[m] = b1[m]; p.b2[m] = b2[m];
+        p.dil[m] = dil[m];
+    }
+    chain_geometry(dil, p.ht, p.ts);
+    p.lens = lens; p.len_mul = len_mul; p.L = L; p.batch = batch;
+    p.mode = mode; p.div = div; p.slope = slope;
+    p.compact = compact_order(lens, batch) ? 1 : 0;
+    return channels == 32 ? launch_chain_c<32>(p, stream) : launch_chain_c<64>(p, stream);
+}
+
+}
diff --git a/tts-arabic-pytorch_amd/csrc/resblock_fused2.hip b/tts-arabic-pytorch_amd/csrc/resblock_fused2.hip
--- a/tts-arabic-pytorch_amd/csrc/resblock_fused2.hip
+++ b/tts-arabic-pytorch_amd/csrc/resblock_fused2.hip
@@ -2,7 +2,7 @@
 #include <cstdlib>
 #include <cstring>
 
-#include "conv_mfma_common.hpp"
+#include "resblock_fused2.hpp"
 
 namespace ttsamd {
 
@@ -22,30 +22,6 @@
     int32_t compact;
 };
 
-template <int K, int C, int NTW>
-struct Fused2Geo {
-    static constexpr int NOCT = C / 8, MT = C / 32;
-    static constexpr int H = (K - 1) / 2;
-    static constexpr int NB = 128 * NTW;
-    static constexpr int TS = (NB - 2 * H) & ~3;
-    static constexpr int TSTR = NB + K - 1;
-    static constexpr int NG = NOCT * K;
-    static constexpr int NS = K / 3, NL = K - 3 * NS, NGW = 4 * NS + 2 * NL;
-    static constexpr int TSH = TSTR / 2;
-    static constexpr int PF = 2;
-    static constexpr int MPO = 4 * MT * NTW * K;
-    static constexpr int UO = NOCT * MPO <= 640 ? NOCT : (4 * MPO <= 640 ? 4 : 2);
-    static_assert(NOCT % UO == 0 && (UO * K) % PF == 0, "unrolled body of the group loop");
-    static constexpr int WAVES = (C == 128 && NTW == 2) ? 1 : (C == 32 ? 4 : 2);
-    __host__ __device__ static constexpr int npa(int d) { return d * (128 / d); }
-    __host__ __device__ static constexpr int ts_wa(int d) { return (2 * npa(d) - 2 * H) & ~3; }
-    static size_t lds_bytes(int dil) { return (size_t)2 * NOCT * (NB + (K - 1) * dil) * sizeof(float4); }
-};
-
-__device__ __forceinline__ float lrelu_max(const float v, const float slope) {
-    return __builtin_amdgcn_fmed3f(v, v * slope, __builtin_inff());
-}
-
 template <int K, int C, int NTW, bool ACT>
 __device__ __forceinline__ void conv_phase2(f32x16 (&acc)[C / 32][NTW], float4 (&aq)[2][C / 32], const float4* sb, const int bstr,
                                             const int bdil, const float4* __restrict__ wl, const float4* __restrict__ wnext,
@@ -102,81 +78,7 @@
     }
 }
 
-template <int K, int C, bool EO, int MTW>
-__device__ __forceinline__ void conv_phase2_wino(f32x16 (&acc)[4][MTW], float4 (&aq)[2][MTW], const float4* sb,
-                                                 const float4* __restrict__ wl, const int rstride, const int cstep,
-                                                 const float4* __restrict__ wnext) {
-    using G = Fused2Geo<K, C, 2>;
-    constexpr int NOCT = G::NOCT, MT = MTW, PF = G::PF, NS = G::NS, NL = G::NL, NGW = G::NGW, TSH = G::TSH;
-    constexpr int NBU = NS + NL;
-    constexpr int NGT = NOCT * NGW;
-    typedef float f32x4v __attribute__((ext_vector_type(4)));
-#define TTS_ENT(SBO, CC) (SBO)[EO ? ((CC) & 1) * TSH + ((CC) >> 1) : (CC) * cstep]
-    float4 bq[2][4];
-#pragma unroll
-    for (int m = 0; m < 4; ++m) bq[0][m] = TTS_ENT(sb, m);
-#pragma unroll 1
-    for (int o = 0; o < NOCT; ++o) {
-        const float4* sbo = sb + o * 2 * rstride;
-        const float4* sbn = sb + min(o + 1, NOCT - 1) * 2 * rstride;
-#pragma unroll
-        for (int u = 0; u < NBU; ++u) {
-            const int cur = u & 1, nxt = cur ^ 1;
-            {
-                const int un = u + 1;
-                if (un < NS) {
-#pragma unroll
-                    for (int m = 0; m < 4; ++m) bq[nxt][m] = TTS_ENT(sbo, 3 * un + m);
-                } else if (un < NBU) {
-                    bq[nxt][0] = TTS_ENT(sbo, 3 * NS + (un - NS));
-                    bq[nxt][1] = TTS_ENT(sbo, 3 * NS + (un - NS) + 1);
-                } else {
-#pragma unroll
-                    for (int m = 0; m < 4; ++m) bq[nxt][m] = TTS_ENT(sbn, m);
-                }
-            }
-            f32x4v x[4], v[4];
-#pragma unroll
-            for (int m = 0; m < 4; ++m) x[m] = f32x4v{bq[cur][m].x, bq[cur][m].y, bq[cur][m].z, bq[cur][m].w};
-            const bool sub = u < NS;
-            if (sub) { v[0] = x[0] - x[2]; v[1] = x[1] + x[2]; v[2] = x[2] - x[1]; v[3] = x[1] - x[3]; }
-            else { v[0] = x[0]; v[1] = x[1]; }
-            const int ng = sub ? 4 : 2;
-            const int g0 = sub ? 4 * u : 4 * NS + 2 * (u - NS);
-#pragma unroll
-            for (int i = 0; i < ng; ++i) {
-                const int g = g0 + i;
-                const int plane = sub ? i : (i ? 3 : 0);
-                const int slot = g % PF;
-                float4 a4[MT];
-#pragma unroll
-                for (int mt = 0; mt < MT; ++mt) a4[mt] = aq[slot][mt];
-                {
-                    const int gn = o * NGW + g + PF;
-                    const float4* __restrict__ src = gn < NGT ? wl + (int64_t)gn * 2 * C
-                                                              : (wnext ? wnext + (int64_t)(gn - NGT) * 2 * C : wl + (int64_t)(NGT - 1) * 2 * C);
-#pragma unroll
-                    for (int mt = 0; mt < MT; ++mt) aq[slot][mt] = src[32 * mt];
-                }
-                __builtin_amdgcn_sched_barrier(0);
-#pragma unroll
-                for (int pq = 0; pq < 4; ++pq)
-#pragma unroll
-                    for (int mt = 0; mt < MT; ++mt) {
-                        const float av = pq == 0 ? a4[mt].x : (pq == 1 ? a4[mt].y : (pq == 2 ? a4[mt].z : a4[mt].w));
-                        acc[plane][mt] = __builtin_amdgcn_mfma_f32_32x32x2f32(av, v[i][pq], acc[plane][mt], 0, 0, 0);
-                    }
-            }
-        }
-        if (NBU & 1) {
-#pragma unroll
-            for (int m = 0; m < 4; ++m) bq[0][m] = bq[1][m];
-        }
-    }
-#undef TTS_ENT
-}
-
-constexpr int kF2Wa32Waves = 3;
+
 template <int C, int WM>
 constexpr int f2_row_halves() { return (WM == 2 && C == 128) ? 2 : 1; }
 
diff --git a/tts-arabic-pytorch_amd/csrc/resblock_fused2.hpp b/tts-arabic-pytorch_amd/csrc/resblock_fused2.hpp
--- /dev/null
+++ b/tts-arabic-pytorch_amd/csrc/resblock_fused2.hpp
@@ -0,0 +1,112 @@
+#pragma once
+
+#include "conv_mfma_common.hpp"
+
+namespace ttsamd {
+
+template <int K, int C, int NTW>
+struct Fused2Geo {
+    static constexpr int NOCT = C / 8, MT = C / 32;
+    static constexpr int H = (K - 1) / 2;
+    static constexpr int NB = 128 * NTW;
+    static constexpr int TS = (NB - 2 * H) & ~3;
+    static constexpr int TSTR = NB + K - 1;
+    static constexpr int NG = NOCT * K;
+    static constexpr int NS = K / 3, NL = K - 3 * NS, NGW = 4 * NS + 2 * NL;
+    static constexpr int TSH = TSTR / 2;
+    static constexpr int PF = 2;
+    static constexpr int MPO = 4 * MT * NTW * K;
+    static constexpr int UO = NOCT * MPO <= 640 ? NOCT : (4 * MPO <= 640 ? 4 : 2);
+    static_assert(NOCT % UO == 0 && (UO * K) % PF == 0, "unrolled body of the group loop");
+    static constexpr int WAVES = (C == 128 && NTW == 2) ? 1 : (C == 32 ? 4 : 2);
+    __host__ __device__ static constexpr int npa(int d) { return d * (128 / d); }
+    __host__ __device__ static constexpr int ts_wa(int d) { return (2 * npa(d) - 2 * H) & ~3; }
+    static size_t lds_bytes(int dil) { return (size_t)2 * NOCT * (NB + (K - 1) * dil) * sizeof(float4); }
+};
+
+__device__ __forceinline__ float lrelu_max(const float v, const float slope) {
+    return __builtin_amdgcn_fmed3f(v, v * slope, __builtin_inff());
+}
+
+template <int K, int C, bool EO, int MTW, bool ACT = false>
+__device__ __forceinline__ void conv_phase2_wino(f32x16 (&acc)[4][MTW], float4 (&aq)[2][MTW], const float4* sb,
+                                                 const float4* __restrict__ wl, const int rstride, const int cstep,
+                                                 const float4* __restrict__ wnext, const float slope = 1.f) {
+    using G = Fused2Geo<K, C, 2>;
+    constexpr int NOCT = G::NOCT, MT = MTW, PF = G::PF, NS = G::NS, NL = G::NL, NGW = G::NGW, TSH = G::TSH;
+    constexpr int NBU = NS + NL;
+    constexpr int NGT = NOCT * NGW;
+    typedef float f32x4v __attribute__((ext_vector_type(4)));
+#define TTS_ENT(SBO, CC) (SBO)[EO ? ((CC) & 1) * TSH + ((CC) >> 1) : (CC) * cstep]
+    float4 bq[2][4];
+#pragma unroll
+    for (int m = 0; m < 4; ++m) bq[0][m] = TTS_ENT(sb, m);
+#pragma unroll 1
+    for (int o = 0; o < NOCT; ++o) {
+        const float4* sbo = sb + o * 2 * rstride;
+        const float4* sbn = sb + min(o + 1, NOCT - 1) * 2 * rstride;
+#pragma unroll
+        for (int u = 0; u < NBU; ++u) {
+            const int cur = u & 1, nxt = cur ^ 1;
+            {
+                const int un = u + 1;
+                if (un < NS) {
+#pragma unroll
+                    for (int m = 0; m < 4; ++m) bq[nxt][m] = TTS_ENT(sbo, 3 * un + m);
+                } else if (un < NBU) {
+                    bq[nxt][0] = TTS_ENT(sbo, 3 * NS + (un - NS));
+                    bq[nxt][1] = TTS_ENT(sbo, 3 * NS + (un - NS) + 1);
+                } else {
+#pragma unroll
+                    for (int m = 0; m < 4; ++m) bq[nxt][m] = TTS_ENT(sbn, m);
+                }
+            }
+            f32x4v x[4], v[4];
+#pragma unroll
+            for (int m = 0; m < 4; ++m) x[m] = f32x4v{bq[cur][m].x, bq[cur][m].y, bq[cur][m].z, bq[cur][m].w};
+            if constexpr (ACT) {
+#pragma unroll
+                for (int m = 0; m < 4; ++m)
+                    x[m] = f32x4v{lrelu_max(x[m].x, slope), lrelu_max(x[m].y, slope), lrelu_max(x[m].z, slope), lrelu_max(x[m].w, slope)};
+            }
+            const bool sub = u < NS;
+            if (sub) { v[0] = x[0] - x[2]; v[1] = x[1] + x[2]; v[2] = x[2] - x[1]; v[3] = x[1] - x[3]; }
+            else { v[0] = x[0]; v[1] = x[1]; }
+            const int ng = sub ? 4 : 2;
+            const int g0 = sub ? 4 * u : 4 * NS + 2 * (u - NS);
+#pragma unroll
+            for (int i = 0; i < ng; ++i) {
+                const int g = g0 + i;
+                const int plane = sub ? i : (i ? 3 : 0);
+                const int slot = g % PF;
+                float4 a4[MT];
+#pragma unroll
+                for (int mt = 0; mt < MT; ++mt) a4[mt] = aq[slot][mt];
+                {
+                    const int gn = o * NGW + g + PF;
+                    const float4* __restrict__ src = gn < NGT ? wl + (int64_t)gn * 2 * C
+                                                              : (wnext ? wnext + (int64_t)(gn - NGT) * 2 * C : wl + (int64_t)(NGT - 1) * 2 * C);
+#pragma unroll
+                    for (int mt = 0; mt < MT; ++mt) aq[slot][mt] = src[32 * mt];
+                }
+                __builtin_amdgcn_sched_barrier(0);
+#pragma unroll
+                for (int pq = 0; pq < 4; ++pq)
+#pragma unroll
+                    for (int mt = 0; mt < MT; ++mt) {
+                        const float av = pq == 0 ? a4[mt].x : (pq == 1 ? a4[mt].y : (pq == 2 ? a4[mt].z : a4[mt].w));
+                        acc[plane][mt] = __builtin_amdgcn_mfma_f32_32x32x2f32(av, v[i][pq], acc[plane][mt], 0, 0, 0);
+                    }
+            }
+        }
+        if (NBU & 1) {
+#pragma unroll
+            for (int m = 0; m < 4; ++m) bq[0][m] = bq[1][m];
+        }
+    }
+#undef TTS_ENT
+}
+
+constexpr int kF2Wa32Waves = 3;
+
+}
diff --git a/tts-arabic-pytorch_amd/ttsamd/engine.py b/tts-arabic-pytorch_amd/ttsamd/engine.py
--- a/tts-arabic-pytorch_amd/ttsamd/engine.py
+++ b/tts-arabic-pytorch_amd/ttsamd/engine.py
@@ -438,6 +438,34 @@
     return y
 
 
+
+def resblock_chain(x, w1s, b1s, w2s, b2s, dilations, lens=None, len_mul=1, y=None, mode=0, div=1.0, slope=0.1):
+    lib = _require_gpu()
+    x = x.contiguous().float()
+    w1s, w2s, b1s, b2s = ([t.contiguous().float() for t in ts] for ts in (w1s, w2s, b1s, b2s))
+    B, Cc, Lx = x.shape
+    if y is None:
+        assert mode == 0
+        y = torch.zeros_like(x)
+    if lens is not None:
+        lens = lens.to(device=x.device, dtype=torch.int64).contiguous()
+    n_packed = int(lib.ttsamd_resblock_chain_packed_floats(Cc))
+    packed = torch.empty(max(n_packed, 1), dtype=torch.float32, device=x.device)
+    arr = lambda ts: (C.c_void_p * 3)(*[t.data_ptr() for t in ts])
+    dl = (C.c_int32 * 3)(*[int(d) for d in dilations])
+    with torch.cuda.device(x.device):
+        L.check(lib.ttsamd_resblock_chain(_ptr(x), _ptr(y), arr(w1s), arr(b1s), arr(w2s), arr(b2s), dl, Cc, _ptr(lens), int(len_mul),
+                                          Lx, B, int(mode), float(div), float(slope), _ptr(packed), n_packed, _stream()),
+                'resblock_chain')
+    return y
+
+
+def resblock_chain_geometry(channels, dilations, L_, batch):
+    out = (C.c_int64 * 4)()
+    dl = (C.c_int32 * 3)(*[int(d) for d in dilations])
+    L.check(L.load().ttsamd_resblock_chain_geometry(int(channels), dl, int(L_), int(batch), out), 'resblock_chain_geometry')
+    return tuple(int(v) for v in out)
+
 def length_regulate(enc, reps, t_max):
     lib = _require_gpu()
     enc = enc.contiguous().float()
diff --git a/tts-arabic-pytorch_amd/ttsamd/lib.py b/tts-arabic-pytorch_amd/ttsamd/lib.py
--- a/tts-arabic-pytorch_amd/ttsamd/lib.py
+++ b/tts-arabic-pytorch_amd/ttsamd/lib.py
@@ -93,6 +93,9 @@
     'ttsamd_conv1d_ex': (_I32, [_P, _P, _P, _P, _P, _I32, _I32, _I32, _I32, _I32, _I32, _F, _I32, _I32, _F, _P, _P, _P]),
     'ttsamd_resblock_pair_packed_floats': (_I64, [_I32, _I32, _I32]),
     'ttsamd_resblock_pair': (_I32, [_P, _P, _P, _P, _P, _P, _I32, _I32, _I32, _P, _I32, _I32, _I32, _I32, _F, _F, _I32, _P, _I64, _P]),
+    'ttsamd_resblock_chain_packed_floats': (_I64, [_I32]),
+    'ttsamd_resblock_chain_geometry': (_I32, [_I32, _P, _I32, _I32, _P]),
+    'ttsamd_resblock_chain': (_I32, [_P, _P, _P, _P, _P, _P, _P, _I32, _P, _I32, _I32, _I32, _I32, _F, _F, _P, _I64, _P]),
     'ttsamd_bfo_pack': (_I32, [_P, _I32, _I32, _I32, _F, _P, _P]),
     'ttsamd_bfo_unpack': (_I32, [_P, _I32, _I32, _I32, _F, _P, _P]),
     'ttsamd_bfo_weight_elems': (_I64, [_I32, _I32, _I32, _I32]),
@@ -126,7 +129,7 @@
 }
 
 _lib = None
-ABI_VERSION = 7
+ABI_VERSION = 8
 
 
 def load():
```
